# gchhablani/multilingual-image-captioning

Hardware: AMD Instinct MI355X
Metric: train images/sec, ViT-B/32+mBART-50 (bf16 train step, batch 64/GPU, 224x224, seq_len 64) (higher is better)
Workload: dtype bf16

## Files before the change

include/mic_hip.h:

```cpp
#ifndef MIC_HIP_H
#define MIC_HIP_H
#include <stdint.h>
#ifdef __cplusplus
extern "C" {
#endif

#define MIC_OK 0
#define MIC_EINVAL (-1)
#define MIC_ELAUNCH (-2)

#define MIC_BF16 0
#define MIC_F32 1
#define MIC_FP8 2
#define MIC_E4M3 0
#define MIC_E5M2 1

#define MIC_ACT_NONE 0
#define MIC_ACT_GELU_ERF 1
#define MIC_ACT_GELU_TANH 2
#define MIC_ACT_QUICK_GELU 3

int mic_version(void);
const char* mic_last_error(void);

typedef struct {
  int dtype;
  int c_dtype;
  int M, N, K;
  int a_kmajor, b_kmajor;
  const void* A; int lda;
  const void* B; int ldb;
  void* C; int ldc;
  const float* bias;
  int act;
  void* Zout; int ldz;
  const void* Zin; int dact;
  const void* R; int ldr;
  int accumulate;
  float dropout_p; uint32_t dropout_seed;
  float alpha;
  int split_k;
  long long split_stride;
  float* a_rowsum;
  int rowsum_k;
  int a_fmt, b_fmt;
  const float* a_scale_inv;
  const float* b_scale_inv;
  float* rowstat; int rowstat_ld; int rowstat_nvalid;
  const long long* a_ln_stats; const float* a_ln_colsum; int a_ln_width; float a_ln_eps;
  long long* rowsum2;
  int k_valid;
  float* c_q8_state; float* c_q8_amax; int c_q8_fmt;
} mic_gemm_args;
int mic_gemm(const mic_gemm_args* a, void* stream);
int mic_sum_slabs(int dst_dtype, int n_slabs, long long slab_stride, int rows, int cols, const float* src, int ld_src,
                  void* dst, int ld_dst, void* stream);
int mic_gemm_grouped(const mic_gemm_args* args, int count, void* stream);
int mic_set_cu_budget(int cus);
int mic_get_cu_budget(void);
typedef struct { int tile, kgroups, blocks, grid, blocks_per_cu, phased, cu_budget, tile_m; } mic_gemm_plan_info;
int mic_gemm_plan(const mic_gemm_args* args, int count, mic_gemm_plan_info* out);
int mic_ln_fold_weight(int dtype, int N, int K, const void* w, int ldw, const float* gamma, const float* beta, const float* bias,
                       void* w_fold, int ldwf, float* colsum, float* bias_fold, void* stream);

typedef struct {
  const void* src; int ld;
  int rows, cols, rows_pad;
  void* q; int ldq;
  void* qT; int ldqT;
  float* state;
  float* amax_next;
  int fmt;
} mic_fp8_item;
int mic_fp8_amax(const mic_fp8_item* items, int count, void* stream);
int mic_fp8_quantize(const mic_fp8_item* items, int count, void* stream);
int mic_fp8_amax_partials(void);
int mic_fp8_roll_amax(float* state, int stride_floats, float* partials, int count, void* stream);

typedef struct {
  void* q; int ldq;
  float* state;
  float* amax_next;
  int fmt;
} mic_fp8_out;

int mic_layernorm_fwd(int dtype, int rows, int width, const void* x, const float* gamma, const float* beta,
                      float eps, void* y, float* mean, float* rstd, float dropout_p, uint32_t dropout_seed,
                      void* stream);
int mic_layernorm_bwd(int dtype, int rows, int width, const void* x, const float* gamma, const float* mean,
                      const float* rstd, const void* dy, const void* dres, void* dx, float* dgamma, float* dbeta,
                      void* dxm, float dropout_p, uint32_t dropout_seed, float in_dropout_p, uint32_t in_dropout_seed,
                      void* stream);
int mic_layernorm_bwd_blocks(int rows);
int mic_layernorm_bwd_partials(int dtype, int rows, int width, const void* x, const float* gamma, const float* mean,
                               const float* rstd, const void* dy, const void* dres, void* dx, float* partials, void* dxm,
                               float dropout_p, uint32_t dropout_seed, float in_dropout_p, uint32_t in_dropout_seed, void* stream);
int mic_layernorm_fwd_q8(int rows, int width, const void* x, const float* gamma, const float* beta, float eps, void* y, float* mean,
                         float* rstd, float dropout_p, uint32_t dropout_seed, const mic_fp8_out* q8, void* stream);
int mic_layernorm_bwd_partials_q8(int rows, int width, const void* x, const float* gamma, const float* mean, const float* rstd,
                                  const void* dy, const void* dres, void* dx, float* partials, void* dxm, float dropout_p,
                                  uint32_t dropout_seed, float in_dropout_p, uint32_t in_dropout_seed, const mic_fp8_out* q8,
                                  int q8_of_dx, void* stream);
typedef struct { const float* partials; float* dgamma; float* dbeta; int nblk, width, accumulate; } mic_ln_param_item;
int mic_ln_param_grads(const mic_ln_param_item* items, int count, void* stream);

int mic_attn_fwd(int dtype, int B, int H, int Tq, int Tk, const void* q, int ldq, const void* k, int ldk,
                 const void* v, int ldv, void* out, int ldo, const int32_t* key_mask, int causal, float* lse,
                 void* stream);
int mic_attn_bwd(int dtype, int B, int H, int Tq, int Tk, const void* q, int ldq, const void* k, int ldk,
                 const void* v, int ldv, const void* out, int ldo, const void* dout, int lddo, const float* lse,
                 const int32_t* key_mask, int causal, void* dq, int lddq, void* dk, int lddk, void* dv, int lddv,
                 void* stream);

int mic_attn_probs(int dtype, int B, int H, int Tq, int Tk, const void* q, int ldq, const void* k, int ldk,
                   const int32_t* key_mask, int causal, float* out, void* stream);

int mic_attn_fwd_packed(int dtype, int B, int H, int Tq_max, int Tk, const int32_t* q_off, const int32_t* q_len, int kv_packed,
                        const void* q, int ldq, const void* k, int ldk, const void* v, int ldv, void* out, int ldo, int causal,
                        float* lse, void* stream);
int mic_attn_bwd_packed(int dtype, int B, int H, int Tq_max, int Tk, const int32_t* q_off, const int32_t* q_len, int kv_packed,
                        const void* q, int ldq, const void* k, int ldk, const void* v, int ldv, const void* out, int ldo,
                        const void* dout, int lddo, const float* lse, int causal, void* dq, int lddq, void* dk, int lddk,
                        void* dv, int lddv, void* stream);
int mic_attn_bwd_q8(int B, int H, int Tq, int Tk, const int32_t* q_off, const int32_t* q_len, int kv_packed, const void* q, int ldq,
                    const void* k, int ldk, const void* v, int ldv, const void* out, int ldo, const void* dout, int lddo, const float* lse,
                    const int32_t* key_mask, int causal, const mic_fp8_out* dq8, const mic_fp8_out* dk8, void* dv8, void* stream);

int mic_attn_decode(int dtype, int R, int H, int max_len, int cur, const void* q, int ldq, const void* kc,
                    const void* vc, int ldc, const int32_t* src_row, int row_div, void* out, int ldo, void* stream);
int mic_kv_append(int dtype, int R, int HD, int max_len, int cur, const void* k, int ldk, const void* v, int ldv,
                  void* kc, void* vc, void* stream);

int mic_im2col(int dtype, int B, int img, int ps, const float* pixels, void* patches, int ldp, int trunc_int32,
               void* stream);
int mic_vit_assemble(int dtype, int B, int S, int width, const void* patch_out, int ldp, const float* cls,
                     const float* pos, void* x, void* stream);
int mic_vit_assemble_bwd(int dtype, int B, int S, int width, const void* dx, void* dpatch, int ldp, float* dcls,
                         float* dpos, void* stream);

int mic_embed_fwd(int dtype, int rows, int width, const int32_t* ids, const int32_t* pos_ids, const void* table,
                  const float* pos_table, float scale, void* h, void* stream);
int mic_embed_bwd(int dtype, int rows, int width, const int32_t* ids, const int32_t* pos_ids, const void* dh,
                  float scale, float* dtable, float* dpos_table, void* stream);
int mic_embed_rows_add_det(int dtype, int n, int width, int vocab, const int32_t* ids, const void* dh, float scale, float* dtable,
                           int32_t* ws, void* stream);
int64_t mic_embed_rows_add_det_ws(int vocab);

int mic_ce_rows(int dtype, int rows, int V, const void* logits, int ld, const int32_t* labels,
                const int32_t* mask, float label_smoothing, float* row_lse, float* row_loss, void* stream);
int mic_ce_rows_tiles(int dtype, int rows, int V, const void* logits, int ld, const float* rowstat, int stat_ld,
                      const int32_t* labels, float* row_lse, float* row_loss, void* stream);
int mic_ce_reduce(int rows, const float* row_loss, const int32_t* mask, float* loss_out, float* denom_out,
                  void* stream);
int mic_ce_bwd(int dtype, int rows, int V, int Vpad, void* logits, int ld, const int32_t* labels,
               const int32_t* mask, float label_smoothing, const float* row_lse, const float* denom,
               float loss_scale, void* stream);
int mic_ce_bwd_q8(int rows, int V, int Vpad, const void* logits, int ld, const int32_t* labels, const int32_t* mask,
                  float label_smoothing, const float* row_lse, const float* denom, float loss_scale, const mic_fp8_out* q8,
                  float* colsum, float* label_coef, void* stream);
int mic_head_label_terms(int rows, int width, const int32_t* labels, const float* coef, const void* E, int lde, const void* h, int ldh,
                         float* dx_slab, int ldx, float* dE, int ldde, void* stream);
int mic_ce_bwd_t(int rows, int V, int Vpad, void* logits, int ld, const int32_t* labels, const int32_t* mask, float label_smoothing,
                 const float* row_lse, const float* denom, float loss_scale, void* dlogits_t, int ld_t, int rows_pad, float* colsum,
                 void* stream);
int mic_transpose_bf16(int rows, int rows_pad, int cols, const void* src, int ld_src, void* dst, int ld_dst, void* stream);

int mic_colsum(int dtype, int rows, int cols, const void* x, int ld, float* out, int accumulate, void* stream);
typedef struct { const void* x; float* out; int rows, cols, ld; } mic_colsum_item;
int mic_colsum_grouped(int dtype, const mic_colsum_item* items, int count, void* stream);
typedef struct { const void* x; float* out; const float* scale_inv; int rows, cols, ld, fmt; } mic_colsum_q8_item;
int mic_colsum_q8_grouped(const mic_colsum_q8_item* items, int count, void* stream);
int mic_dropout_mask(uint8_t* out, int64_t n, float p, uint32_t seed, void* stream);
int mic_cast(int src_dtype, int dst_dtype, const void* src, void* dst, int64_t n, void* stream);
int mic_zero(void* p, int64_t bytes, void* stream);
int mic_stream_create_cu_masked(int first_cu, int n_cus, void** stream);
int mic_stream_destroy(void* stream);
int mic_comm_emulate(const void* src, void* dst, int64_t bytes, float micros, int blocks, void* stream);
int mic_copy_rows(int dtype, int n, int width, const void* src, int ld_src, const int32_t* src_idx, void* dst, int ld_dst,
                  const int32_t* dst_idx, void* stream);
int mic_cast2d(int src_dtype, int dst_dtype, int rows, int cols, const void* src, int ld_src, void* dst, int ld_dst,
               void* stream);

int mic_adamw(int64_t n, float* p, float* m, float* v, const float* g, void* p_lp, const float* hyper, double b1,
              double b2, double eps, double wd, float grad_scale, void* stream);
int mic_adamw_rows(int64_t rows, int width, const uint8_t* row_flag, int want, float* p, float* m, float* v, const float* g,
                   void* p_lp, const float* hyper, double b1, double b2, double eps, double wd, float grad_scale, void* stream);
int mic_row_flags(const int32_t* ids, int n_ids, uint8_t* flags, int n_rows, void* stream);

int mic_row_lse_topk(int dtype, int R, int V, const void* logits, int ld, int k, int forced_token,
                     int suppress_eos, int eos_token_id, int raw_logits, const float* row_bias, float* top_val,
                     int32_t* top_idx, void* stream);

int mic_row_topk_tiles(int dtype, int R, int V, const void* logits, int ld, const float* rowstat, int stat_ld, int k,
                       int suppress_eos, int eos_token_id, int raw_logits, const float* row_bias, float* top_val,
                       int32_t* top_idx, void* stream);

typedef struct {
  int B, K, max_len, V;
  int cur_len;
  int eos_token_id, pad_token_id;
  float length_penalty; int early_stopping;
  const float* cand_val;
  const int32_t* cand_idx;
  int32_t* running_seq;
  float* running_scores;
  int32_t* seq;
  float* scores;
  int32_t* finished;
  int32_t* src_row;
  int32_t* next_token;
  int32_t* flags;
  int32_t* gstate;
} mic_beam_step_args;
int mic_beam_step(const mic_beam_step_args* a, void* stream);

int mic_greedy_step(int B, int max_len, int cur_len, int eos_token_id, int pad_token_id, const int32_t* top_idx,
                    int ld_top, int32_t* sequences, int32_t* finished, int32_t* next_token, void* stream);

int mic_sample_rows(int dtype, int R, int V, const void* logits, int ld, uint32_t key0, uint32_t key1,
                    float temperature, int forced_token, int suppress_eos, int eos_token_id, const float* min_keep,
                    const int32_t* tie_limit, int32_t* out_idx, void* stream);
int mic_warp_thresholds(int dtype, int R, int V, const void* logits, int ld, float temperature, int suppress_eos,
                        int eos_token_id, int top_k, float top_p, float* thr, int32_t* tie_limit, void* stream);

typedef struct { const void* src; int H, W, hwc; } mic_image_item;
int mic_image_transform(const mic_image_item* items, int n, int out_size, const float* mean, const float* std,
                        float* dst, int dst_chw, void* stream);

#ifdef __cplusplus
}
#endif
#endif
```

multilingual-image-captioning_amd/_lib.py:

```python
from __future__ import annotations

import ctypes as C
import os

_HERE = os.path.dirname(os.path.abspath(__file__))
LIB_PATH = os.path.join(_HERE, "libmic_hip.so")

MIC_BF16, MIC_F32, MIC_FP8 = 0, 1, 2
MIC_E4M3, MIC_E5M2 = 0, 1
ACT_NONE, ACT_GELU_ERF, ACT_GELU_TANH, ACT_QUICK_GELU = 0, 1, 2, 3
ACT_IDS = {"none": 0, None: 0, "gelu": 1, "erf": 1, "gelu_erf": 1, "tanh": 2, "gelu_tanh": 2, "gelu_new": 2, "quick_gelu": 3}


class MicError(RuntimeError):
    pass


class GemmArgs(C.Structure):
    _fields_ = [
        ("dtype", C.c_int), ("c_dtype", C.c_int), ("M", C.c_int), ("N", C.c_int), ("K", C.c_int),
        ("a_kmajor", C.c_int), ("b_kmajor", C.c_int),
        ("A", C.c_void_p), ("lda", C.c_int), ("B", C.c_void_p), ("ldb", C.c_int), ("C", C.c_void_p), ("ldc", C.c_int),
        ("bias", C.c_void_p), ("act", C.c_int), ("Zout", C.c_void_p), ("ldz", C.c_int), ("Zin", C.c_void_p),
        ("dact", C.c_int), ("R", C.c_void_p), ("ldr", C.c_int), ("accumulate", C.c_int), ("dropout_p", C.c_float),
        ("dropout_seed", C.c_uint32), ("alpha", C.c_float), ("split_k", C.c_int),
        ("split_stride", C.c_longlong), ("a_rowsum", C.c_void_p), ("rowsum_k", C.c_int),
        ("a_fmt", C.c_int), ("b_fmt", C.c_int), ("a_scale_inv", C.c_void_p), ("b_scale_inv", C.c_void_p),
        ("rowstat", C.c_void_p), ("rowstat_ld", C.c_int), ("rowstat_nvalid", C.c_int),
        ("a_ln_stats", C.c_void_p), ("a_ln_colsum", C.c_void_p), ("a_ln_width", C.c_int), ("a_ln_eps", C.c_float),
        ("rowsum2", C.c_void_p), ("k_valid", C.c_int),
        ("c_q8_state", C.c_void_p), ("c_q8_amax", C.c_void_p), ("c_q8_fmt", C.c_int),
    ]


class Fp8Item(C.Structure):
    _fields_ = [("src", C.c_void_p), ("ld", C.c_int), ("rows", C.c_int), ("cols", C.c_int), ("rows_pad", C.c_int),
                ("q", C.c_void_p), ("ldq", C.c_int), ("qT", C.c_void_p), ("ldqT", C.c_int), ("state", C.c_void_p), ("amax_next", C.c_void_p),
                ("fmt", C.c_int)]


class Fp8Out(C.Structure):
    _fields_ = [("q", C.c_void_p), ("ldq", C.c_int), ("state", C.c_void_p), ("amax_next", C.c_void_p), ("fmt", C.c_int)]


class ColsumQ8Item(C.Structure):
    _fields_ = [("x", C.c_void_p), ("out", C.c_void_p), ("scale_inv", C.c_void_p), ("rows", C.c_int), ("cols", C.c_int), ("ld", C.c_int), ("fmt", C.c_int)]


class ColsumItem(C.Structure):
    _fields_ = [("x", C.c_void_p), ("out", C.c_void_p), ("rows", C.c_int), ("cols", C.c_int), ("ld", C.c_int)]


class BeamStepArgs(C.Structure):
    _fields_ = [
        ("B", C.c_int), ("K", C.c_int), ("max_len", C.c_int), ("V", C.c_int), ("cur_len", C.c_int),
        ("eos_token_id", C.c_int), ("pad_token_id", C.c_int), ("length_penalty", C.c_float), ("early_stopping", C.c_int),
        ("cand_val", C.c_void_p), ("cand_idx", C.c_void_p), ("running_seq", C.c_void_p), ("running_scores", C.c_void_p),
        ("seq", C.c_void_p), ("scores", C.c_void_p), ("finished", C.c_void_p), ("src_row", C.c_void_p),
        ("next_token", C.c_void_p), ("flags", C.c_void_p), ("gstate", C.c_void_p),
    ]


class GemmPlanInfo(C.Structure):
    _fields_ = [("tile", C.c_int), ("kgroups", C.c_int), ("blocks", C.c_int), ("grid", C.c_int), ("blocks_per_cu", C.c_int),
                ("phased", C.c_int), ("cu_budget", C.c_int), ("tile_m", C.c_int)]


class LnParamItem(C.Structure):
    _fields_ = [("partials", C.c_void_p), ("dgamma", C.c_void_p), ("dbeta", C.c_void_p), ("nblk", C.c_int), ("width", C.c_int), ("accumulate", C.c_int)]


class ImageItem(C.Structure):
    _fields_ = [("src", C.c_void_p), ("H", C.c_int), ("W", C.c_int), ("hwc", C.c_int)]


_i, _f, _p, _u32, _i64 = C.c_int, C.c_float, C.c_void_p, C.c_uint32, C.c_int64
_SIGS = {
    "mic_version": ([], C.c_int),
    "mic_last_error": ([], C.c_char_p),
    "mic_gemm": ([C.POINTER(GemmArgs), _p], C.c_int),
    "mic_gemm_grouped": ([C.POINTER(GemmArgs), _i, _p], C.c_int),
    "mic_set_cu_budget": ([_i], C.c_int),
    "mic_get_cu_budget": ([], C.c_int),
    "mic_gemm_plan": ([C.POINTER(GemmArgs), _i, C.POINTER(GemmPlanInfo)], C.c_int),
    "mic_comm_emulate": ([_p, _p, _i64, _f, _i, _p], C.c_int),
    "mic_ln_fold_weight": ([_i, _i, _i, _p, _i, _p, _p, _p, _p, _i, _p, _p, _p], C.c_int),
    "mic_fp8_amax": ([C.POINTER(Fp8Item), _i, _p], C.c_int),
    "mic_fp8_quantize": ([C.POINTER(Fp8Item), _i, _p], C.c_int),
    "mic_fp8_amax_partials": ([], C.c_int),
    "mic_fp8_roll_amax": ([_p, _i, _p, _i, _p], C.c_int),
    "mic_sum_slabs": ([_i, _i, C.c_longlong, _i, _i, _p, _i, _p, _i, _p], C.c_int),
    "mic_layernorm_fwd": ([_i, _i, _i, _p, _p, _p, _f, _p, _p, _p, _f, _u32, _p], C.c_int),
    "mic_layernorm_bwd": ([_i, _i, _i, _p, _p, _p, _p, _p, _p, _p, _p, _p, _p, _f, _u32, _f, _u32, _p], C.c_int),
    "mic_layernorm_bwd_blocks": ([_i], C.c_int),
    "mic_layernorm_bwd_partials": ([_i, _i, _i, _p, _p, _p, _p, _p, _p, _p, _p, _p, _f, _u32, _f, _u32, _p], C.c_int),
    "mic_ln_param_grads": ([C.POINTER(LnParamItem), _i, _p], C.c_int),
    "mic_layernorm_fwd_q8": ([_i, _i, _p, _p, _p, _f, _p, _p, _p, _f, _u32, C.POINTER(Fp8Out), _p], C.c_int),
    "mic_layernorm_bwd_partials_q8": ([_i, _i, _p, _p, _p, _p, _p, _p, _p, _p, _p, _f, _u32, _f, _u32, C.POINTER(Fp8Out), _i, _p], C.c_int),
    "mic_attn_bwd_q8": ([_i, _i, _i, _i, _p, _p, _i, _p, _i, _p, _i, _p, _i, _p, _i, _p, _i, _p, _p, _i, C.POINTER(Fp8Out), C.POINTER(Fp8Out), _p, _p], C.c_int),
    "mic_colsum_q8_grouped": ([C.POINTER(ColsumQ8Item), _i, _p], C.c_int),
    "mic_attn_fwd": ([_i, _i, _i, _i, _i, _p, _i, _p, _i, _p, _i, _p, _i, _p, _i, _p, _p], C.c_int),
    "mic_attn_probs": ([_i, _i, _i, _i, _i, _p, _i, _p, _i, _p, _i, _p, _p], C.c_int),
    "mic_attn_bwd": ([_i, _i, _i, _i, _i, _p, _i, _p, _i, _p, _i, _p, _i, _p, _i, _p, _p, _i, _p, _i, _p, _i, _p, _i, _p], C.c_int),
    "mic_attn_fwd_packed": ([_i, _i, _i, _i, _i, _p, _p, _i, _p, _i, _p, _i, _p, _i, _p, _i, _i, _p, _p], C.c_int),
    "mic_attn_bwd_packed": ([_i, _i, _i, _i, _i, _p, _p, _i, _p, _i, _p, _i, _p, _i, _p, _i, _p, _i, _p, _i, _p, _i, _p, _i, _p, _i, _p], C.c_int),
    "mic_attn_decode": ([_i, _i, _i, _i, _i, _p, _i, _p, _p, _i, _p, _i, _p, _i, _p], C.c_int),
    "mic_kv_append": ([_i, _i, _i, _i, _i, _p, _i, _p, _i, _p, _p, _p], C.c_int),
    "mic_im2col": ([_i, _i, _i, _i, _p, _p, _i, _i, _p], C.c_int),
    "mic_vit_assemble": ([_i, _i, _i, _i, _p, _i, _p, _p, _p, _p], C.c_int),
    "mic_vit_assemble_bwd": ([_i, _i, _i, _i, _p, _p, _i, _p, _p, _p], C.c_int),
    "mic_embed_fwd": ([_i, _i, _i, _p, _p, _p, _p, _f, _p, _p], C.c_int),
    "mic_embed_bwd": ([_i, _i, _i, _p, _p, _p, _f, _p, _p, _p], C.c_int),
    "mic_embed_rows_add_det": ([_i, _i, _i, _i, _p, _p, _f, _p, _p, _p], C.c_int),
    "mic_embed_rows_add_det_ws": ([_i], C.c_int64),
    "mic_ce_rows": ([_i, _i, _i, _p, _i, _p, _p, _f, _p, _p, _p], C.c_int),
    "mic_ce_rows_tiles": ([_i, _i, _i, _p, _i, _p, _i, _p, _p, _p, _p], C.c_int),
    "mic_row_topk_tiles": ([_i, _i, _i, _p, _i, _p, _i, _i, _i, _i, _i, _p, _p, _p, _p], C.c_int),
    "mic_ce_reduce": ([_i, _p, _p, _p, _p, _p], C.c_int),
    "mic_ce_bwd": ([_i, _i, _i, _i, _p, _i, _p, _p, _f, _p, _p, _f, _p], C.c_int),
    "mic_ce_bwd_t": ([_i, _i, _i, _p, _i, _p, _p, _f, _p, _p, _f, _p, _i, _i, _p, _p], C.c_int),
    "mic_ce_bwd_q8": ([_i, _i, _i, _p, _i, _p, _p, _f, _p, _p, _f, C.POINTER(Fp8Out), _p, _p, _p], C.c_int),
    "mic_head_label_terms": ([_i, _i, _p, _p, _p, _i, _p, _i, _p, _i, _p, _i, _p], C.c_int),
    "mic_transpose_bf16": ([_i, _i, _i, _p, _i, _p, _i, _p], C.c_int),
    "mic_colsum": ([_i, _i, _i, _p, _i, _p, _i, _p], C.c_int),
    "mic_colsum_grouped": ([_i, C.POINTER(ColsumItem), _i, _p], C.c_int),
    "mic_dropout_mask": ([_p, _i64, _f, _u32, _p], C.c_int),
    "mic_cast": ([_i, _i, _p, _p, _i64, _p], C.c_int),
    "mic_zero": ([_p, _i64, _p], C.c_int),
    "mic_stream_create_cu_masked": ([_i, _i, C.POINTER(C.c_void_p)], C.c_int),
    "mic_stream_destroy": ([_p], C.c_int),
    "mic_copy_rows": ([_i, _i, _i, _p, _i, _p, _p, _i, _p, _p], C.c_int),
    "mic_cast2d": ([_i, _i, _i, _i, _p, _i, _p, _i, _p], C.c_int),
    "mic_adamw": ([_i64, _p, _p, _p, _p, _p, _p, C.c_double, C.c_double, C.c_double, C.c_double, _f, _p], C.c_int),
    "mic_adamw_rows": ([_i64, _i, _p, _i, _p, _p, _p, _p, _p, _p, C.c_double, C.c_double, C.c_double, C.c_double, _f, _p], C.c_int),
    "mic_row_flags": ([_p, _i, _p, _i, _p], C.c_int),
    "mic_row_lse_topk": ([_i, _i, _i, _p, _i, _i, _i, _i, _i, _i, _p, _p, _p, _p], C.c_int),
    "mic_beam_step": ([C.POINTER(BeamStepArgs), _p], C.c_int),
    "mic_greedy_step": ([_i, _i, _i, _i, _i, _p, _i, _p, _p, _p, _p], C.c_int),
    "mic_sample_rows": ([_i, _i, _i, _p, _i, _u32, _u32, _f, _i, _i, _i, _p, _p, _p, _p], C.c_int),
    "mic_warp_thresholds": ([_i, _i, _i, _p, _i, _f, _i, _i, _i, _f, _p, _p, _p], C.c_int),
    "mic_image_transform": ([C.POINTER(ImageItem), _i, _i, C.POINTER(C.c_float), C.POINTER(C.c_float), _p, _i, _p], C.c_int),
}
EXPORTS = tuple(_SIGS)

_lib = None


def lib() -> C.CDLL:
    global _lib
    if _lib is None:
        if not os.path.exists(LIB_PATH):
            raise MicError(f"{LIB_PATH} is missing: build it with `python -c 'import __graft_entry__ as g; g.build()'` "
                           "(hipcc --offload-arch=gfx950).  The HIP path has no fallback.")
        l = C.CDLL(LIB_PATH)
        for name, (args, res) in _SIGS.items():
            fn = getattr(l, name)
            fn.argtypes, fn.restype = args, res
        _lib = l
    return _lib


def check(rc: int, what: str = "") -> None:
    if rc != 0:
        raise MicError(f"{what} failed (rc={rc}): {lib().mic_last_error().decode()}")
```

multilingual-image-captioning_amd/csrc/elementwise.hip:

```cpp
#include "common.h"
#include <stdarg.h>
#include <type_traits>

static thread_local char g_err[512] = "";
void mic_set_error(const char* fmt, ...) {
  va_list ap;
  va_start(ap, fmt);
  vsnprintf(g_err, sizeof(g_err), fmt, ap);
  va_end(ap);
}
extern "C" const char* mic_last_error(void) { return g_err; }
extern "C" int mic_version(void) { return 1; }

template <typename F>
static int dispatch_t(int dtype, F&& f) {
  if (dtype == MIC_BF16) f((uint16_t*)nullptr);
  else if (dtype == MIC_F32) f((float*)nullptr);
  else { mic_set_error("bad dtype %d", dtype); return MIC_EINVAL; }
  hipError_t e = hipGetLastError();
  if (e != hipSuccess) { mic_set_error("launch failed: %s", hipGetErrorString(e)); return MIC_ELAUNCH; }
  return MIC_OK;
}
#define TYPE_OF(tag) typename std::remove_pointer<decltype(tag)>::type

// ... 464 lines not shown
__global__ __launch_bounds__(256) void ce_bwd_kernel(int V, int Vpad, T* __restrict__ logits, int ld,
                                                     const int32_t* __restrict__ labels, const int32_t* __restrict__ mask,
                                                     float ls, const float* __restrict__ row_lse, const float* __restrict__ denom,
                                                     float loss_scale) {
  const int row = blockIdx.x;
  T* lr = logits + (size_t)row * ld;
  const float w = mask[row] ? loss_scale / denom[0] : 0.f;
  const float lse = row_lse[row];
  const int label = labels[row];
  const float conf = 1.0f - ls, low = ls > 0.f ? ls / (float)(V - 1) : 0.f;
  const int nchunk = Vpad >> 3;
  constexpr int U = 4;
  for (int ch0 = threadIdx.x; ch0 < nchunk; ch0 += 256 * U) {
    float v[U][8];
#pragma unroll
    for (int u = 0; u < U; ++u)
      if (ch0 + u * 256 < nchunk) ld8(lr + (ch0 + u * 256) * 8, v[u]);
#pragma unroll
    for (int u = 0; u < U; ++u) {
      const int ch = ch0 + u * 256;
      if (ch >= nchunk) break;
      float o[8];
#pragma unroll
      for (int i = 0; i < 8; ++i) {
        const int c = ch * 8 + i;
        o[i] = c < V ? w * (__expf(v[u][i] - lse) - (c == label ? conf : low)) : 0.f;
      }
      st8(lr + ch * 8, o);
    }
  }
}
extern "C" int mic_ce_bwd(int dtype, int rows, int V, int Vpad, void* logits, int ld, const int32_t* labels,
                          const int32_t* mask, float label_smoothing, const float* row_lse, const float* denom,
                          float loss_scale, void* stream) {
  MIC_CHECK(rows > 0 && V > 1 && Vpad >= V && Vpad % 8 == 0 && ld >= Vpad && logits && labels && mask && row_lse && denom, "mic_ce_bwd: bad args");
  return dispatch_t(dtype, [&](auto* tag) {
    using T = TYPE_OF(tag);
    hipLaunchKernelGGL(ce_bwd_kernel<T>, dim3(rows), dim3(256), 0, (hipStream_t)stream, V, Vpad, (T*)logits, ld, labels, mask, label_smoothing, row_lse, denom, loss_scale);
  });
}

struct TransposeArgs {
  const uint16_t* src; uint16_t* src_rw; int ld_src;
  uint16_t* dst; int ld_dst;
  int rows, cols;
  int V; const int32_t* labels; const int32_t* mask; float ls; const float* row_lse; const float* denom; float loss_scale;
  float* colsum;
};
template <int OP>
__global__ __launch_bounds__(256) void tile_transpose_kernel(TransposeArgs a) {
  __shared__ __attribute__((aligned(16))) char img[64 * 1024];
  const int tid = threadIdx.x, lane = tid & 63, wave = tid >> 6;
  const int c0 = blockIdx.x * 512, r0 = blockIdx.y * 64;
  const int col = c0 + lane * 8;
  const bool col_ok = col < a.cols;
  uint4 q[16];
#pragma unroll
  for (int rr = 0; rr < 16; ++rr) {
    const int row = r0 + wave * 16 + rr;
    q[rr] = make_uint4(0u, 0u, 0u, 0u);
    if (row < a.rows && col_ok) q[rr] = *reinterpret_cast<const uint4*>(a.src + (size_t)row * a.ld_src + col);
  }
  float inv_denom = 0.f;
  if constexpr (OP == 1) inv_denom = a.loss_scale / a.denom[0];
#pragma unroll
  for (int rr = 0; rr < 16; ++rr) {
    const int k = wave * 16 + rr, row = r0 + k;
    uint4 u = q[rr];
    if constexpr (OP == 1) {
      if (row < a.rows && col_ok) {
        const float w = a.mask[row] ? inv_denom : 0.f;
        const float lse = a.row_lse[row];
        const int label = a.labels[row];
        const float conf = 1.0f - a.ls, low = a.ls > 0.f ? a.ls / (float)(a.V - 1) : 0.f;
        const uint32_t wd[4] = {u.x, u.y, u.z, u.w};
        float o[8];
#pragma unroll
        for (int i = 0; i < 8; ++i) {
          const float x = __uint_as_float((i & 1) ? (wd[i >> 1] & 0xffff0000u) : (wd[i >> 1] << 16));
          const int c = col + i;
          o[i] = c < a.V ? w * (__expf(x - lse) - (c == label ? conf : low)) : 0.f;
        }
        u.x = f2bf_pk(o[0], o[1]); u.y = f2bf_pk(o[2], o[3]); u.z = f2bf_pk(o[4], o[5]); u.w = f2bf_pk(o[6], o[7]);
        *reinterpret_cast<uint4*>(a.src_rw + (size_t)row * a.ld_src + col) = u;
      }
    }
    const int pos = (lane & ~7) | ((lane ^ (k >> 3)) & 7);
    *reinterpret_cast<uint4*>(img + k * 1024 + pos * 16) = u;
  }
  __syncthreads();
  const int kc = lane & 7, xx = lane >> 3;
#pragma unroll 4
  for (int it = 0; it < 16; ++it) {
    const int xl = wave * 128 + it * 8 + xx;
    const int c = xl >> 3;
    const int pos = (c & ~7) | ((c ^ kc) & 7);
    const char* base = img + (kc * 8) * 1024 + pos * 16 + (xl & 7) * 2;
    uint16_t e[8];
#pragma unroll
    for (int i = 0; i < 8; ++i) e[i] = *reinterpret_cast<const uint16_t*>(base + i * 1024);
    const int x = c0 + xl;
    if (x < a.cols) {
      uint4 u;
      u.x = (uint32_t)e[0] | ((uint32_t)e[1] << 16); u.y = (uint32_t)e[2] | ((uint32_t)e[3] << 16);
      u.z = (uint32_t)e[4] | ((uint32_t)e[5] << 16); u.w = (uint32_t)e[6] | ((uint32_t)e[7] << 16);
      *reinterpret_cast<uint4*>(a.dst + (size_t)x * a.ld_dst + r0 + kc * 8) = u;
    }
    if constexpr (OP == 1) {
      if (a.colsum != nullptr) {
        float sacc = 0.f;
#pragma unroll
        for (int i = 0; i < 8; ++i) sacc += bf2f(e[i]);
        sacc = group8_sum(sacc);
        if (kc == 0 && x < a.cols && sacc != 0.f) atomicAdd(a.colsum + x, sacc);
      }
    }
  }
}
extern "C" int mic_transpose_bf16(int rows, int rows_pad, int cols, const void* src, int ld_src, void* dst, int ld_dst, void* stream) {
  if (rows_pad <= 0) rows_pad = (rows + 63) / 64 * 64;
  MIC_CHECK(rows > 0 && cols > 0 && cols % 8 == 0 && src && dst && ld_src >= cols && ld_src % 8 == 0 && rows_pad >= rows && rows_pad % 64 == 0 &&
                ld_dst >= rows_pad && ld_dst % 8 == 0,
            "mic_transpose_bf16: bad args (cols %% 8 == 0, ld_src %% 8 == 0, rows_pad %% 64 == 0, ld_dst >= rows_pad and %% 8 == 0)");
  MIC_CHECK(((uintptr_t)src & 15) == 0 && ((uintptr_t)dst & 15) == 0, "mic_transpose_bf16: 16-B aligned operands");
  TransposeArgs a{};
  a.src = (const uint16_t*)src; a.ld_src = ld_src; a.dst = (uint16_t*)dst; a.ld_dst = ld_dst; a.rows = rows; a.cols = cols;
  hipLaunchKernelGGL(tile_transpose_kernel<0>, dim3((cols + 511) / 512, rows_pad / 64), dim3(256), 0, (hipStream_t)stream, a);
  MIC_LAUNCH_CHECK();
  return MIC_OK;
}
extern "C" int mic_ce_bwd_t(int rows, int V, int Vpad, void* logits, int ld, const int32_t* labels, const int32_t* mask,
                            float label_smoothing, const float* row_lse, const float* denom, float loss_scale, void* dlogits_t,
                            int ld_t, int rows_pad, float* colsum, void* stream) {
  if (rows_pad <= 0) rows_pad = (rows + 63) / 64 * 64;
  MIC_CHECK(rows_pad >= rows && rows_pad % 64 == 0, "mic_ce_bwd_t: rows_pad >= rows, a multiple of 64");
  MIC_CHECK(rows > 0 && V > 1 && Vpad >= V && Vpad % 8 == 0 && ld >= Vpad && ld % 8 == 0 && logits && labels && mask && row_lse && denom && dlogits_t,
            "mic_ce_bwd_t: bad args");
  MIC_CHECK(ld_t >= rows_pad && ld_t % 8 == 0 && ((uintptr_t)logits & 15) == 0 && ((uintptr_t)dlogits_t & 15) == 0,
            "mic_ce_bwd_t: ld_t >= rows rounded up to 64, ld_t %% 8 == 0, 16-B aligned operands");
  TransposeArgs a{};
  a.src = (const uint16_t*)logits; a.src_rw = (uint16_t*)logits; a.ld_src = ld; a.dst = (uint16_t*)dlogits_t; a.ld_dst = ld_t;
  a.rows = rows; a.cols = Vpad; a.V = V; a.labels = labels; a.mask = mask; a.ls = label_smoothing; a.row_lse = row_lse; a.denom = denom;
  a.loss_scale = loss_scale; a.colsum = colsum;
  hipLaunchKernelGGL(tile_transpose_kernel<1>, dim3((Vpad + 511) / 512, rows_pad / 64), dim3(256), 0, (hipStream_t)stream, a);
  MIC_LAUNCH_CHECK();
  return MIC_OK;
}

struct CeQ8Args {
  const uint16_t* logits; int ld; int rows, V, Vpad;
  const int32_t* labels; const int32_t* mask; float ls; const float* row_lse; const float* denom; float loss_scale;
  float* colsum; uint8_t* q; int ldq; float* state; int fmt;
  float* label_coef;
};
constexpr int CEQ8_RG = 4;
__global__ __launch_bounds__(256) void ce_bwd_q8_kernel(CeQ8Args a) {
  __shared__ __attribute__((aligned(16))) float cs[4][512];
  const int tid = threadIdx.x, lane = tid & 63, wave = tid >> 6;
  const int c0 = blockIdx.x * 512;
  const int col = c0 + lane * 8;
  const bool col_ok = col < a.Vpad;
  const float fmax = a.fmt == MIC_E4M3 ? 448.0f : 57344.0f;
  const float inv_denom = a.loss_scale / a.denom[0];
  if (blockIdx.x == 0 && blockIdx.y == 0 && tid == 0) { a.state[0] = fmax / inv_denom; a.state[1] = inv_denom / fmax; }
  const float conf = 1.0f - a.ls, low = a.ls > 0.f ? a.ls / (float)(a.V - 1) : 0.f;
  float csum[8] = {0.f, 0.f, 0.f, 0.f, 0.f, 0.f, 0.f, 0.f};
  for (int rg = 0; rg < CEQ8_RG; ++rg) {
    const int r0 = (blockIdx.y * CEQ8_RG + rg) * 64;
    if (r0 >= a.rows) break;
    uint4 q[16];
#pragma unroll
    for (int rr = 0; rr < 16; ++rr) {
      const int row = r0 + wave * 16 + rr;
      q[rr] = make_uint4(0u, 0u, 0u, 0u);
      if (row < a.rows && col_ok) q[rr] = *reinterpret_cast<const uint4*>(a.logits + (size_t)row * a.ld + col);
    }
#pragma unroll
    for (int rr = 0; rr < 16; ++rr) {
      const int row = r0 + wave * 16 + rr;
      if (row < a.rows && col_ok) {
        const float w = a.mask[row] ? 1.0f : 0.f;
        const float lse = a.row_lse[row];
        const int label = a.labels[row];
        if (a.label_coef != nullptr && col == 0 && (label < 0 || label >= a.V)) a.label_coef[row] = 0.f;
        const uint32_t wd[4] = {q[rr].x, q[rr].y, q[rr].z, q[rr].w};
        float o[8];
#pragma unroll
        for (int i = 0; i < 8; ++i) {
          const float x = __uint_as_float((i & 1) ? (wd[i >> 1] & 0xffff0000u) : (wd[i >> 1] << 16));
          const int c = col + i;
          const float g = c < a.V ? w * (__expf(x - lse) - (c == label ? conf : low)) : 0.f;
          csum[i] += g;
          o[i] = fminf(fmaxf(g * fmax, -fmax), fmax);
          if (c == label && a.label_coef != nullptr) {
            a.label_coef[row] = g * inv_denom;
            o[i] = 0.f;
          }
        }
        *reinterpret_cast<uint2*>(a.q + (size_t)row * a.ldq + col) = make_uint2(cvt4_fp8(o, a.fmt), cvt4_fp8(o + 4, a.fmt));
      }
    }
  }
  if (a.colsum != nullptr) {
    *reinterpret_cast<float4*>(&cs[wave][lane * 8]) = make_float4(csum[0], csum[1], csum[2], csum[3]);
    *reinterpret_cast<float4*>(&cs[wave][lane * 8 + 4]) = make_float4(csum[4], csum[5], csum[6], csum[7]);
    __syncthreads();
#pragma unroll
    for (int h = 0; h < 2; ++h) {
      const int c = tid + h * 256;
      const float s4 = (cs[0][c] + cs[1][c]) + (cs[2][c] + cs[3][c]);
      if (c0 + c < a.Vpad && s4 != 0.f) atomicAdd(a.colsum + c0 + c, s4 * inv_denom);
    }
  }
}
extern "C" int mic_ce_bwd_q8(int rows, int V, int Vpad, const void* logits, int ld, const int32_t* labels, const int32_t* mask,
                             float label_smoothing, const float* row_lse, const float* denom, float loss_scale, const mic_fp8_out* q8,
                             float* colsum, float* label_coef, void* stream) {
  MIC_CHECK(rows > 0 && V > 1 && Vpad >= V && Vpad % 8 == 0 && ld >= Vpad && ld % 8 == 0 && logits && labels && mask && row_lse && denom && q8,
            "mic_ce_bwd_q8: bad args");
  MIC_CHECK(q8->q && q8->state && q8->ldq >= Vpad && q8->ldq % 8 == 0 && ((uintptr_t)q8->q & 7) == 0 && ((uintptr_t)logits & 15) == 0 &&
                (q8->fmt == MIC_E4M3 || q8->fmt == MIC_E5M2),
            "mic_ce_bwd_q8: fp8 output [rows][ldq >= Vpad] (ldq %% 8 == 0, 8-B aligned), a scale state, 16-B aligned bf16 logits");
  CeQ8Args a{};
  a.logits = (const uint16_t*)logits; a.ld = ld; a.rows = rows; a.V = V; a.Vpad = Vpad; a.labels = labels; a.mask = mask; a.ls = label_smoothing;
  a.row_lse = row_lse; a.denom = denom; a.loss_scale = loss_scale; a.colsum = colsum;
  a.q = (uint8_t*)q8->q; a.ldq = q8->ldq; a.state = q8->state; a.fmt = q8->fmt; a.label_coef = label_coef;
  hipLaunchKernelGGL(ce_bwd_q8_kernel, dim3((Vpad + 511) / 512, (rows + 64 * CEQ8_RG - 1) / (64 * CEQ8_RG)), dim3(256), 0, (hipStream_t)stream, a);
  MIC_LAUNCH_CHECK();
  return MIC_OK;
}

__global__ __launch_bounds__(256) void head_label_terms_kernel(int rows, int width, const int32_t* __restrict__ labels, const float* __restrict__ coef,
                                                               const uint16_t* __restrict__ E, int lde, const uint16_t* __restrict__ h, int ldh,
                                                               float* __restrict__ dx_slab, int ldx, float* __restrict__ dE, int ldde) {
  const int m = blockIdx.x;
  const float c = coef[m];
  const int lab = labels[m];
  for (int j = threadIdx.x; j < width; j += 256) {
    float o = 0.f;
    if (c != 0.f) {
      o = c * bf2f(E[(size_t)lab * lde + j]);
      atomicAdd(dE + (size_t)lab * ldde + j, c * bf2f(h[(size_t)m * ldh + j]));
    }
    dx_slab[(size_t)m * ldx + j] = o;
  }
}
extern "C" int mic_head_label_terms(int rows, int width, const int32_t* labels, const float* coef, const void* E, int lde, const void* h, int ldh,
                                    float* dx_slab, int ldx, float* dE, int ldde, void* stream) {
  MIC_CHECK(rows > 0 && width > 0 && width % 8 == 0 && labels && coef && E && h && dx_slab && dE && lde % 8 == 0 && ldh % 8 == 0 && ldx % 4 == 0,
            "mic_head_label_terms: bad args (width, lde, ldh multiples of 8; bf16 E and h)");
  hipLaunchKernelGGL(head_label_terms_kernel, dim3(rows), dim3(256), 0, (hipStream_t)stream, rows, width, labels, coef, (const uint16_t*)E, lde,
                     (const uint16_t*)h, ldh, dx_slab, ldx, dE, ldde);
  MIC_LAUNCH_CHECK();
  return MIC_OK;
}

#define COLSUM_MAX 8
struct ColsumItem { const void* x; float* out; int rows, cols, ld, gx, gy, block_begin; };
struct ColsumTable { int count; ColsumItem it[COLSUM_MAX]; };

template <typename T>
__global__ __launch_bounds__(256) void colsum_kernel(ColsumTable tab) {
  __shared__ float red[8][256 + 8];
  int pi = 0;
#pragma unroll
  for (int i = 1; i < COLSUM_MAX; ++i)
    if (i < tab.count && (int)blockIdx.x >= tab.it[i].block_begin) pi = i;
  const ColsumItem& I = tab.it[pi];
  const int local = blockIdx.x - I.block_begin;
  const int bx = local % I.gx, by = local / I.gx;
  const T* __restrict__ x = (const T*)I.x;
  const int rows = I.rows, cols = I.cols, ld = I.ld;
  const int cc = threadIdx.x & 31, rl = threadIdx.x >> 5;
  const int c0 = bx * 256 + cc * 8;
  const int rows_per = (rows + I.gy - 1) / I.gy;
  const int r0 = by * rows_per, r1 = min(rows, r0 + rows_per);
  float acc[8] = {0, 0, 0, 0, 0, 0, 0, 0};
  if (c0 + 8 <= cols) {
    for (int r = r0 + rl; r < r1; r += 8) {
      float v[8];
      ld8(x + (size_t)r * ld + c0, v);
#pragma unroll
      for (int i = 0; i < 8; ++i) acc[i] += v[i];
    }
  } else if (c0 < cols) {
    for (int r = r0 + rl; r < r1; r += 8)
      for (int i = 0; i < cols - c0; ++i) acc[i] += ElemT<T>::ld(x + (size_t)r * ld + c0 + i);
  }
#pragma unroll
  for (int i = 0; i < 8; ++i) red[rl][cc * 8 + i] = acc[i];
  __syncthreads();
  const int c = bx * 256 + threadIdx.x;
  if (c < cols) {
    float s = 0.f;
#pragma unroll
    for (int j = 0; j < 8; ++j) s += red[j][threadIdx.x];
    atomicAdd(I.out + c, s);
  }
}
static int colsum_launch(int dtype, const mic_colsum_item* items, int count, void* stream) {
  ColsumTable tab;
  tab.count = count;
  int blocks = 0;
  for (int i = 0; i < count; ++i) {
    const mic_colsum_item& a = items[i];
    MIC_CHECK(a.rows > 0 && a.cols > 0 && a.x && a.out, "mic_colsum: bad args");
    MIC_CHECK(a.ld % 8 == 0 && ((uintptr_t)a.x & 15) == 0, "mic_colsum: rows must be 16-B aligned");
    ColsumItem& t = tab.it[i];
    t.x = a.x; t.out = a.out; t.rows = a.rows; t.cols = a.cols; t.ld = a.ld;
    t.gx = (a.cols + 255) / 256;
    int gy = (a.rows + 63) / 64;
    const int cap = (1024 + t.gx - 1) / t.gx;
    if (gy > cap) gy = cap;
    t.gy = gy < 1 ? 1 : gy;
    t.block_begin = blocks;
    blocks += t.gx * t.gy;
  }
  return dispatch_t(dtype, [&](auto* tag) {
    using T = TYPE_OF(tag);
    hipLaunchKernelGGL(colsum_kernel<T>, dim3(blocks), dim3(256), 0, (hipStream_t)stream, tab);
  });
}
struct Colsum8Item { const uint8_t* x; float* out; const float* scale_inv; int rows, cols, ld, fmt, gx, gy, block_begin; };
struct Colsum8Table { int count; Colsum8Item it[COLSUM_MAX]; };
typedef float f32x2v __attribute__((ext_vector_type(2)));
__global__ __launch_bounds__(256) void colsum_q8_kernel(Colsum8Table tab) {
  __shared__ float red[8][256 + 8];
  int pi = 0;
#pragma unroll
  for (int i = 1; i < COLSUM_MAX; ++i)
    if (i < tab.count && (int)blockIdx.x >= tab.it[i].block_begin) pi = i;
  const Colsum8Item& I = tab.it[pi];
  const int local = blockIdx.x - I.block_begin;
  const int bx = local % I.gx, by = local / I.gx;
  const int cc = threadIdx.x & 31, rl = threadIdx.x >> 5;
  const int c0 = bx * 256 + cc * 8;
  const int rows_per = (I.rows + I.gy - 1) / I.gy;
  const int r0 = by * rows_per, r1 = min(I.rows, r0 + rows_per);
  float acc[8] = {0, 0, 0, 0, 0, 0, 0, 0};
  if (c0 < I.cols) {
    for (int r = r0 + rl; r < r1; r += 8) {
      const uint2 u = *reinterpret_cast<const uint2*>(I.x + (size_t)r * I.ld + c0);
      const int w[2] = {(int)u.x, (int)u.y};
#pragma unroll
      for (int h = 0; h < 2; ++h) {
        f32x2v lo, hi;
        if (I.fmt == MIC_E4M3) { lo = __builtin_amdgcn_cvt_pk_f32_fp8(w[h], false); hi = __builtin_amdgcn_cvt_pk_f32_fp8(w[h], true); }
        else { lo = __builtin_amdgcn_cvt_pk_f32_bf8(w[h], false); hi = __builtin_amdgcn_cvt_pk_f32_bf8(w[h], true); }
        acc[4 * h + 0] += lo[0]; acc[4 * h + 1] += lo[1]; acc[4 * h + 2] += hi[0]; acc[4 * h + 3] += hi[1];
      }
    }
  }
#pragma unroll
  for (int i = 0; i < 8; ++i) red[rl][cc * 8 + i] = acc[i];
  __syncthreads();
  const int c = bx * 256 + threadIdx.x;
  if (c < I.cols) {
    float t = 0.f;
#pragma unroll
    for (int j = 0; j < 8; ++j) t += red[j][threadIdx.x];
    atomicAdd(I.out + c, t * I.scale_inv[0]);
  }
}
extern "C" int mic_colsum_q8_grouped(const mic_colsum_q8_item* items, int count, void* stream) {
  MIC_CHECK(items && count >= 1, "mic_colsum_q8_grouped: bad args");
  for (int i0 = 0; i0 < count; i0 += COLSUM_MAX) {
    Colsum8Table tab;
    tab.count = count - i0 < COLSUM_MAX ? count - i0 : COLSUM_MAX;
    int blocks = 0;
    for (int i = 0; i < tab.count; ++i) {
      const mic_colsum_q8_item& a = items[i0 + i];
      MIC_CHECK(a.rows > 0 && a.cols > 0 && a.x && a.out && a.scale_inv, "mic_colsum_q8_grouped: bad item %d", i0 + i);
      MIC_CHECK(a.cols % 8 == 0 && a.ld % 8 == 0 && ((uintptr_t)a.x & 7) == 0 && (a.fmt == MIC_E4M3 || a.fmt == MIC_E5M2), "mic_colsum_q8_grouped: cols, ld multiples of 8; fmt");
      Colsum8Item& t = tab.it[i];
      t.x = (const uint8_t*)a.x; t.out = a.out; t.scale_inv = a.scale_inv; t.rows = a.rows; t.cols = a.cols; t.ld = a.ld; t.fmt = a.fmt;
      t.gx = (a.cols + 255) / 256;
      int gy = (a.rows + 63) / 64;
      const int cap = (1024 + t.gx - 1) / t.gx;
      if (gy > cap) gy = cap;
// ... 267 lines not shown
```

multilingual-image-captioning_amd/csrc/gemm.hip:

```cpp
#include "gemm_common.h"

__global__ __launch_bounds__(256) void gemm_f32_kernel(const float* __restrict__ A, long sam, long sak,
                                                       const float* __restrict__ B, long sbk, long sbn, int M, int N,
                                                       int K, EpiArgs epi) {
  __shared__ float As[64][17];
  __shared__ float Bs[16][65];
  const int tid = threadIdx.x, lane = tid & 63, wave = tid >> 6;
  const int m0 = blockIdx.y * 64, n0 = blockIdx.x * 64;
  const int wr = wave >> 1, wc = wave & 1;
  f32x16 acc;
#pragma unroll
  for (int r = 0; r < 16; ++r) acc[r] = 0.0f;
  for (int k0 = 0; k0 < K; k0 += 16) {
#pragma unroll
    for (int i = 0; i < 4; ++i) {
      const int e = tid + i * 256;
      {
        int mm, kk;
        if (sak == 1) { mm = e >> 4; kk = e & 15; } else { kk = e >> 6; mm = e & 63; }
        const int gm = m0 + mm, gk = k0 + kk;
        As[mm][kk] = (gm < M && gk < K) ? A[gm * sam + gk * sak] : 0.0f;
      }
      {
        int nn, kk;
        if (sbk == 1) { nn = e >> 4; kk = e & 15; } else { kk = e >> 6; nn = e & 63; }
        const int gn = n0 + nn, gk = k0 + kk;
        Bs[kk][nn] = (gn < N && gk < K) ? B[gk * sbk + gn * sbn] : 0.0f;
      }
    }
    __syncthreads();
#pragma unroll
    for (int k = 0; k < 16; k += 2) {
      const float a = As[wr * 32 + (lane & 31)][k + (lane >> 5)];
      const float b = Bs[k + (lane >> 5)][wc * 32 + (lane & 31)];
      acc = __builtin_amdgcn_mfma_f32_32x32x2f32(a, b, acc, 0, 0, 0);
    }
    __syncthreads();
  }
  const int n = n0 + wc * 32 + (lane & 31);
#pragma unroll
  for (int r = 0; r < 16; ++r) {
    const int m = m0 + wr * 32 + (r & 3) + 8 * (r >> 2) + 4 * (lane >> 5);
    if (m < M && n < N) epilogue_store<float>(epi, m, n, acc[r]);
  }
}

static int fill_epi(const mic_gemm_args* a, EpiArgs& e) {
  MIC_CHECK(a && a->A && a->B && a->C, "mic_gemm: null pointer");
  MIC_CHECK(a->M > 0 && a->N > 0 && a->K > 0, "mic_gemm: bad shape M=%d N=%d K=%d", a->M, a->N, a->K);
  MIC_CHECK(a->dtype == MIC_BF16 || a->dtype == MIC_F32 || a->dtype == MIC_FP8, "mic_gemm: bad dtype %d", a->dtype);
  if (a->dtype == MIC_FP8) {
    MIC_CHECK(a->c_dtype == MIC_BF16 || a->c_dtype == MIC_F32 || a->c_dtype == MIC_FP8, "mic_gemm(fp8): C is bf16, f32 or (fused emission) fp8");
    if (a->c_dtype == MIC_FP8) {
      MIC_CHECK(a->c_q8_state && (a->c_q8_fmt == MIC_E4M3 || a->c_q8_fmt == MIC_E5M2), "mic_gemm(fp8 C): c_q8_state / c_q8_fmt");
      MIC_CHECK((a->act || a->dact || a->Zout) && !a->accumulate && a->split_k <= 1 && !a->a_kmajor, "mic_gemm(fp8 C): an activation / dact epilogue of an NT launch, no accumulate / split-K");
      MIC_CHECK(a->N % 8 == 0 && a->ldc % 8 == 0 && ((uintptr_t)a->C & 7) == 0 && (!a->Zout || a->ldz % 8 == 0) && (!a->Zin || a->ldz % 8 == 0) && (!a->R || a->ldr % 8 == 0),
                "mic_gemm(fp8 C): N, ldc, ldz, ldr multiples of 8");
    }
    MIC_CHECK(a->a_kmajor == a->b_kmajor, "mic_gemm(fp8): both operands k-contiguous (NT) or both k-major (TN, the weight-gradient GEMM)");
    if (a->a_kmajor) MIC_CHECK(a->M % 16 == 0 && a->N % 16 == 0, "mic_gemm(fp8, k-major): M and N must be multiples of 16");
    MIC_CHECK((a->a_fmt == MIC_E4M3 || a->a_fmt == MIC_E5M2) && a->b_fmt == MIC_E4M3, "mic_gemm(fp8): A is e4m3 or e5m2, B is e4m3");
    MIC_CHECK(a->K % 128 == 0, "mic_gemm(fp8): K=%d must be a multiple of 128 (zero-pad the reduction dim)", a->K);
    MIC_CHECK(a->lda % 16 == 0 && a->ldb % 16 == 0, "mic_gemm(fp8): lda/ldb must be multiples of 16 bytes");
    MIC_CHECK(((uintptr_t)a->A & 15) == 0 && ((uintptr_t)a->B & 15) == 0, "mic_gemm(fp8): A/B must be 16-B aligned");
    MIC_CHECK(!a->a_rowsum, "mic_gemm(fp8): no row sums on the fp8 path (mic_colsum_q8_grouped)");
    if (a->split_k > 1)
      MIC_CHECK(a->split_stride > 0 && a->c_dtype == MIC_F32 && !a->a_kmajor && !a->bias && !a->act && !a->dact && !a->Zout && !a->R && !a->accumulate && a->dropout_p == 0.f,
                "mic_gemm(fp8): split_k writes raw fp32 partial sums into per-split slabs (split_stride > 0, NT, no other epilogue)");
  } else
  MIC_CHECK(a->c_dtype == a->dtype || a->c_dtype == MIC_F32, "mic_gemm: c_dtype must be dtype or f32");
  MIC_CHECK(!(a->dact && !a->Zin), "mic_gemm: dact needs Zin");
  MIC_CHECK(a->dropout_p >= 0.f && a->dropout_p < 1.f, "mic_gemm: dropout_p out of range");
  MIC_CHECK(a->c_dtype != MIC_FP8 || a->dtype == MIC_FP8, "mic_gemm: an fp8 C belongs to the fp8 GEMMs");
  e.C = a->C; e.ldc = a->ldc; e.c_f32 = (a->c_dtype == MIC_F32);
  e.c_q8 = a->c_dtype == MIC_FP8 ? 1 + a->c_q8_fmt : 0; e.q8_state = a->c_q8_state; e.q8_amax = a->c_q8_amax;
  e.bias = a->bias; e.act = a->act; e.Zout = a->Zout; e.ldz = a->ldz; e.Zin = a->Zin; e.dact = a->dact;
  e.R = a->R; e.ldr = a->ldr; e.accumulate = a->accumulate;
  e.drop_thr = a->dropout_p > 0.f ? (uint32_t)fminf(a->dropout_p * 4294967296.0f, 4294967295.0f) : 0u;
  e.drop_seed = a->dropout_seed; e.drop_scale = 1.0f / (1.0f - a->dropout_p);
  e.alpha = a->alpha == 0.f ? 1.0f : a->alpha; e.N = a->N;
  e.rowstat = a->rowstat; e.stat_ld = a->rowstat_ld; e.stat_nvalid = a->rowstat_nvalid > 0 ? a->rowstat_nvalid : a->N;
  if (a->rowstat) {
    MIC_CHECK((a->dtype == MIC_BF16 || (a->dtype == MIC_FP8 && !a->a_kmajor)) && a->c_dtype == MIC_BF16 && a->split_k <= 1 && !a->act && !a->dact && !a->R &&
                  !a->accumulate && a->dropout_p == 0.f && !a->Zout,
              "mic_gemm: rowstat goes with the bare bias epilogue of a bf16 / fp8 NT GEMM with a bf16 C (the LM head)");
    MIC_CHECK(a->N % 64 == 0 && a->ldc % 8 == 0 && ((uintptr_t)a->C & 15) == 0, "mic_gemm: rowstat needs N %% 64 == 0 and a 16-B aligned C");
    MIC_CHECK(a->rowstat_ld >= a->N / 64 && ((uintptr_t)a->rowstat & 7) == 0, "mic_gemm: rowstat needs ld >= N / 64 float2 entries per row");
  }
  e.ln_stats = a->a_ln_stats; e.ln_g = a->a_ln_colsum; e.ln_bias = nullptr; e.ln_inv_d = 0.f; e.ln_eps = a->a_ln_eps;
  e.rowsum2 = a->rowsum2;
  if (a->a_ln_stats) {
    MIC_CHECK(a->dtype == MIC_BF16 && a->a_ln_colsum && a->bias && a->a_ln_width > 0, "mic_gemm: a folded LayerNorm needs bf16 operands, a_ln_colsum, bias' and a_ln_width");
    MIC_CHECK(a->split_k <= 1 && !a->dact && !a->accumulate && (a->alpha == 0.f || a->alpha == 1.f), "mic_gemm: folded LayerNorm: no split-K / dact / accumulate / alpha");
    MIC_CHECK(a->N % 8 == 0 && a->ldc % 8 == 0 && ((uintptr_t)a->C & 15) == 0 && (!a->R || a->ldr % 8 == 0) && (!a->Zout || a->ldz % 8 == 0),
              "mic_gemm: folded LayerNorm needs the vector epilogue (N, ldc, ldr, ldz multiples of 8, 16-B aligned C)");
    e.ln_bias = a->bias; e.bias = nullptr; e.ln_inv_d = 1.0f / (float)a->a_ln_width;
  }
  if (a->rowsum2) {
    MIC_CHECK(a->dtype == MIC_BF16 && a->N % 128 == 0 && a->split_k <= 1 && !a->act && !a->dact && !a->Zout && !a->accumulate,
              "mic_gemm: rowsum2 goes with the bare / residual epilogue of a bf16 GEMM, N %% 128 == 0");
    MIC_CHECK(a->ldc % 8 == 0 && ((uintptr_t)a->C & 15) == 0 && (!a->R || (a->ldr % 8 == 0 && ((uintptr_t)a->R & 15) == 0 && a->c_dtype != MIC_F32)),
              "mic_gemm: rowsum2 needs the PLAIN store path (16-B aligned C / R rows)");
  }
  if (a->dtype == MIC_BF16) {
    MIC_CHECK(a->K % 64 == 0, "mic_gemm(bf16): K=%d must be a multiple of 64 (zero-pad the reduction dim)", a->K);
    MIC_CHECK(a->lda % 8 == 0 && a->ldb % 8 == 0, "mic_gemm(bf16): lda/ldb must be multiples of 8");
    MIC_CHECK(((uintptr_t)a->A & 15) == 0 && ((uintptr_t)a->B & 15) == 0, "mic_gemm(bf16): A/B must be 16-B aligned");
    if (a->a_kmajor) MIC_CHECK(a->M % 8 == 0, "mic_gemm(bf16): k-major A needs M %% 8 == 0");
    if (a->b_kmajor) MIC_CHECK(a->N % 8 == 0, "mic_gemm(bf16): k-major B needs N %% 8 == 0");
    if (a->split_k > 1)
      MIC_CHECK(a->c_dtype == MIC_F32 && !a->bias && !a->act && !a->dact && !a->Zout && !a->R && !a->accumulate && a->dropout_p == 0.f,
                "mic_gemm: split_k accumulates raw fp32 partial sums into a zeroed C (no other epilogue)");
  }
  return MIC_OK;
}

bool table_is_plain(const LaunchTable& t) {
  for (int i = 0; i < t.count; ++i) {
    const EpiArgs& e = t.p[i].epi;
    if (t.p[i].nsplit > 1 || e.act || e.Zout || e.dact || e.accumulate || (e.ldc & 7)) return false;
    if (((uintptr_t)e.C & 15) != 0) return false;
    if (e.R && ((e.ldr & 7) || ((uintptr_t)e.R & 15) || e.c_f32)) return false;
  }
  return true;
}
static bool any_rowsum_early(const mic_gemm_args* args, int count) {
  for (int i = 0; i < count; ++i)
    if (args[i].a_rowsum) return true;
  return false;
}
static thread_local int g_cu_budget = 0;
int mic_cu_budget_now() {
  static const int env = [] { const char* e = getenv("MIC_FREE_CUS"); return e ? atoi(e) : 0; }();
  int c = g_cu_budget > 0 ? g_cu_budget : (env > 0 ? env : 256);
  c = c < 8 ? 8 : (c > 256 ? 256 : c);
  return c & ~7;
}
extern "C" int mic_set_cu_budget(int cus) {
  MIC_CHECK(cus == 0 || (cus >= 8 && cus <= 1024), "mic_set_cu_budget: %d (0 = default, else 8..1024)", cus);
  g_cu_budget = cus;
  return MIC_OK;
}
extern "C" int mic_get_cu_budget(void) { return mic_cu_budget_now(); }

struct GemmPlan { int bm, bm_m, kgroups, blocks, grid, per_cu, phased; };

static GemmPlan plan_bf16(const mic_gemm_args* args, int count) {
  const int cus = mic_cu_budget_now();
  GemmPlan pl{};
  long tiles_big = 0, tiles_small = 0;
  for (int i = 0; i < count; ++i) {
    const int sp = args[i].split_k > 1 ? args[i].split_k : 1;
    tiles_big += (long)((args[i].M + 255) / 256) * ((args[i].N + 255) / 256) * sp;
    tiles_small += (long)((args[i].M + 127) / 128) * ((args[i].N + 127) / 128) * sp;
  }
  static const int force = [] { const char* e = getenv("MIC_GEMM_TILE"); return e ? atoi(e) : 0; }();
  static const int tiny_below = [] { const char* e = getenv("MIC_TINY_BELOW"); return e ? atoi(e) : MIC_TINY_BELOW; }();
  int bm = tiles_big >= (200L * cus) / 256 ? 256 : (tiles_small < ((long)tiny_below * cus) / 256 ? 64 : 128);
  static const int quant_env = [] { const char* e = getenv("MIC_GEMM_QUANT"); return e ? atoi(e) : 0; }();
  if (bm == 256 && (cus < 256 || quant_env)) {
    const double c256 = (double)((tiles_big + cus - 1) / cus), c128 = 0.3125 * (double)((tiles_small + cus - 1) / cus);
    if (c128 < c256) bm = 128;
  }
  if (force == 256 || force == 128 || force == 64) bm = force;
  if (args[0].dtype == MIC_FP8 && args[0].a_kmajor && bm < 128) bm = 128;
  for (int i = 0; i < count; ++i)
    if (args[i].c_dtype == MIC_FP8 && bm == 256) bm = 128;
  for (int i = 0; i < count; ++i)
    if (args[i].rowstat) bm = 256;
  static const int t192 = [] { const char* e = getenv("MIC_GEMM_T192"); return e ? atoi(e) : 1; }();
  int bm_m = bm;
  if (bm == 128 && t192 && force == 0 && count == 1 && args[0].dtype == MIC_BF16 && !args[0].a_kmajor && args[0].split_k <= 1) {
    const long t128 = (long)((args[0].M + 127) / 128) * ((args[0].N + 127) / 128), t192n = (long)((args[0].M + 191) / 192) * ((args[0].N + 127) / 128);
    if (t128 > 2L * cus && t192n <= 2L * cus) bm_m = 192;
  }
  int blocks = 0, kmin = 1 << 30;
  for (int i = 0; i < count; ++i) {
    int nsplit = args[i].split_k > 1 ? args[i].split_k : 1;
    const int kt = (args[i].dtype == MIC_FP8 ? args[i].K / 2 : args[i].K) / 64;
    if (nsplit > kt) nsplit = kt;
    if (nsplit < 1) nsplit = 1;
    blocks += ((args[i].M + bm_m - 1) / bm_m) * ((args[i].N + bm - 1) / bm) * nsplit;
    kmin = kt / nsplit < kmin ? kt / nsplit : kmin;
  }
  pl.bm = bm; pl.bm_m = bm_m; pl.blocks = pl.grid = blocks; pl.kgroups = 1; pl.per_cu = 1;
  static const int phased_env = [] { const char* e = getenv("MIC_GEMM_PHASED"); return e ? atoi(e) : 2; }();
  const bool f8 = args[0].dtype == MIC_FP8;
  pl.phased = bm == 256 && !f8 && phased_env != 0 && !args[0].a_kmajor && !args[0].b_kmajor && count == 1 && !any_rowsum_early(args, count);
  static const int w4_env = [] { const char* e = getenv("MIC_GEMM_W4"); return e ? atoi(e) : 1; }();
  if (pl.phased && w4_env && args[0].K >= 256 && args[0].K % 128 == 0) pl.phased = 2;
  if (bm == 256) {
    pl.per_cu = 1;
  } else if (bm == 128) {
    static const int kg128 = [] { const char* e = getenv("MIC_GEMM_KG128"); return e ? atoi(e) : -1; }();
    const bool two = bm_m == 128 && (kg128 >= 0 ? kg128 == 2 : (blocks <= cus && kmin >= 8));
    pl.kgroups = two ? 2 : 1;
    pl.per_cu = two ? 1 : 2;
  } else {
    static const int kg_force = [] { const char* e = getenv("MIC_GEMM_KG"); return e ? atoi(e) : 0; }();
    int kgs = blocks <= cus && kmin >= 16 ? 4 : (blocks <= 2 * cus && kmin >= 8 ? 2 : 1);
    if (kg_force == 1 || kg_force == 2 || kg_force == 4) kgs = kg_force;
    pl.kgroups = kgs;
    pl.per_cu = 4 / kgs;
  }
  return pl;
}

extern "C" int mic_gemm_plan(const mic_gemm_args* args, int count, mic_gemm_plan_info* out) {
  MIC_CHECK(args && out && count >= 1 && count <= MAX_PROBLEMS, "mic_gemm_plan: bad args (1..%d problems)", MAX_PROBLEMS);
  MIC_CHECK(args[0].dtype == MIC_BF16 || args[0].dtype == MIC_FP8, "mic_gemm_plan: the planner belongs to the bf16 / fp8 kernels");
  const GemmPlan pl = plan_bf16(args, count);
  out->tile = pl.bm; out->tile_m = pl.bm_m; out->kgroups = pl.kgroups; out->blocks = pl.blocks; out->blocks_per_cu = pl.per_cu; out->phased = pl.phased;
  out->cu_budget = mic_cu_budget_now();
  static const int persist_env = [] { const char* e = getenv("MIC_GEMM_PERSIST"); return e ? atoi(e) : 1; }();
  bool plain = true;
  for (int i = 0; i < count; ++i) {
    const mic_gemm_args& a = args[i];
    if (a.split_k > 1 || a.act || a.Zout || a.dact || a.accumulate || (a.ldc & 7) || ((uintptr_t)a.C & 15)) plain = false;
    if (a.R && ((a.ldr & 7) || ((uintptr_t)a.R & 15) || a.c_dtype == MIC_F32)) plain = false;
  }
  const bool persist = persist_env && plain && pl.bm == 256 && !pl.phased && pl.kgroups == 1 && pl.blocks > out->cu_budget;
  out->grid = persist ? out->cu_budget : pl.blocks;
  static const int d2_plan_env = [] { const char* e = getenv("MIC_GEMM_D2"); return e ? atoi(e) : 3; }();
  if (d2_plan_env && pl.phased == 2 && count == 1 && args[0].rowstat && args[0].N % 128 == 0) {
    out->tile = 128; out->tile_m = 256; out->blocks_per_cu = 2;
    out->blocks = out->grid = ((args[0].M + 255) / 256) * ((args[0].N + 127) / 128);
  }
  return MIC_OK;
}

static int launch_bf16(const mic_gemm_args* args, int count, hipStream_t s) {
  LaunchTable tab;
  tab.count = count;
  const int f8 = args[0].dtype == MIC_FP8 ? (args[0].a_fmt == MIC_E5M2 ? 2 : 1) : 0;
  const GemmPlan pl = plan_bf16(args, count);
  const int bm = pl.bm, bm_m = pl.bm_m;
  int blocks = 0;
  for (int i = 0; i < count; ++i) {
    Problem& p = tab.p[i];
    if (int rc = fill_epi(&args[i], p.epi)) return rc;
    MIC_CHECK(args[i].a_kmajor == args[0].a_kmajor && args[i].b_kmajor == args[0].b_kmajor && args[i].dtype == args[0].dtype &&
                  (args[i].dtype == MIC_BF16 || (args[i].dtype == MIC_FP8 && args[i].a_fmt == args[0].a_fmt)),
              "mic_gemm_grouped: all problems of a group must share dtype (bf16 / fp8 format) and operand layouts");
    p.A = (const uint16_t*)args[i].A; p.B = (const uint16_t*)args[i].B;
    p.lda = args[i].lda; p.ldb = args[i].ldb; p.M = args[i].M; p.N = args[i].N; p.K = args[i].K;
    p.sa = p.sb = nullptr;
    if (f8) {
      if (!args[i].a_kmajor) { p.lda /= 2; p.ldb /= 2; }
      p.K /= 2;
      p.sa = args[i].a_scale_inv; p.sb = args[i].b_scale_inv;
    }
    p.tiles_m = (p.M + bm_m - 1) / bm_m; p.tiles_n = (p.N + bm - 1) / bm;
    p.nsplit = args[i].split_k > 1 ? args[i].split_k : 1;
    if (p.nsplit > p.K / 64) p.nsplit = p.K / 64;
    p.split_stride = p.nsplit > 1 ? args[i].split_stride : 0;
    MIC_CHECK(args[i].split_stride >= 0 && (args[i].split_stride == 0 || args[i].split_stride >= (long long)(p.M - 1) * args[i].ldc + p.N),
              "mic_gemm: split_stride must cover one M x N slab");
    MIC_CHECK(p.split_stride == 0 || p.nsplit == args[i].split_k, "mic_gemm: split_k exceeds K/64 with a slab workspace");
    MIC_CHECK(!args[i].a_rowsum || args[i].a_kmajor, "mic_gemm: a_rowsum needs a_kmajor (A = dy^T of the weight-gradient GEMM)");
    p.a_rowsum = args[i].a_rowsum;
    p.rowsum_k = args[i].rowsum_k > 0 ? args[i].rowsum_k : p.K;
    MIC_CHECK(args[i].k_valid >= 0 && (args[i].k_valid == 0 || (args[i].a_kmajor && args[i].b_kmajor)),
              "mic_gemm: k_valid is a feature of the k-major x k-major (weight-gradient) launches");
    p.k_valid = args[i].k_valid > 0 ? args[i].k_valid : 0x7fffffff;
    p.block_begin = blocks;
    blocks += p.tiles_m * p.tiles_n * p.nsplit;
  }
  tab.total_blocks = blocks;
  for (int i = 0; i < count; ++i)
    MIC_CHECK(!args[i].rowsum2 || table_is_plain(tab), "mic_gemm_grouped: rowsum2 needs every problem of the launch on the bare / residual epilogue");
  static const int d2_env = [] { const char* e = getenv("MIC_GEMM_D2"); return e ? atoi(e) : 3; }();
  const bool nt1 = bm == 256 && !f8 && !args[0].a_kmajor && !args[0].b_kmajor && count == 1;
  if (d2_env && nt1 && gemm_d2_takes(tab) && (d2_env == 2 || (pl.phased == 2 && gemm_w4_takes(tab))) && (d2_env != 3 || tab.p[0].epi.rowstat)) {
    Problem& p = tab.p[0];
    p.tiles_n = (p.N + 127) / 128;
    tab.total_blocks = p.tiles_m * p.tiles_n * p.nsplit;
    launch_gemm_d2(tab, s);
  } else
  if (bm == 256 && pl.phased == 2 && gemm_w4_takes(tab)) launch_gemm_w4(tab, s);
  else if (bm == 256 && pl.phased && tab.p[0].nsplit == 1) launch_gemm_phased(tab, args[0].a_kmajor, args[0].b_kmajor, table_is_plain(tab), s);
  else if (bm == 256) launch_gemm_t256(tab, args[0].a_kmajor, args[0].b_kmajor, s, f8);
  else if (bm == 128 && bm_m == 192) launch_gemm_t192(tab, args[0].b_kmajor, s);
  else if (bm == 128) launch_gemm_t128(tab, args[0].a_kmajor, args[0].b_kmajor, s, f8, pl.kgroups);
  else launch_gemm_t64(tab, args[0].a_kmajor, args[0].b_kmajor, s, f8, pl.kgroups);
  MIC_LAUNCH_CHECK();
  return MIC_OK;
}

extern "C" int mic_gemm(const mic_gemm_args* a, void* stream) {
  MIC_CHECK(a, "mic_gemm: null args");
  hipStream_t s = (hipStream_t)stream;
  if (a->dtype == MIC_BF16 || a->dtype == MIC_FP8) return launch_bf16(a, 1, s);
  EpiArgs e;
  if (int rc = fill_epi(a, e)) return rc;
  MIC_CHECK(a->split_k <= 1, "mic_gemm(f32): split_k is a bf16-path feature");
  MIC_CHECK(!a->a_rowsum, "mic_gemm(f32): a_rowsum is a bf16-path feature (use mic_colsum)");
  MIC_CHECK(a->k_valid == 0, "mic_gemm(f32): k_valid is a bf16-path feature");
  dim3 grid((a->N + 63) / 64, (a->M + 63) / 64), block(256);
  const long sam = a->a_kmajor ? 1 : a->lda, sak = a->a_kmajor ? a->lda : 1;
  const long sbk = a->b_kmajor ? a->ldb : 1, sbn = a->b_kmajor ? 1 : a->ldb;
  hipLaunchKernelGGL(gemm_f32_kernel, grid, block, 0, s, (const float*)a->A, sam, sak, (const float*)a->B, sbk, sbn,
                     a->M, a->N, a->K, e);
  MIC_LAUNCH_CHECK();
  return MIC_OK;
}

extern "C" int mic_gemm_grouped(const mic_gemm_args* args, int count, void* stream) {
  MIC_CHECK(args && count >= 1, "mic_gemm_grouped: bad args");
  hipStream_t s = (hipStream_t)stream;
  if (args[0].dtype != MIC_BF16 && args[0].dtype != MIC_FP8) {
    for (int i = 0; i < count; ++i)
      if (int rc = mic_gemm(&args[i], stream)) return rc;
    return MIC_OK;
  }
  for (int i = 0; i < count; i += MAX_PROBLEMS) {
    const int n = count - i < MAX_PROBLEMS ? count - i : MAX_PROBLEMS;
    if (int rc = launch_bf16(args + i, n, s)) return rc;
  }
  return MIC_OK;
}
```

multilingual-image-captioning_amd/csrc/gemm_common.h:

```cpp
#pragma once
#include "common.h"

#define MAX_PROBLEMS 8
#ifndef MIC_TINY_BELOW
#define MIC_TINY_BELOW 128
#endif

struct Problem {
  const uint16_t* A; const uint16_t* B;
  int lda, ldb, M, N, K;
  int tiles_m, tiles_n, block_begin, nsplit;
  float* a_rowsum; int rowsum_k;
  int k_valid;
  long long split_stride;
  const float* sa; const float* sb;
  EpiArgs epi;
};
struct LaunchTable { int count; int total_blocks; Problem p[MAX_PROBLEMS]; };
int mic_cu_budget_now();
void launch_gemm_phased(const LaunchTable& tab, int akm, int bkm, bool plain, hipStream_t s);
bool gemm_w4_takes(const LaunchTable& tab);
void launch_gemm_w4(const LaunchTable& tab, hipStream_t s);
bool gemm_d2_takes(const LaunchTable& tab);
void launch_gemm_d2(const LaunchTable& tab, hipStream_t s);
bool table_is_plain(const LaunchTable& t);
void launch_gemm_t256(const LaunchTable& tab, int akm, int bkm, hipStream_t s, int f8);
void launch_gemm_t128(const LaunchTable& tab, int akm, int bkm, hipStream_t s, int f8, int kgroups);
void launch_gemm_t192(const LaunchTable& tab, int bkm, hipStream_t s);
void launch_gemm_t64(const LaunchTable& tab, int akm, int bkm, hipStream_t s, int f8, int kgroups);

template <bool KMAJOR, int NWAVES, int BKT, int ROWS>
struct HalfStager {
  static_assert(ROWS == 128 || (ROWS == 64 && BKT == 64), "image = 128 rows (x) of BKT k, or 64 rows of 64 k");
  static constexpr int NINST = ROWS * BKT * 2 / 1024;
  static constexpr int PER = NINST / NWAVES;
  static_assert(PER >= 1, "too many waves for this image");
  static __device__ __forceinline__ void coords(int q, int lane, int& row, int& c) {
    if (!KMAJOR) {
      if (BKT == 64) { row = q * 8 + (lane >> 3); c = lane & 7; }
      else { row = q * 16 + (lane >> 2); c = lane & 3; }
    } else if (ROWS == 128) { row = q * 4 + (lane >> 4); c = lane & 15; }
    else { row = q * 8 + (lane >> 3); c = lane & 7; }
  }
  static __device__ __forceinline__ void load(u32x4 (&r)[PER], const uint16_t* __restrict__ src, int ld, int x0, int k0, int lim,
                                              int wave, int lane) {
#pragma unroll
    for (int i = 0; i < PER; ++i) {
      int row, c;
      coords(wave * PER + i, lane, row, c);
      const uint16_t* g;
      if (!KMAJOR) {
        int gr = x0 + row;
        gr = gr < lim ? gr : lim - 1;
        g = src + (size_t)gr * ld + k0 + c * 8;
      } else {
        int gx = x0 + c * 8;
        gx = gx < lim ? gx : 0;
        g = src + (size_t)(k0 + row) * ld + gx;
      }
      r[i] = *reinterpret_cast<const u32x4*>(g);
    }
  }
  static __device__ __forceinline__ void store(const u32x4 (&r)[PER], char* lds_tile, int wave, int lane, int k_rows_valid = 0x7fffffff) {
#pragma unroll
    for (int i = 0; i < PER; ++i) {
      int row, c;
      coords(wave * PER + i, lane, row, c);
      int off;
      if (!KMAJOR) off = BKT == 64 ? row * 128 + ((c ^ ((row >> 1) & 7)) << 4) : row * 64 + ((c ^ ((row >> 2) & 3)) << 4);
      else if (ROWS == 128) off = row * 256 + ((c ^ ((row & 3) << 2)) << 4);
      else off = row * 128 + ((c ^ (((row >> 1) & 1) << 2)) << 4);
      u32x4 v = r[i];
      if (KMAJOR && row >= k_rows_valid) v = u32x4{0u, 0u, 0u, 0u};
      *reinterpret_cast<u32x4*>(lds_tile + off) = v;
    }
  }
};

template <bool KMAJOR, int BKT, int ROWS>
__device__ __forceinline__ bf16x8 read_frag(const char* lds_tile, int xb, int kk, int lane) {
  if (!KMAJOR) {
    const int row = xb + (lane & 31);
    const int kc = kk * 2 + (lane >> 5);
    if (BKT == 64) return *reinterpret_cast<const bf16x8*>(lds_tile + row * 128 + ((kc ^ ((row >> 1) & 7)) << 4));
    return *reinterpret_cast<const bf16x8*>(lds_tile + row * 64 + ((kc ^ ((row >> 2) & 3)) << 4));
  } else {
    const int g = lane >> 4, p = lane & 15;
    const int x = xb + 16 * (g & 1) + (p & 3) * 4;
    const int k = kk * 16 + 8 * (g >> 1) + (p >> 2);
    constexpr int RB = ROWS * 2;
    const int off = ROWS == 128 ? k * 256 + ((((x >> 3) ^ ((k & 3) << 2)) << 4) | ((x & 7) << 1))
                                : k * 128 + ((((x >> 3) ^ (((k >> 1) & 1) << 2)) << 4) | ((x & 7) << 1));
    s16x4 lo = __builtin_amdgcn_ds_read_tr16_b64_v4i16(LDS_PTR(s16x4, lds_tile + off));
    s16x4 hi = __builtin_amdgcn_ds_read_tr16_b64_v4i16(LDS_PTR(s16x4, lds_tile + off + 4 * RB));
    s16x8 r = {lo[0], lo[1], lo[2], lo[3], hi[0], hi[1], hi[2], hi[3]};
    return __builtin_bit_cast(bf16x8, r);
  }
}

typedef int i32x8 __attribute__((ext_vector_type(8)));
__device__ __forceinline__ i32x8 read_frag8(const char* lds_tile, int xb, int mm, int lane) {
  const int row = xb + (lane & 31);
  const int kc = mm * 4 + 2 * (lane >> 5);
  const int sw = (row >> 1) & 7;
  const u32x4 lo = *reinterpret_cast<const u32x4*>(lds_tile + row * 128 + (((kc) ^ sw) << 4));
  const u32x4 hi = *reinterpret_cast<const u32x4*>(lds_tile + row * 128 + (((kc + 1) ^ sw) << 4));
  i32x8 r = {(int)lo.x, (int)lo.y, (int)lo.z, (int)lo.w, (int)hi.x, (int)hi.y, (int)hi.z, (int)hi.w};
  return r;
}

typedef int i32x2 __attribute__((ext_vector_type(2)));
template <int NWAVES>
struct Half8Stager {
  static constexpr int NINST = 16, PER = NINST / NWAVES;
  static_assert(PER >= 1, "too many waves for this image");
  static __device__ __forceinline__ void load(u32x4 (&r)[PER], const uint16_t* __restrict__ src, int ld, int x0, int k0, int lim, int wave, int lane) {
    const uint8_t* s8 = reinterpret_cast<const uint8_t*>(src);
#pragma unroll
    for (int i = 0; i < PER; ++i) {
      const int row = (wave * PER + i) * 8 + (lane >> 3), c = lane & 7;
      int gx = x0 + c * 16;
      gx = gx < lim ? gx : 0;
      r[i] = *reinterpret_cast<const u32x4*>(s8 + (size_t)(2 * k0 + row) * ld + gx);
    }
  }
  static __device__ __forceinline__ void store(const u32x4 (&r)[PER], char* lds_tile, int wave, int lane, int k_rows_valid = 0x7fffffff) {
#pragma unroll
    for (int i = 0; i < PER; ++i) {
      const int row = (wave * PER + i) * 8 + (lane >> 3), c = lane & 7;
      u32x4 v = r[i];
      if (row >= k_rows_valid) v = u32x4{0u, 0u, 0u, 0u};
      *reinterpret_cast<u32x4*>(lds_tile + row * 128 + ((c ^ (((row >> 1) & 3) << 1)) << 4)) = v;
    }
  }
};
__device__ __forceinline__ i32x8 read_frag8_tr(const char* lds_tile, int xb, int mm, int lane) {
  const int g = lane >> 4, p = lane & 15;
  const int x = xb + 16 * (g & 1) + 8 * (p & 1);
  const int k = mm * 64 + 32 * (g >> 1) + (p >> 1);
  const char* a = lds_tile + k * 128 + ((((x >> 4) ^ (((k >> 1) & 3) << 1)) << 4) | (x & 15));
  const i32x2 r0 = __builtin_amdgcn_ds_read_tr8_b64_v2i32(LDS_PTR(i32x2, a));
  const i32x2 r1 = __builtin_amdgcn_ds_read_tr8_b64_v2i32(LDS_PTR(i32x2, a + 1024));
  const i32x2 r2 = __builtin_amdgcn_ds_read_tr8_b64_v2i32(LDS_PTR(i32x2, a + 2048));
  const i32x2 r3 = __builtin_amdgcn_ds_read_tr8_b64_v2i32(LDS_PTR(i32x2, a + 3072));
  i32x8 r = {r0[0], r0[1], r1[0], r1[1], r2[0], r2[1], r3[0], r3[1]};
  return r;
}

__device__ __forceinline__ void tile_coords(int lid, int tiles_m, int tiles_n, int& tm, int& tn) {
  const int GROUP_M = 8;
  const int per_group = GROUP_M * tiles_n;
  const int gidx = lid / per_group;
  const int first_m = gidx * GROUP_M;
  const int gsz = min(tiles_m - first_m, GROUP_M);
  const int in_g = lid - gidx * per_group;
  tm = first_m + in_g % gsz;
  tn = in_g / gsz;
}


template <int WM, int WN, int WNW, int KG, bool PLAIN, int F8>
__device__ __forceinline__ void gemm_epilogue(f32x16 (&acc)[WM / 32][WN / 32], const Problem& P, char* smem, int m0, int n0, int split,
                                              int kg, int wave, int lane, int tid) {
  constexpr int NWAVES = 2 * WNW, NTHREADS = 64 * NWAVES * KG, AI = WM / 32, NJ = WN / 32;
  const int wr = wave / WNW, wc = wave % WNW;
  const int M = P.M, N = P.N;
  EpiArgs E = P.epi;
  const bool is_split = P.nsplit > 1;
  const long long split_stride = P.split_stride;
  {
    float bj[NJ];
#pragma unroll
    for (int j = 0; j < NJ; ++j) {
      const int n = n0 + wc * WN + j * 32 + (lane & 31);
      bj[j] = (E.bias && !is_split && n < N) ? E.bias[n] : 0.0f;
// ... 53 lines not shown
```

multilingual-image-captioning_amd/csrc/gemm_w4.hip:

```cpp
#include "gemm_common.h"
#ifdef MIC_TRACE_BLOCKS
__device__ unsigned long long* mic_trace_buf;
#define MIC_TRACE(SLOT) do { if (threadIdx.x == 0) mic_trace_buf[5 * blockIdx.x + (SLOT)] = wall_clock64(); } while (0)
#define MIC_TRACE_ID() do { if (threadIdx.x == 0) { unsigned hw_, xcc_; asm volatile("s_getreg_b32 %0, hwreg(HW_REG_HW_ID)" : "=s"(hw_)); \
  asm volatile("s_getreg_b32 %0, hwreg(HW_REG_XCC_ID)" : "=s"(xcc_)); mic_trace_buf[5 * blockIdx.x + 4] = ((unsigned long long)(xcc_ & 0xf) << 16) | (hw_ & 0xffff); } } while (0)
#else
#define MIC_TRACE(SLOT) do { } while (0)
#define MIC_TRACE_ID() do { } while (0)
#endif

namespace {

constexpr int W4_BK = 64, W4_HIMG = 128 * W4_BK * 2, W4_SLOT = 4 * W4_HIMG;

__device__ __forceinline__ uint32_t w4_source(int ld, int x0, int lim, int q, int lane) {
  const int R = q * 8 + (lane >> 3), c = (lane & 7) ^ ((R >> 1) & 7);
  int gx = x0 + R;
  gx = gx < lim ? gx : lim - 1;
  return ((uint32_t)gx * (uint32_t)ld + (uint32_t)(c * 8)) * 2u;
}

constexpr int W4_EP = 132;
template <bool STATS, bool LNF>
__device__ __forceinline__ void w4_epilogue_lean(f32x16 (&acc)[4][4], const Problem& P, char* smem, int mw, int nw, int wave, int lane) {
  const EpiArgs& E = P.epi;
  const int M = P.M, N = P.N;
  {
    const float alpha = E.alpha;
    float bj[4];
#pragma unroll
    for (int j = 0; j < 4; ++j) {
      const int n = nw + j * 32 + (lane & 31);
      bj[j] = (E.bias && n < N) ? E.bias[n] : 0.0f;
    }
#pragma unroll
    for (int i = 0; i < 4; ++i)
#pragma unroll
      for (int j = 0; j < 4; ++j)
#pragma unroll
        for (int r = 0; r < 16; ++r) acc[i][j][r] = acc[i][j][r] * alpha + bj[j];
  }
  float* Cw = reinterpret_cast<float*>(smem) + wave * (32 * W4_EP);
  uint16_t* C = (uint16_t*)E.C;
  const int ldc = E.ldc;
  const int urow = lane >> 4, c8 = (lane & 15) * 8;
  const int n = nw + c8;
  const bool nfull = n + 8 <= N;
  float2* lnr = reinterpret_cast<float2*>(smem + 4 * 32 * W4_EP * 4) + wave * 128;
  float g8[8], b8[8];
  if constexpr (LNF) {
#pragma unroll
    for (int k = 0; k < 2; ++k) {
      const int m = mw + lane + 64 * k;
      float mu = 0.0f, rstd = 0.0f;
      if (m < M) {
        const longlong2 st = reinterpret_cast<const longlong2*>(E.ln_stats)[m];
        mu = (float)st.x * (MIC_ROWSUM_INV_SCALE * E.ln_inv_d);
        rstd = rsqrtf(fmaxf((float)st.y * (MIC_ROWSUM_INV_SCALE * E.ln_inv_d) - mu * mu, 0.0f) + E.ln_eps);
      }
      lnr[lane + 64 * k] = make_float2(mu, rstd);
    }
#pragma unroll
    for (int i = 0; i < 8; ++i) g8[i] = b8[i] = 0.0f;
    if (nfull) { ld8(E.ln_g + n, g8); ld8(E.ln_bias + n, b8); }
  }
  const bool stat_all = STATS && nw + 128 <= E.stat_nvalid;
#pragma unroll
  for (int p = 0; p < 4; ++p) {
#pragma unroll
    for (int j = 0; j < 4; ++j)
#pragma unroll
      for (int r = 0; r < 16; ++r) Cw[((r & 3) + 8 * (r >> 2) + 4 * (lane >> 5)) * W4_EP + j * 32 + (lane & 31)] = acc[p][j][r];
#pragma unroll
    for (int it = 0; it < 8; ++it) {
      const int row = it * 4 + urow;
      const int m = mw + p * 32 + row;
      const float* src = Cw + row * W4_EP + c8;
      const float4 lo = *reinterpret_cast<const float4*>(src);
      const float4 hi = *reinterpret_cast<const float4*>(src + 4);
      float v[8] = {lo.x, lo.y, lo.z, lo.w, hi.x, hi.y, hi.z, hi.w};
      const bool ok = m < M && n < N;
      if constexpr (LNF) {
        const float2 mr = lnr[p * 32 + row];
        if (nfull) {
#pragma unroll
          for (int i = 0; i < 8; ++i) v[i] = fmaf(mr.y, v[i] - mr.x * g8[i], b8[i]);
        }
      }
      uint4 u;
      u.x = f2bf_pk(v[0], v[1]); u.y = f2bf_pk(v[2], v[3]);
      u.z = f2bf_pk(v[4], v[5]); u.w = f2bf_pk(v[6], v[7]);
      if (ok) {
        if (nfull) *reinterpret_cast<uint4*>(C + (size_t)m * ldc + n) = u;
        else
          for (int i = 0; i < N - n; ++i) C[(size_t)m * ldc + n + i] = f2bf(v[i]);
      }
      if constexpr (STATS) {
        const uint32_t w[4] = {u.x, u.y, u.z, u.w};
        float gm, sm;
        granule_stat8(w, stat_all ? 8 : (ok ? E.stat_nvalid - n : 0), gm, sm);
        if ((lane & 7) == 0 && ok) reinterpret_cast<float2*>(E.rowstat)[(size_t)m * E.stat_ld + n / 64] = make_float2(gm, sm);
      }
    }
  }
}

__device__ __forceinline__ void w4_epilogue_f32(f32x16 (&acc)[4][4], const Problem& P, char* smem, int mw, int nw, int split, int wave, int lane) {
  const EpiArgs& E = P.epi;
  const int M = P.M, N = P.N;
  {
    const float alpha = E.alpha;
    float bj[4];
#pragma unroll
    for (int j = 0; j < 4; ++j) {
      const int n = nw + j * 32 + (lane & 31);
      bj[j] = (E.bias && n < N) ? E.bias[n] : 0.0f;
    }
#pragma unroll
    for (int i = 0; i < 4; ++i)
#pragma unroll
      for (int j = 0; j < 4; ++j)
#pragma unroll
        for (int r = 0; r < 16; ++r) acc[i][j][r] = acc[i][j][r] * alpha + bj[j];
  }
  float* Cw = reinterpret_cast<float*>(smem) + wave * (32 * W4_EP);
  float* C = (float*)E.C + (size_t)split * (size_t)P.split_stride;
  const int ldc = E.ldc;
  const int urow = lane >> 5, c4 = (lane & 31) * 4;
  const int n = nw + c4;
  const bool nfull = n + 4 <= N && (ldc & 3) == 0;
#pragma unroll
  for (int p = 0; p < 4; ++p) {
#pragma unroll
    for (int j = 0; j < 4; ++j)
#pragma unroll
      for (int r = 0; r < 16; ++r) Cw[((r & 3) + 8 * (r >> 2) + 4 * (lane >> 5)) * W4_EP + j * 32 + (lane & 31)] = acc[p][j][r];
#pragma unroll
    for (int it = 0; it < 16; ++it) {
      const int row = it * 2 + urow;
      const int m = mw + p * 32 + row;
      const float4 v = *reinterpret_cast<const float4*>(Cw + row * W4_EP + c4);
      if (m < M && n < N) {
        float* dst = C + (size_t)m * ldc + n;
        if (nfull) *reinterpret_cast<float4*>(dst) = v;
        else {
          const float x[4] = {v.x, v.y, v.z, v.w};
          for (int i = 0; i < N - n && i < 4; ++i) dst[i] = x[i];
        }
      }
    }
  }
}

template <int EPI>
__global__ __launch_bounds__(256) void gemm_w4_kernel(LaunchTable tab) {
  constexpr int WM = 128, WN = 128, WNW = 2, AI = 4, NJ = 4, BM = 256, BN = 256;
  extern __shared__ __attribute__((aligned(16))) char smem[];
  const int tid = threadIdx.x, lane = tid & 63, wave = __builtin_amdgcn_readfirstlane(tid >> 6);
  int lid;
  {
    const int bid = blockIdx.x, nwg = tab.total_blocks;
    const int xcd = bid & 7, q = nwg >> 3, r = nwg & 7;
    lid = (xcd < r ? xcd * (q + 1) : r * (q + 1) + (xcd - r) * q) + (bid >> 3);
  }
  const Problem& P = tab.p[0];
  MIC_TRACE(0);
  MIC_TRACE_ID();
  int tile = lid, split = 0;
  if (P.nsplit > 1) {
    const int T = P.tiles_m * P.tiles_n;
    if ((P.nsplit & 7) == 0) {
      const int S = P.nsplit >> 3, j = blockIdx.x >> 3;
      split = (blockIdx.x & 7) * S + j / T;
      tile = j % T;
    } else {
      split = lid / T;
      tile = lid - split * T;
    }
  }
  int tm, tn;
  tile_coords(tile, P.tiles_m, P.tiles_n, tm, tn);
  const int m0 = tm * BM, n0 = tn * BN;
  const int wr = wave >> 1, wc = wave & 1;

  f32x16 acc[AI][NJ];
#pragma unroll
  for (int i = 0; i < AI; ++i)
#pragma unroll
    for (int j = 0; j < NJ; ++j)
#pragma unroll
      for (int r = 0; r < 16; ++r) acc[i][j][r] = 0.0f;

  const int nk_total = P.K / 64;
  const int nk_per = ((nk_total + P.nsplit - 1) / P.nsplit + 1) & ~1;
  const int kt0 = min(nk_total, split * nk_per), kt1 = min(nk_total, kt0 + nk_per);
  const int nsteps = 2 * max(kt1 - kt0, 0);

  uint32_t go[16];
#pragma unroll
  for (int h = 0; h < 4; ++h)
#pragma unroll
    for (int i = 0; i < 4; ++i)
      go[h * 4 + i] = h < 2 ? w4_source(P.lda, m0 + h * 128, P.M, wave * 4 + i, lane) : w4_source(P.ldb, n0 + (h - 2) * 128, P.N, wave * 4 + i, lane);
  const __amdgpu_buffer_rsrc_t rA = __builtin_amdgcn_make_buffer_rsrc((void*)(reinterpret_cast<const char*>(P.A) + (size_t)kt0 * 128), 0, 0x7fffffff, 0x00020000);
  const __amdgpu_buffer_rsrc_t rB = __builtin_amdgcn_make_buffer_rsrc((void*)(reinterpret_cast<const char*>(P.B) + (size_t)kt0 * 128), 0, 0x7fffffff, 0x00020000);
  const int nk = nsteps / 2;
  bf16x8 fa[AI][4], fb[NJ][4];
  const char* fa_ = smem + wr * W4_HIMG;
  const char* fb_ = smem + (2 + wc) * W4_HIMG;
  const __amdgpu_buffer_rsrc_t rZ = __builtin_amdgcn_make_buffer_rsrc((void*)P.A, 0, 0, 0x00020000);
#define W4_DMA(TILE, SLOT, Q)                                                                                                  \
  __builtin_amdgcn_raw_ptr_buffer_load_lds((TILE) < nk ? ((Q) < 8 ? rA : rB) : rZ,                                             \
                                           LDS_PTR(void, smem + (SLOT) * W4_SLOT + ((Q) >> 2) * W4_HIMG + (wave * 4 + ((Q) & 3)) * 1024), \
                                           16, go[Q], (TILE) * 128, 0, 0)
#define W4_BARRIER()                       \
  do {                                     \
    __builtin_amdgcn_sched_barrier(0);     \
    __builtin_amdgcn_s_barrier();          \
    __builtin_amdgcn_sched_barrier(0);     \
  } while (0)
#define W4_TILE(C)                                                                                                             \
  do {                                                                                                                         \
    _Pragma("unroll") for (int g_ = 0; g_ < 64; ++g_) {                                                                        \
      if (g_ == 16) {                                                                                                          \
        asm volatile("s_waitcnt vmcnt(0) lgkmcnt(0)" ::: "memory");                                                            \
        W4_BARRIER();                                                                                                          \
      }                                                                                                                        \
      acc[(g_ & 15) >> 2][g_ & 3] = __builtin_amdgcn_mfma_f32_32x32x16_bf16(fa[(g_ & 15) >> 2][g_ >> 4], fb[g_ & 3][g_ >> 4],  \
                                                                           acc[(g_ & 15) >> 2][g_ & 3], 0, 0, 0);             \
      const int q_ = g_ >> 4, x_ = g_ & 15;                                                                                    \
      const int rk_ = (q_ + 3) & 3, rs_ = q_ == 0 ? (C) : 1 - (C);            \
      if (x_ < 4) fa[x_][rk_] = read_frag<false, W4_BK, 128>(fa_ + rs_ * W4_SLOT, x_ * 32, rk_, lane);                         \
      else if (x_ < 8) fb[x_ - 4][rk_] = read_frag<false, W4_BK, 128>(fb_ + rs_ * W4_SLOT, (x_ - 4) * 32, rk_, lane);          \
      if ((q_ == 1 || q_ == 2) && (x_ & 1) == 1) W4_DMA(t + (C) + 2, C, (q_ - 1) * 8 + (x_ >> 1));                             \
      __builtin_amdgcn_sched_barrier(0);                                                                                       \
    }                                                                                                                          \
  } while (0)

  const bool live = m0 + wr * WM < P.M;
  if (nk >= 2) {
#pragma unroll
    for (int q = 0; q < 16; ++q) W4_DMA(0, 0, q);
#pragma unroll
    for (int q = 0; q < 16; ++q) W4_DMA(1, 1, q);
    asm volatile("s_waitcnt vmcnt(16)" ::: "memory");
    W4_BARRIER();
    MIC_TRACE(1);
#pragma unroll
    for (int kk = 0; kk < 3; ++kk)
#pragma unroll
      for (int x = 0; x < 4; ++x) {
        fa[x][kk] = read_frag<false, W4_BK, 128>(fa_, x * 32, kk, lane);
        fb[x][kk] = read_frag<false, W4_BK, 128>(fb_, x * 32, kk, lane);
      }
    __builtin_amdgcn_sched_barrier(0);
    if (live) {
      for (int t = 0; t < nk; t += 2) {
        W4_TILE(0);
        W4_TILE(1);
      }
    } else {
      for (int t = 0; t < nk; ++t) {
        asm volatile("s_waitcnt vmcnt(0)" ::: "memory");
        W4_BARRIER();
#pragma unroll
        for (int q = 0; q < 16; ++q) W4_DMA(t + 2, t & 1, q);
      }
    }
    asm volatile("s_waitcnt vmcnt(0)" ::: "memory");
  }
  __syncthreads();
  MIC_TRACE(2);
  if (live) {
    if constexpr (EPI == 8) w4_epilogue_f32(acc, P, smem, m0 + wr * WM, n0 + wc * WN, split, wave, lane);
    else w4_epilogue_lean<(EPI & 1) != 0, (EPI & 4) != 0>(acc, P, smem, m0 + wr * WM, n0 + wc * WN, wave, lane);
  }
#ifdef MIC_TRACE_BLOCKS
  asm volatile("s_waitcnt vmcnt(0)" ::: "memory");
#endif
  MIC_TRACE(3);
}

template <int EPI>
void launch_w4(const LaunchTable& tab, hipStream_t s) {
  constexpr int lds = 2 * W4_SLOT;
  static bool attr_set_dev[64] = {};
  int dev_ = 0;
  (void)hipGetDevice(&dev_);
  bool& attr_set = attr_set_dev[dev_ & 63];
  if (!attr_set) {
    hipFuncSetAttribute(reinterpret_cast<const void*>(&gemm_w4_kernel<EPI>), hipFuncAttributeMaxDynamicSharedMemorySize, lds);
    attr_set = true;
  }
  hipLaunchKernelGGL((gemm_w4_kernel<EPI>), dim3(tab.total_blocks), dim3(256), lds, s, tab);
}

}

bool gemm_w4_takes(const LaunchTable& tab) {
  if (tab.count != 1) return false;
  const Problem& p = tab.p[0];
  const EpiArgs& e = p.epi;
  const long long lim = 0x7fffffffLL;
  if ((long long)p.M * p.lda * 2 >= lim || (long long)p.N * p.ldb * 2 >= lim) return false;
  if (p.K < 256 || p.K % 128 != 0 || e.R || e.drop_thr || e.rowsum2 || e.act || e.Zout || e.dact || e.accumulate) return false;
  if (((uintptr_t)e.C & 15) != 0) return false;
  if (e.c_f32)
    return !e.rowstat && !e.ln_stats && (p.nsplit == 1 || p.split_stride > 0) && p.K / 64 / p.nsplit >= 2;
  return p.nsplit == 1 && (e.ldc & 7) == 0 && (!e.ln_stats || p.N % 8 == 0);
}
void launch_gemm_w4(const LaunchTable& tab, hipStream_t s) {
  const EpiArgs& e = tab.p[0].epi;
  if (e.c_f32) { launch_w4<8>(tab, s); return; }
  const int epi = 2 + (e.rowstat ? 1 : 0) + (e.ln_stats ? 4 : 0);
  switch (epi) {
    case 2: launch_w4<2>(tab, s); break;
    case 3: launch_w4<3>(tab, s); break;
    case 6: launch_w4<6>(tab, s); break;
    default: launch_w4<7>(tab, s); break;
  }
}
```

multilingual-image-captioning_amd/engine.py:

```python
from __future__ import annotations

import math
from typing import Dict, Optional

import torch

from . import _lib as L
from . import ops
from .params import ParamStore, _rup

ROWPAD = 128


def _mix(seed: int, site: int) -> int:
    x = (seed * 0x9E3779B1 + site * 0x85EBCA6B + 0x27D4EB2F) & 0xFFFFFFFF
    x ^= x >> 15
    x = (x * 0x2C1B3C6D) & 0xFFFFFFFF
    x ^= x >> 12
    return x & 0xFFFFFFFF


class Engine:
    def __init__(self, store: ParamStore):
        self.P = store
        self.dt = store.dtype
        self.dev = store.device
        self._bufs: Dict[str, torch.Tensor] = {}
        mc = store.cfg.mbart_config
        self.gelu = L.ACT_IDS[getattr(mc, "gelu_variant", "tanh")]
        self.dec_eps = float(getattr(mc, "decoder_ln_eps", 1e-6))
        self.vit_eps = float(store.cfg.clip_vision_config.layer_norm_eps)
        self.p_drop = float(mc.dropout)
        self.embed_scale = math.sqrt(store.d) if mc.scale_embedding else 1.0
        self.defer_embed = False
        self.embed_rows = None
        self._dw_queue = []
        self._cs_queue = []
        self.on_free = []
        self.fp8 = False
        import os
        self.use_head_stats = os.environ.get("MIC_HEAD_STATS", "1") != "0"
        self.grad_progress = None
        self.on_embed_rows = None
        self.dw_overlap = self.dev.type == "cuda" and os.environ.get("MIC_DW_OVERLAP", "1") != "0"
        self.decode_ln_fold = self.dev.type == "cuda" and os.environ.get("MIC_DECODE_LNFOLD", "1") != "0"
        self._ckv_hoist = os.environ.get("MIC_CKV_HOIST", "1") != "0"
        self._lnf = {}
        self._lnf_version = -1
        self._dw_stream = None
        import os as _os
        self.head_nt = _os.environ.get("MIC_HEAD_NT", "1") != "0"
        self.ln_partials = _os.environ.get("MIC_LN_PARTIALS", "1") != "0"
        self._lnp_queue = []
        self._head_nt_state = None
        self.fp8_head = 0
        self._head8_state = None
        self._head_x8 = None
        self._ET_version, self._ET_event = -1, None
        self._dw_events = []
        self.dw_every = int(os.environ.get("MIC_DW_EVERY", "0"))
        self.dw_late_flush = os.environ.get("MIC_DW_LATE_FLUSH", "1") != "0"
        self._dw_side = False
        self._ckv_block_name = None

    FP8_KINDS = ("qkv", "cq", "ckv", "fc1", "fc2")

    def set_gemm_dtype(self, name, scaling: str = "delayed", head: Optional[str] = None):
        if name in (None, "bf16", "bfloat16", "f32", "float32"):
            self.fp8 = False
            return
        if name != "fp8":
            raise ValueError(f"unknown gemm_dtype {name!r}")
        if scaling not in ("delayed", "current"):
            raise ValueError(f"fp8 scaling must be 'delayed' or 'current', got {scaling!r}")
        if self.dt != torch.bfloat16:
            raise ValueError("gemm_dtype='fp8' needs the bfloat16 storage mode (dtype=bfloat16)")
        import os as _os
        P = self.P
        self.fp8 = True
        self.fp8_scaling = scaling
        kinds = tuple(k for k in self.FP8_KINDS if not (k == "ckv" and self._ckv_hoist))
        names = [f"dec{l}.{k}" for l in range(P.L) for k in kinds] + [f"vit{l}.{k}" for l in range(P.vL) for k in ("qkv", "fc1", "fc2")]
        if self._ckv_hoist:
            names.append("ckvcat")
        mode = head if head is not None else _os.environ.get("MIC_FP8_HEAD", "all")
        if mode not in ("0", "bwd", "all"):
            raise ValueError(f"MIC_FP8_HEAD / head={mode!r}: 0 | bwd | all")
        self.fp8_head = {"0": 0, "bwd": 1, "all": 2}[mode] if (P.d % 128 == 0 and P.Vpad % 128 == 0) else 0
        if self.fp8_head:
            names.append("shared")
        self._head8_state = None
        self._head_x8 = None
        self._w8 = {}
        self._w8_state = torch.zeros((len(names), 2), dtype=torch.float32, device=self.dev)
        for i, n in enumerate(names):
            N, K = self._w8_src(n).shape
            self._w8[n] = (torch.empty((N, K), dtype=torch.float8_e4m3fn, device=self.dev),
                           torch.empty((K, N), dtype=torch.float8_e4m3fn, device=self.dev),
                           self._w8_state[i])
        self._w8_stale = True
        self._w8_part = torch.zeros((len(names), ops.fp8_amax_partials()), dtype=torch.float32, device=self.dev) if scaling == "delayed" else None
        self._w8_seen = False
        self._w8_fresh = set()
        self._w8_requant_opt = _os.environ.get("MIC_FP8_REQUANT_OPT", "0") == "1"
        self._w8_async = _os.environ.get("MIC_FP8_W8_ASYNC", "1") != "0"
        self._w8_event = None
        self._w8_rolled = False
        self._w8_index = {n: i for i, n in enumerate(names)}
        segs = P.segs
        def span(n):
            if n == "ckvcat":
                return segs["dec0.ckv.w"].offset, segs[f"dec{P.L - 1}.ckv.w"].offset + segs[f"dec{P.L - 1}.ckv.w"].numel
            sg = segs["shared" if n == "shared" else n + ".w"]
            return sg.offset, sg.offset + sg.numel
        self._w8_span = {n: span(n) for n in names}
        self._a8_state = torch.zeros((1024, 2), dtype=torch.float32, device=self.dev)
        self._a8_part = torch.zeros((1024, ops.fp8_amax_partials()), dtype=torch.float32, device=self.dev) if scaling == "delayed" else None
        self._a8_slots: Dict[str, int] = {}
        self._a8_ready = set()
        self._a8_cache: Dict = {}
        self._dw8_queue = []
        self._cs8_queue = []
        self._x8: Dict[str, tuple] = {}
        self.fp8_fused = scaling == "delayed" and self.ln_partials and _os.environ.get("MIC_FP8_FUSED", "1") != "0"

    def _w8_src(self, name: str):
        if name == "shared":
            return self.P.w("shared")
        return self.P.ckv_cat("w")[0] if name == "ckvcat" else self.P.w(name + ".w")

    def storage_dtype_gemms(self):
        import contextlib

        @contextlib.contextmanager
        def ctx():
            keep = self.fp8
            self.fp8 = False
            try:
                yield
            finally:
                self.fp8 = keep
        return ctx()

    def fp8_weights_changed(self, by_optimizer: bool = False):
        self._w8_stale = True
        if not by_optimizer:
            self._w8_seen = False
            self._w8_fresh = set()

    def _w8_items_all(self):
        key = (self.P.lp.data_ptr(), id(self._w8))
        if getattr(self, "_w8_items_key", None) != key:
            self._w8_items = [ops.fp8_item(self._w8_src(n), q.shape[0], q.shape[1], st, torch.float8_e4m3fn, q=q, qT=qT,
                                           amax_next=self._w8_part[i]) for i, (n, (q, qT, st)) in enumerate(self._w8.items())]
            self._w8_items_key = key
        return self._w8_items

    def fp8_refresh_weights(self, side, upto: Optional[int] = None, wait_event=None):
        if not (self.fp8 and self.fp8_scaling == "delayed" and self._w8_seen and self._w8_async):
            return
        items = self._w8_items_all()
        names = list(self._w8)
        if upto is not None:
            todo = [i for i, n in enumerate(names) if self._w8_span[n][1] <= upto and n not in self._w8_fresh]
            if not todo:
                return
            with torch.cuda.stream(side):
                if wait_event is not None:
                    side.wait_event(wait_event)
                with ops.pinned_stream():
                    if not self._w8_rolled:
                        ops.fp8_roll_amax(self._w8_state, self._w8_part, len(names))
                        self._w8_rolled = True
                    ops.fp8_quantize([items[i] for i in todo], amax_pass=False)
            self._w8_fresh.update(names[i] for i in todo)
            return
        if not self._w8_stale:
            return
        todo = [i for i, n in enumerate(names) if n not in self._w8_fresh]
        ev = torch.cuda.Event()
        ev.record(torch.cuda.current_stream())
        with torch.cuda.stream(side):
            side.wait_event(ev)
            with ops.pinned_stream():
                if not self._w8_rolled:
                    ops.fp8_roll_amax(self._w8_state, self._w8_part, len(names))
                if todo:
                    ops.fp8_quantize([items[i] for i in todo], amax_pass=False)
            done = torch.cuda.Event()
            done.record(side)
        self._w8_event, self._w8_stale, self._w8_fresh, self._w8_rolled = done, False, set(), False

    def _w8_wait(self):
        if self._w8_event is not None:
            torch.cuda.current_stream().wait_event(self._w8_event)
            self._w8_event = None

    def fp8_requantize_range(self, b: int, e: int):
        if not (self.fp8 and self.fp8_scaling == "delayed" and self._w8_seen and self._w8_requant_opt):
            return
        todo = [n for n, (o, oe) in self._w8_span.items() if b < oe <= e and n not in self._w8_fresh and n != "shared"]
        if not todo:
            return
        items = []
        for n in todo:
            q, qT, st = self._w8[n]
            items.append(ops.fp8_item(self._w8_src(n), q.shape[0], q.shape[1], st, torch.float8_e4m3fn, q=q, qT=qT,
                                      amax_next=self._w8_part[self._w8_index[n]]))
        ops.fp8_quantize(items, amax_pass=False)
        self._w8_fresh.update(todo)

    def _fp8_begin_pass(self):
        if not self.fp8:
            return
        if self._w8_stale and self.fp8_scaling == "delayed" and self._w8_seen and len(self._w8_fresh) == len(self._w8):
            ops.fp8_roll_amax(self._w8_state, self._w8_part, len(self._w8))
            self._w8_stale = False
        self._w8_fresh = set()
        if self._w8_stale:
            P = self.P
            delayed = self.fp8_scaling == "delayed"
            if delayed and self._w8_seen:
                ops.fp8_roll_amax(self._w8_state, self._w8_part, len(self._w8))
            else:
                ops.zero(self._w8_state)
                if delayed:
                    ops.zero(self._w8_part)
            self._w8_wait()
            items = self._w8_items_all() if delayed else [ops.fp8_item(self._w8_src(n), q.shape[0], q.shape[1], st, torch.float8_e4m3fn, q=q, qT=qT)
                                                          for (n, (q, qT, st)) in self._w8.items()]
            ops.fp8_quantize(items, amax_pass=not (delayed and self._w8_seen))
            self._w8_seen = delayed
            self._w8_stale = False
        n = len(self._a8_slots)
        if self.fp8_scaling == "delayed":
            if n:
                ops.fp8_roll_amax(self._a8_state, self._a8_part, n)
            self._a8_ready = set(self._a8_slots)
        else:
            ops.zero(self._a8_state[: max(n, 1)])
        self._a8_cache = {}
        self._x8 = {}
        self._head_x8 = None

    def _fp8_ok(self, wname: str) -> bool:
        return self.fp8 and wname.split(".")[-1] in self.FP8_KINDS and wname in self._w8

    def _a8_slot(self, tag: str) -> int:
        i = self._a8_slots.get(tag)
        if i is None:
            i = self._a8_slots[tag] = len(self._a8_slots)
            if i >= self._a8_state.shape[0]:
                raise RuntimeError("fp8: out of activation scale slots")
        return i

    def _quant(self, x, rows: int, cols: int, tag: str, buf_tag: str, fmt, cache: bool = False):
        key = (x.data_ptr(), rows, cols, fmt)
        hit = self._a8_cache.get(key) if cache else None
        if hit is not None:
            return hit
        cap = max(int(x.shape[0]), _rup(rows, ROWPAD))
        q = self.buf(buf_tag + ".q8", cap, cols, fmt)
        slot = self._a8_slot(tag)
        st = self._a8_state[slot]
        delayed = self.fp8_scaling == "delayed"
        item = ops.fp8_item(x, rows, cols, st, fmt, q=q, amax_next=self._a8_part[slot] if delayed else None)
        ops.fp8_quantize([item], amax_pass=not (delayed and tag in self._a8_ready))
        if cache:
            self._a8_cache[key] = (q, st)
        return q, st

    def _q8_target(self, tag: str, buf_tag: str, rows_cap: int, cols: int, fmt):
        if not (self.fp8 and self.fp8_fused and tag in self._a8_ready):
            return None
        slot = self._a8_slot(tag)
        st, part = self._a8_state[slot], self._a8_part[slot]
        q = self.buf(buf_tag + ".q8", rows_cap, cols, fmt)
        return q, st, ops.fp8_out(q, st, part), (st, part)

    def ln_x8(self, x, ln: str, eps: float, a_name: str, cap: int, mean, rstd, rows: int, wname: str, q_tag: str, **kw):
        P = self.P
        width = x.shape[-1]
        t = self._q8_target(wname + ".x", q_tag + wname.split(".")[-1] + ".x", cap, width, torch.float8_e4m3fn) if self._fp8_ok(wname) else None
        if t is not None:
            ops.layernorm_fwd(x, P.f32(ln + ".g"), P.f32(ln + ".b"), eps, None, mean, rstd, rows=rows, q8=t[2], **kw)
            return None, (t[0], t[1])
        a = self.buf(a_name, cap, width)
        ops.layernorm_fwd(x, P.f32(ln + ".g"), P.f32(ln + ".b"), eps, a, mean, rstd, rows=rows, **kw)
        return a, None

    def _done(self, seg_name: str):
        if self.grad_progress is not None:
            if self._dw_events and not self._dw_side:
                torch.cuda.current_stream().wait_event(self._dw_events[-1])
            s = self.P.segs[seg_name]
            self.grad_progress(s.offset + s.numel)

    def buf(self, name: str, rows: int, cols: int, dtype=None) -> torch.Tensor:
        dtype = dtype or self.dt
        key = (name, rows, cols, dtype)
        t = self._bufs.get(key)
        if t is None:
            t = torch.zeros((_rup(max(rows, 1), ROWPAD), cols), dtype=dtype, device=self.dev)
            self._bufs[key] = t
        return t

    def vec(self, name: str, n: int, dtype=torch.float32) -> torch.Tensor:
        key = (name, n, dtype)
        t = self._bufs.get(key)
        if t is None:
            t = torch.zeros(n, dtype=dtype, device=self.dev)
            self._bufs[key] = t
        return t

    def free_buffers(self):
        for cb in list(self.on_free):
            cb()
        self._bufs.clear()
        self._ET_version, self._ET_event, self._head_nt_state = -1, None, None
        self._lnf = {}
        self._lnf_version = -1

    def linear(self, x, wname, out, M, *, act=0, zout=None, residual=None, drop_seed=None, bias=True, save_tag=None, fp8=True,
               stable_input=False, x8=None, out8=None):
        P = self.P
        w = P.w(wname + ".w")
        N, K = w.shape
        p = self.p_drop if drop_seed is not None else 0.0
        if fp8 and self._fp8_ok(wname):
            self._w8_wait()
            wq, _, ws = self._w8[wname]
            if x8 is None:
                x8 = self._quant(x, M, K, wname + ".x", (save_tag or "f8.") + wname.split(".")[-1] + ".x", torch.float8_e4m3fn,
                                 cache=stable_input)
            if save_tag is not None:
                self._x8[wname] = x8
            kw = dict(bias=P.f32(wname + ".b") if bias else None, act=act, zout=zout, residual=residual, dropout_p=p, dropout_seed=drop_seed or 0,
                      a_scale_inv=x8[1][1:], b_scale_inv=ws[1:])
            if out8 is not None:
                ops.gemm(x8[0], wq, out8[0], M, N, K, c_q8=out8[3], **kw)
                return out8[0], out8[1]
            return ops.gemm(x8[0], wq, out, M, N, K, **kw)
        return ops.gemm(x, w, out, M, N, K, bias=P.f32(wname + ".b") if bias else None, act=act, zout=zout,
                        residual=residual, dropout_p=p, dropout_seed=drop_seed or 0)

    def linear_bwd(self, wname, x, dy, M, *, dx=None, zin=None, dact=0, dx_accumulate=False, bias=True, defer=False, x_tag=True,
                   dy8=None, dx8=None, par=0):
        P = self.P
        w = P.w(wname + ".w")
        N, K = w.shape
        Mp = _rup(M, ROWPAD)
        if self._fp8_ok(wname) and x_tag is not None:
            kind = wname.split(".")[0].rstrip("0123456789") + "." + wname.split(".")[-1]
            if dy8 is None:
                dy8 = self._quant(dy, M, N, wname + ".dy", f"f8.{kind}.dy.{par}", torch.float8_e5m2)
            x8 = self._x8.get(wname)
            if x8 is None:
                raise RuntimeError(f"fp8 backward of {wname}: the forward pass did not keep the fp8 copy of its input (save_tag missing)")
            _, wqT, ws = self._w8[wname]
            ga = ops.gemm_args(dy8[0], x8[0], P.g(wname + ".w"), N, K, Mp, a_kmajor=True, b_kmajor=True, k_valid=M,
                               a_scale_inv=dy8[1][1:], b_scale_inv=x8[1][1:])
            cs = (dy8[0], P.g(wname + ".b"), dy8[1][1:], M, N) if bias else None
            if defer:
                self._dw8_queue.append((ga, wname, bias))
                if cs is not None:
                    self._cs8_queue.append(cs)
            else:
                ops.gemm_grouped([ga])
                if cs is not None:
                    ops.colsum_q8_grouped([cs])
            if dx8 is not None:
                ops.gemm(dy8[0], wqT, dx8[0], M, K, N, zin=zin, dact=dact, a_scale_inv=dy8[1][1:], b_scale_inv=ws[1:], c_q8=dx8[3])
            elif dx is not None:
                ops.gemm(dy8[0], wqT, dx, M, K, N, zin=zin, dact=dact, accumulate=dx_accumulate, a_scale_inv=dy8[1][1:], b_scale_inv=ws[1:])
            if not defer:
                self._done(wname + ".w")
            return dx
        fuse = bias and self.dt == torch.bfloat16
        rs = dict(a_rowsum=P.g(wname + ".b"), rowsum_k=M) if fuse else {}
        if self.dt == torch.bfloat16:
            rs["k_valid"] = M
        if defer:
            self._dw_queue.append((ops.gemm_args(dy, x, P.g(wname + ".w"), N, K, Mp, a_kmajor=True, b_kmajor=True, **rs), wname, bias))
        else:
            ops.gemm(dy, x, P.g(wname + ".w"), N, K, Mp, a_kmajor=True, b_kmajor=True, **rs)
        if bias and not fuse:
            if defer:
                self._cs_queue.append((dy, P.g(wname + ".b"), M, N, dy.stride(0)))
            else:
                ops.colsum(dy, P.g(wname + ".b"), M, N, dy.stride(0), accumulate=True)
        if dx is not None:
            ops.gemm(dy, w, dx, M, K, N, b_kmajor=True, zin=zin, dact=dact, accumulate=dx_accumulate)
        if not defer:
            self._done(wname + ".w")
        return dx

    def dy8_target(self, wname: str, par: int, cap: int):
        if not self._fp8_ok(wname):
            return None
        kind = wname.split(".")[0].rstrip("0123456789") + "." + wname.split(".")[-1]
        return self._q8_target(wname + ".dy", f"f8.{kind}.dy.{par}", cap, self.P.w(wname + ".w").shape[0], torch.float8_e5m2)

    def ln_folded(self, wname: str, ln: str):
        P = self.P
        ver = getattr(P, "version", 0)
        if ver != self._lnf_version:
            self._lnf_fresh = set()
            self._lnf_version = ver
        hit = self._lnf.get(wname)
        if hit is None:
            w = P.w(wname + ".w")
            hit = self._lnf[wname] = (torch.empty_like(w), torch.empty(w.shape[0], dtype=torch.float32, device=self.dev),
                                      torch.empty(w.shape[0], dtype=torch.float32, device=self.dev))
        if wname not in self._lnf_fresh:
            ops.ln_fold_weight(P.w(wname + ".w"), P.f32(ln + ".g"), P.f32(ln + ".b"), P.f32(wname + ".b"), *hit)
            self._lnf_fresh.add(wname)
        return hit

    def dyb(self, name: str, l: int, rows: int, cols: int) -> torch.Tensor:
        return self.buf(f"{name}.{self._par(l)}" if self._dw_on() else name, rows, cols)

    def ln_bwd(self, tag: str, l: int, x, ln: str, mean, rstd, dy, dx, rows: int, **kw):
        P = self.P
        if not self.ln_partials:
            return ops.layernorm_bwd(x, P.f32(ln + ".g"), mean, rstd, dy, dx, P.g(ln + ".g"), P.g(ln + ".b"), rows=rows, **kw)
        width = x.shape[-1]
        part = self.buf(f"lnp.{tag}.{self._par(l)}", 2 * ops.layernorm_bwd_blocks(1 << 30), width, torch.float32)
        ops.layernorm_bwd_partials(x, P.f32(ln + ".g"), mean, rstd, dy, dx, part, rows=rows, **kw)
        self._lnp_queue.append((part, ops.layernorm_bwd_blocks(rows), width, P.g(ln + ".g"), P.g(ln + ".b"), False))
        return dx

    def _dw_on(self) -> bool:
        return self.dw_overlap

    def _par(self, l: int) -> int:
        return l % (2 * self._dw_every_now())

    def _dw_every_now(self) -> int:
        if not self._dw_on():
            return 1
        return self.dw_every if self.dw_every > 0 else (2 if self.fp8 else 1)

    def _dw_flush_layer(self, l: int) -> bool:
        return l % self._dw_every_now() == 0

    def dw_fence(self) -> bool:
        if not (self._dw_on() and self.dw_late_flush):
            return False
        if self._dw_events:
            torch.cuda.current_stream().wait_event(self._dw_events[-1])
        return True

    def flush_dw(self, fence: bool = True):
        if not (self._cs_queue or self._dw_queue or self._lnp_queue or (self.fp8 and (self._dw8_queue or self._cs8_queue))):
            return
        side = None
        if self._dw_on():
            if self._dw_stream is None:
                import os

                n = int(os.environ.get("MIC_DW_CUS", "0"))
                self._dw_stream = ops.cu_masked_stream(256 - n, n, self.dev) if n > 0 else ops.role_stream(self.dev, "dw")
            side = self._dw_stream
            ev = torch.cuda.Event()
            ev.record(torch.cuda.current_stream())
            side.wait_event(ev)
        import contextlib

        with (torch.cuda.stream(side) if side is not None else contextlib.nullcontext()):
            with (ops.pinned_stream() if side is not None else contextlib.nullcontext()):
                self._dw_side = side is not None
                try:
# ... 128 lines not shown
            if flush_now and not late:
                self.flush_dw()
            dx = self.dyb("vb.dx", l - 1, Mv, vd)
            dx8t = self.dy8_target(f"vit{l - 1}.fc2", self._par(l - 1), Mv) if l > 0 else None
            if dx8t is not None:
                self.ln_bwd("v1", l, x_in, p + "ln1", st1[0], st1[1], da, dx, Mv, dres=dxm, q8=dx8t[2], q8_of_dx=True)
                dx8 = (dx8t[0], dx8t[1])
            else:
                self.ln_bwd("v1", l, x_in, p + "ln1", st1[0], st1[1], da, dx, Mv, dres=dxm)
                dx8 = None
            if flush_now and late:
                self.flush_dw(fence=False)
        emb = self.buf("v.emb", Mv, vd)
        st = self.buf("v.pre.stats", 2, _rup(Mv, ROWPAD), torch.float32)
        demb = self.buf("vb.demb", Mv, vd)
        self.ln_bwd("vpre", 0, emb, "vit.pre_ln", st[0], st[1], dx, demb, Mv)
        dpe = self.buf("vb.dpe", Mp, vd)
        ops.vit_assemble_bwd(demb, dpe, P.g("vit.cls"), P.g("vit.pos"), B, S, vd, vd)
        pk = P.ps * P.ps * 3
        patches = self.buf("v.patches", Mp, pk)
        ops.gemm(dpe, patches, P.g("patch.w"), vd, pk, _rup(Mp, ROWPAD), a_kmajor=True, b_kmajor=True)
        self._done("patch.w")

    def decoder_forward(self, ids, pos_ids, key_mask, ehs, B: int, T: int, save: bool, seed: Optional[int], pack=None):
        P = self.P
        d, f, H, S = P.d, P.ffn, P.H, P.S
        Mcap, Mv = B * T, B * S
        M = pack[2] if pack is not None else Mcap
        drop = seed is not None and self.p_drop > 0

        def sd(site):
            return _mix(seed, site) if drop else None

        h0 = self.buf("d.h0", Mcap, d)
        ops.embed_fwd(ids, pos_ids, P.w("shared"), P.f32("dec.pos"), self.embed_scale, h0, M, d)
        x = self.buf("d.x0", Mcap, d)
        ste = self.buf("d.emb.stats", 2, _rup(Mcap, ROWPAD), torch.float32)
        ops.layernorm_fwd(h0, P.f32("dec.ln_emb.g"), P.f32("dec.ln_emb.b"), self.dec_eps, x, ste[0], ste[1], rows=M,
                          dropout_p=self.p_drop if drop else 0.0, dropout_seed=sd(1) or 0)
        kvcat = self.cross_kv_all(ehs, Mv, "d." if save else "d_.", save) if self.ckv_hoisted() else None
        for l in range(P.L):
            tag = f"d{l}." if save else "d_."
            p = f"dec{l}."
            stats = self.buf(tag + "stats", 6, _rup(Mcap, ROWPAD), torch.float32)
            a, a8 = self.ln_x8(x, p + "ln_sa", self.dec_eps, tag + "a_sa", Mcap, stats[0], stats[1], M, p + "qkv", tag)
            qkv = self.buf(tag + "qkv", Mcap, 3 * d)
            self.linear(a, p + "qkv", qkv, M, save_tag=tag if save else None, x8=a8)
            ctx = self.buf(tag + "ctx", Mcap, d)
            lse = self.vec(tag + "lse", B * H * T)
            if pack is not None:
                ops.attn_fwd_packed(qkv, qkv[:, d:], qkv[:, 2 * d:], ctx, B, H, T, T, pack[0], pack[1], kv_packed=True, ldq=3 * d, ldk=3 * d,
                                    ldv=3 * d, ldo=d, causal=True, lse=lse)
            else:
                ops.attn_fwd(qkv, qkv[:, d:], qkv[:, 2 * d:], ctx, B, H, T, T, ldq=3 * d, ldk=3 * d, ldv=3 * d, ldo=d, key_mask=key_mask,
                             causal=True, lse=lse)
            x1 = self.buf(tag + "x1", Mcap, d)
            self.linear(ctx, p + "so", x1, M, residual=x, drop_seed=sd(10 + 3 * l))
            a, a8 = self.ln_x8(x1, p + "ln_ca", self.dec_eps, tag + "a_ca", Mcap, stats[2], stats[3], M, p + "cq", tag)
            q = self.buf(tag + "cq", Mcap, d)
            self.linear(a, p + "cq", q, M, save_tag=tag if save else None, x8=a8)
            if kvcat is not None:
                kv, ldkv = kvcat[:, l * 2 * d:], kvcat.stride(0)
            else:
                kv, ldkv = self.buf(tag + "ckv", Mv, 2 * d), 2 * d
                self.linear(ehs, p + "ckv", kv, Mv, save_tag="d.ehs." if save else None, stable_input=True)
            cctx = self.buf(tag + "cctx", Mcap, d)
            clse = self.vec(tag + "clse", B * H * T)
            if pack is not None:
                ops.attn_fwd_packed(q, kv, kv[:, d:], cctx, B, H, T, S, pack[0], pack[1], kv_packed=False, ldq=d, ldk=ldkv, ldv=ldkv, ldo=d,
                                    lse=clse)
            else:
                ops.attn_fwd(q, kv, kv[:, d:], cctx, B, H, T, S, ldq=d, ldk=ldkv, ldv=ldkv, ldo=d, lse=clse)
            x2 = self.buf(tag + "x2", Mcap, d)
            self.linear(cctx, p + "co", x2, M, residual=x1, drop_seed=sd(11 + 3 * l))
            a, a8 = self.ln_x8(x2, p + "ln_ff", self.dec_eps, tag + "a_ff", Mcap, stats[4], stats[5], M, p + "fc1", tag)
            z = self.buf(tag + "z", Mcap, f)
            u8t = self._q8_target(p + "fc2.x", tag + "fc2.x", Mcap, f, torch.float8_e4m3fn) if self._fp8_ok(p + "fc2") else None
            u = self.buf(tag + "u", Mcap, f) if u8t is None else None
            u8 = self.linear(a, p + "fc1", u, M, act=self.gelu, zout=z, save_tag=tag if save else None, x8=a8, out8=u8t)
            x3 = self.buf(f"d{l}.x3" if save else f"d_.x3{l & 1}", Mcap, d)
            self.linear(u, p + "fc2", x3, M, residual=x2, drop_seed=sd(12 + 3 * l), save_tag=tag if save else None,
                        x8=u8 if u8t is not None else None)
            x = x3
        hf = self.buf("d.hf", Mcap, d)
        stf = self.buf("d.f.stats", 2, _rup(Mcap, ROWPAD), torch.float32)
        ops.layernorm_fwd(x, P.f32("dec.ln_f.g"), P.f32("dec.ln_f.b"), self.dec_eps, hf, stf[0], stf[1], rows=M)
        return hf

    def ckv_hoisted(self) -> bool:
        return self._ckv_hoist

    def cross_kv_all(self, ehs, Mv: int, tag: str, save: bool = False):
        P = self.P
        w, b = P.ckv_cat("w")
        kvcat = self.buf(tag + "ckvcat", Mv, P.L * 2 * P.d)
        if self.fp8 and "ckvcat" in self._w8:
            self._w8_wait()
            wq, _, ws = self._w8["ckvcat"]
            x8 = self._quant(ehs, Mv, P.d, "ckvcat.x", tag + "ckvcat.x", torch.float8_e4m3fn)
            if save:
                self._x8["ckvcat"] = x8
            ops.gemm(x8[0], wq, kvcat, Mv, P.L * 2 * P.d, P.d, bias=b, a_scale_inv=x8[1][1:], b_scale_inv=ws[1:])
        else:
            ops.gemm(ehs, w, kvcat, Mv, P.L * 2 * P.d, P.d, bias=b)
        return kvcat

    def head_logits(self, hf, M: int, name: str = "d.logits", stats: bool = False, fp8: bool = False):
        P = self.P
        logits = self.buf(name, M, P.Vpad)
        stat = self.head_stats(name, M) if stats else None
        self._head_project(hf, logits, M, stat, fp8=fp8)
        return (logits, stat) if stats else logits

    def _head8(self) -> bool:
        return self.fp8 and self.fp8_head > 0

    def _head_project(self, hf, logits, M: int, stat, fp8: bool = True):
        P = self.P
        if fp8 and self._head8() and self.fp8_head == 2:
            x8 = self._head_x8 = self._quant(hf, M, P.d, "head.x", "head.x", torch.float8_e4m3fn)
            E8, _, wst = self._w8["shared"]
            self._w8_wait()
            ops.gemm(x8[0], E8, logits, M, P.Vpad, P.d, bias=P.f32("flb"), rowstat=stat, rowstat_nvalid=P.V,
                     a_scale_inv=x8[1][1:], b_scale_inv=wst[1:])
        else:
            ops.gemm(hf, P.w("shared"), logits, M, P.Vpad, P.d, bias=P.f32("flb"), rowstat=stat, rowstat_nvalid=P.V)

    def head_stats(self, name: str, M: int):
        if self.dt != torch.bfloat16 or not self.use_head_stats:
            return None
        return self.buf(name + ".stat", M, 2 * (self.P.Vpad // 64), torch.float32)

    def decoder_backward(self, B: int, T: int, ids, pos_ids, key_mask, ehs, dlogits, seed: Optional[int], rows=None, pack=None):
        P = self.P
        d, f, H, S = P.d, P.ffn, P.H, P.S
        Mcap, Mv = B * T, B * S
        M = pack[2] if pack is not None else Mcap
        drop = seed is not None and self.p_drop > 0
        pd = self.p_drop if drop else 0.0

        def sd(site):
            return _mix(seed, site) if drop else 0

        dhf = self.buf("db.dhf", Mcap, d)
        if rows is None:
            hf = self.buf("d.hf", Mcap, d)
            Mh = M
        else:
            hf = self.buf("d.hf" if pack is not None else "d.hfc", Mcap, d)
            Mh = rows[1]
        Mhp = _rup(Mh, 64)
        nt = self._head_nt_state
        self._head_nt_state = None
        h8s, self._head8_state = self._head8_state, None
        if h8s is not None:
            x8 = self._head_x8 or self._quant(hf, Mh, d, "head.x", "head.x", torch.float8_e4m3fn)
            ops.gemm(h8s[0], x8[0], P.g("shared"), P.Vpad, d, _rup(Mh, 128), a_kmajor=True, b_kmajor=True, k_valid=Mh,
                     a_scale_inv=h8s[1][1:], b_scale_inv=x8[1][1:])
            tiles = ((Mh + 255) // 256) * ((d + 255) // 256)
            nsp = max(1, min(ops.get_cu_budget() // tiles, P.Vpad // 128 // 2))
            slab_rows = _rup(Mh, 256)
            cap_rows = max(_rup(Mcap, 256), (256 // max(1, (d + 255) // 256)) * 256) + _rup(Mcap, 256)
            d32 = self.buf("db.dhf32", cap_rows, d, torch.float32)
            assert (nsp + 1) * slab_rows <= d32.shape[0], (nsp, slab_rows, d32.shape)
            ops.head_label_terms(h8s[3], h8s[2], P.w("shared"), hf, d32[nsp * slab_rows:], P.g("shared"), Mh, d)
        elif nt is not None:
            dT, Kp = nt
            hfT = self.buf("d.hfT", d, dT.shape[1])
            ops.transpose_bf16(hf, hfT, Mh, d, rows_pad=Kp)
            ops.gemm(dT, hfT, P.g("shared"), P.Vpad, d, Kp)
        elif self.dt == torch.bfloat16:
            ops.zero(P.g("flb"))
            ops.gemm(dlogits, hf, P.g("shared"), P.Vpad, d, Mhp, a_kmajor=True, b_kmajor=True, a_rowsum=P.g("flb"), rowsum_k=Mh)
        else:
            ops.colsum(dlogits, P.g("flb"), Mh, P.Vpad, dlogits.stride(0))
            ops.gemm(dlogits, hf, P.g("shared"), P.Vpad, d, Mhp, a_kmajor=True, b_kmajor=True)
        self._done("shared")
        dhc = dhf if (rows is None or pack is not None) else self.buf("db.dhfc", Mcap, d)
        if h8s is not None:
            _, ET8, wst = self._w8["shared"]
            self._w8_wait()
            slab = slab_rows * d
            ops.gemm(h8s[0], ET8, d32, Mh, d, P.Vpad, split_k=nsp, split_stride=slab if nsp > 1 else 0, a_scale_inv=h8s[1][1:], b_scale_inv=wst[1:])
            ops.sum_slabs(d32, nsp + 1, slab, dhc, Mh, d, d32.stride(0), dhc.stride(0))
        elif nt is not None:
            tiles = ((Mh + 255) // 256) * ((d + 255) // 256)
            nsp = max(1, min(ops.get_cu_budget() // tiles, P.Vpad // 128 // 2))
            slab_rows = _rup(Mh, 256)
            cap_rows = max(_rup(Mcap, 256), (256 // max(1, (d + 255) // 256)) * 256)
            d32 = self.buf("db.dhf32", cap_rows, d, torch.float32)
            assert nsp * slab_rows <= d32.shape[0], (nsp, slab_rows, d32.shape)
            slab = slab_rows * d
            ops.gemm(dlogits, self.shared_T(), d32, Mh, d, P.Vpad, split_k=nsp, split_stride=slab if nsp > 1 else 0)
            if nsp > 1:
                ops.sum_slabs(d32, nsp, slab, dhc, Mh, d, d32.stride(0), dhc.stride(0))
            else:
                ops.cast2d(d32, dhc, Mh, d, d32.stride(0), dhc.stride(0))
        elif self.dt == torch.bfloat16 and P.Vpad >= 16384:
            nsp = 32
            d32 = self.buf("db.dhf32", nsp * _rup(Mcap, ROWPAD), d, torch.float32)
            slab = _rup(Mcap, ROWPAD) * d
            ops.gemm(dlogits, P.w("shared"), d32, Mh, d, P.Vpad, b_kmajor=True, split_k=nsp, split_stride=slab)
            ops.sum_slabs(d32, nsp, slab, dhc, Mh, d, d32.stride(0), dhc.stride(0))
        else:
            ops.gemm(dlogits, P.w("shared"), dhc, Mh, d, P.Vpad, b_kmajor=True)
        if rows is not None and pack is None:
            ops.zero(dhf[:M])
            ops.copy_rows(dhc, dhf, Mh, d, dst_idx=rows[0])
        dx = self.buf("db.dx", Mcap, d)
        stf = self.buf("d.f.stats", 2, _rup(Mcap, ROWPAD), torch.float32)
        x_last = self.buf(f"d{P.L - 1}.x3", Mcap, d)
        dxm8t = self.dy8_target(f"dec{P.L - 1}.fc2", self._par(P.L - 1), Mcap)
        dxm = self.dyb("db.dxm_a", P.L - 1, Mcap, d) if dxm8t is None else None
        self.ln_bwd("f", 0, x_last, "dec.ln_f", stf[0], stf[1], dhf, dx, M, dxm=dxm, dropout_p=pd, dropout_seed=sd(12 + 3 * (P.L - 1)),
                    **({} if dxm8t is None else dict(q8=dxm8t[2])))
        dxm8 = None if dxm8t is None else (dxm8t[0], dxm8t[1])
        f8 = self.fp8
        dehs = self.buf("db.dehs", Mv, d)
        hoist = self.ckv_hoisted()
        kvcat = self.buf("d.ckvcat", Mv, P.L * 2 * d) if hoist else None
        hoist8 = hoist and self.fp8 and "ckvcat" in self._w8
        dkvcat8t = self._q8_target("ckvcat.dy", "f8.ckvcat.dy", Mv, P.L * 2 * d, torch.float8_e5m2) if (hoist8 and T <= 64 and S <= 64) else None
        dkvcat = self.buf("db.dkvcat", Mv, P.L * 2 * d) if (hoist and dkvcat8t is None) else None
        for l in reversed(range(P.L)):
            tag, p = f"d{l}.", f"dec{l}."
            stats = self.buf(tag + "stats", 6, _rup(Mcap, ROWPAD), torch.float32)
            qkv, ctx, x1 = (self.buf(tag + n, Mcap, c) for n, c in (("qkv", 3 * d), ("ctx", d), ("x1", d)))
            cq, cctx, x2 = (self.buf(tag + n, Mcap, d) for n in ("cq", "cctx", "x2"))
            ckv, ldkv = (kvcat[:, l * 2 * d:], kvcat.stride(0)) if hoist else (self.buf(tag + "ckv", Mv, 2 * d), 2 * d)
            z = self.buf(tag + "z", Mcap, f)
            a_sa, a_ca, a_ff, u = (None,) * 4 if f8 else (self.buf(tag + "a_sa", Mcap, d), self.buf(tag + "a_ca", Mcap, d),
                                                          self.buf(tag + "a_ff", Mcap, d), self.buf(tag + "u", Mcap, f))
            lse, clse = self.vec(tag + "lse", B * H * T), self.vec(tag + "clse", B * H * T)
            x_in = self.buf(f"d{l - 1}.x3", Mcap, d) if l > 0 else self.buf("d.x0", Mcap, d)
            dxm_b, dxm_c = self.dyb("db.dxm_b", l, Mcap, d), self.dyb("db.dxm_c", l, Mcap, d)
            dz8t = self.dy8_target(p + "fc1", self._par(l), Mcap)
            dz = self.dyb("db.dz", l, Mcap, f) if dz8t is None else None
            self.linear_bwd(p + "fc2", u, dxm, M, dx=dz, zin=z, dact=self.gelu, defer=True, dy8=dxm8, dx8=dz8t, par=self._par(l))
            da = self.buf("db.da", Mcap, d)
            self.linear_bwd(p + "fc1", a_ff, dz, M, dx=da, defer=True, dy8=None if dz8t is None else (dz8t[0], dz8t[1]), par=self._par(l))
            dx2 = self.buf("db.dx2", Mcap, d)
            self.ln_bwd("ff", l, x2, p + "ln_ff", stats[4], stats[5], da, dx2, M,
                        dres=dx, dxm=dxm_b, dropout_p=pd, dropout_seed=sd(11 + 3 * l))
            dctx = self.buf("db.dctx", Mcap, d)
            self.linear_bwd(p + "co", cctx, dxm_b, M, dx=dctx, defer=True)
            one_tile = T <= 64 and S <= 64
            dq8t = self.dy8_target(p + "cq", self._par(l), Mcap) if one_tile else None
            if hoist:
                kv8 = None if dkvcat8t is None else dkvcat8t[0][:, l * 2 * d:]
                dkv8t = None if kv8 is None else (kv8, dkvcat8t[1], ops.fp8_out(kv8, dkvcat8t[1], dkvcat8t[3][1]))
            else:
                dkv8t = self.dy8_target(p + "ckv", self._par(l), Mv) if one_tile else None
            if dq8t is not None and dkv8t is not None:
                ops.attn_bwd_q8(cq, ckv, ckv[:, d:], cctx, dctx, clse, dq8t[2], dkv8t[2], dkv8t[0][:, d:], B, H, T, S, ldq=d, ldk=ldkv, ldv=ldkv,
                                ldo=d, lddo=d, q_off=pack[0] if pack is not None else None, q_len=pack[1] if pack is not None else None, kv_packed=False)
                self.linear_bwd(p + "cq", a_ca, None, M, dx=da, defer=True, dy8=(dq8t[0], dq8t[1]), par=self._par(l))
                if not hoist:
                    self.linear_bwd(p + "ckv", ehs, None, Mv, dx=dehs, dx_accumulate=(l != P.L - 1), defer=True, dy8=(dkv8t[0], dkv8t[1]), par=self._par(l))
            elif hoist and dkvcat8t is not None:
                raise RuntimeError("fp8: cross-attention dQ without a scale history beside a hoisted k/v gradient with one")
            else:
                dq = self.dyb("db.dq", l, Mcap, d)
                dkv = dkvcat[:, l * 2 * d:] if hoist else self.dyb("db.dkv", l, Mv, 2 * d)
                if pack is not None:
                    ops.attn_bwd_packed(cq, ckv, ckv[:, d:], cctx, dctx, clse, dq, dkv, dkv[:, d:], B, H, T, S, pack[0], pack[1], kv_packed=False,
                                        ldq=d, ldk=ldkv, ldv=ldkv, ldo=d, lddo=d, lddq=d, lddk=ldkv, lddv=ldkv)
                else:
                    ops.attn_bwd(cq, ckv, ckv[:, d:], cctx, dctx, clse, dq, dkv, dkv[:, d:], B, H, T, S, ldq=d, ldk=ldkv, ldv=ldkv, ldo=d,
                                 lddo=d, lddq=d, lddk=ldkv, lddv=ldkv)
                self.linear_bwd(p + "cq", a_ca, dq, M, dx=da, defer=True, par=self._par(l))
                if not hoist:
                    self.linear_bwd(p + "ckv", ehs, dkv, Mv, dx=dehs, dx_accumulate=(l != P.L - 1), defer=True, par=self._par(l))
            dx1 = self.buf("db.dx1", Mcap, d)
            self.ln_bwd("ca", l, x1, p + "ln_ca", stats[2], stats[3], da, dx1, M,
                        dres=dx2, dxm=dxm_c, dropout_p=pd, dropout_seed=sd(10 + 3 * l))
            self.linear_bwd(p + "so", ctx, dxm_c, M, dx=dctx, defer=True)
            dqkv8t = self.dy8_target(p + "qkv", self._par(l), Mcap) if T <= 64 else None
            if dqkv8t is not None:
                q8 = dqkv8t[0]
                ops.attn_bwd_q8(qkv, qkv[:, d:], qkv[:, 2 * d:], ctx, dctx, lse, dqkv8t[2], ops.fp8_out(q8[:, d:], dqkv8t[1], dqkv8t[3][1]), q8[:, 2 * d:],
                                B, H, T, T, ldq=3 * d, ldk=3 * d, ldv=3 * d, ldo=d, lddo=d, q_off=pack[0] if pack is not None else None,
                                q_len=pack[1] if pack is not None else None, kv_packed=pack is not None,
                                key_mask=key_mask if pack is None else None, causal=True)
                self.linear_bwd(p + "qkv", a_sa, None, M, dx=da, defer=True, dy8=(dqkv8t[0], dqkv8t[1]), par=self._par(l))
            else:
                dqkv = self.dyb("db.dqkv", l, Mcap, 3 * d)
                if pack is not None:
                    ops.attn_bwd_packed(qkv, qkv[:, d:], qkv[:, 2 * d:], ctx, dctx, lse, dqkv, dqkv[:, d:], dqkv[:, 2 * d:], B, H, T, T, pack[0],
                                        pack[1], kv_packed=True, ldq=3 * d, ldk=3 * d, ldv=3 * d, ldo=d, lddo=d, lddq=3 * d, lddk=3 * d,
                                        lddv=3 * d, causal=True)
                else:
                    ops.attn_bwd(qkv, qkv[:, d:], qkv[:, 2 * d:], ctx, dctx, lse, dqkv, dqkv[:, d:], dqkv[:, 2 * d:], B, H, T, T, ldq=3 * d,
                                 ldk=3 * d, ldv=3 * d, ldo=d, lddo=d, lddq=3 * d, lddk=3 * d, lddv=3 * d, key_mask=key_mask, causal=True)
                self.linear_bwd(p + "qkv", a_sa, dqkv, M, dx=da, defer=True, par=self._par(l))
            flush_now = self._dw_flush_layer(l)
            late = self.dw_fence() if flush_now else False
            if flush_now and not late:
                self.flush_dw()
            if l > 0:
                dxm8t = self.dy8_target(f"dec{l - 1}.fc2", self._par(l - 1), Mcap)
                dxm = self.dyb("db.dxm_a", l - 1, Mcap, d) if dxm8t is None else None
                self.ln_bwd("sa", l, x_in, p + "ln_sa", stats[0], stats[1], da, dx, M, dres=dx1, dxm=dxm, dropout_p=pd,
                            dropout_seed=sd(12 + 3 * (l - 1)), **({} if dxm8t is None else dict(q8=dxm8t[2])))
                dxm8 = None if dxm8t is None else (dxm8t[0], dxm8t[1])
            else:
                self.ln_bwd("sa", l, x_in, p + "ln_sa", stats[0], stats[1], da, dx, M, dres=dx1)
            if flush_now and late:
                self.flush_dw(fence=False)
        if hoist:
            wcat, _ = P.ckv_cat("w")
            gw, gb = P.ckv_cat("g")
            N = P.L * 2 * d
            Mvp = _rup(Mv, ROWPAD)
            if hoist8:
                dkv8 = (dkvcat8t[0], dkvcat8t[1]) if dkvcat8t is not None else self._quant(dkvcat, Mv, N, "ckvcat.dy", "f8.ckvcat.dy", torch.float8_e5m2)
                x8 = self._x8.get("ckvcat")
                if x8 is None:
                    raise RuntimeError("fp8 backward of the hoisted cross k/v projection: the forward pass did not keep the fp8 encoder states")
                _, wqT, ws = self._w8["ckvcat"]
                nsp = min(8, N // 128)
                if nsp > 1:
                    slab = Mvp * d
                    d32 = self.buf("db.dehs32", nsp * Mvp, d, torch.float32)
                    ops.gemm(dkv8[0], wqT, d32, Mv, d, N, split_k=nsp, split_stride=slab, a_scale_inv=dkv8[1][1:], b_scale_inv=ws[1:])
                    ops.sum_slabs(d32, nsp, slab, dehs, Mv, d, d32.stride(0), dehs.stride(0))
                else:
                    ops.gemm(dkv8[0], wqT, dehs, Mv, d, N, a_scale_inv=dkv8[1][1:], b_scale_inv=ws[1:])
                self._dw8_queue.append((ops.gemm_args(dkv8[0], x8[0], gw, N, d, Mvp, a_kmajor=True, b_kmajor=True, k_valid=Mv,
                                                      a_scale_inv=dkv8[1][1:], b_scale_inv=x8[1][1:]), f"dec{P.L - 1}.ckv", True))
                self._cs8_queue.append((dkv8[0], gb, dkv8[1][1:], Mv, N))
                self._ckv_block_name = f"dec{P.L - 1}.ckv"
                try:
                    self.flush_dw()
                finally:
                    self._ckv_block_name = None
            else:
                fuse = self.dt == torch.bfloat16
                rs = dict(a_rowsum=gb, rowsum_k=Mv) if fuse else {}
                nsp = min(8, N // 64)
                if self.dt == torch.bfloat16 and nsp > 1:
                    slab = Mvp * d
                    d32 = self.buf("db.dehs32", nsp * Mvp, d, torch.float32)
                    ops.gemm(dkvcat, wcat, d32, Mv, d, N, b_kmajor=True, split_k=nsp, split_stride=slab)
                    ops.sum_slabs(d32, nsp, slab, dehs, Mv, d, d32.stride(0), dehs.stride(0))
                else:
                    ops.gemm(dkvcat, wcat, dehs, Mv, d, N, b_kmajor=True)
                self._dw_queue.append((ops.gemm_args(dkvcat, ehs, gw, N, d, Mvp, a_kmajor=True, b_kmajor=True, **rs), f"dec{P.L - 1}.ckv", True))
                if not fuse:
                    self._cs_queue.append((dkvcat, gb, Mv, N, dkvcat.stride(0)))
                self._ckv_block_name = f"dec{P.L - 1}.ckv"
                try:
                    self.flush_dw()
                finally:
                    self._ckv_block_name = None
        else:
            self._done(f"dec{P.L - 1}.ckv.w")
        h0 = self.buf("d.h0", Mcap, d)
        ste = self.buf("d.emb.stats", 2, _rup(Mcap, ROWPAD), torch.float32)
        dh0 = self.buf("db.dh0", Mcap, d)
        self.ln_bwd("emb", 0, h0, "dec.ln_emb", ste[0], ste[1], dx, dh0, M,
                    in_dropout_p=pd, in_dropout_seed=sd(1))
        if self.defer_embed:
            ops.embed_bwd(ids, pos_ids, dh0, self.embed_scale, None, P.g("dec.pos"), M, d)
            n_x = Mcap if pack is not None else M
            ids_x = self.vec("db.ids_x", Mcap, torch.int32)
            ids_x[:n_x].copy_(ids[:n_x])
            if pack is not None:
                if M < Mcap:
                    ids_x[M:Mcap].fill_(-1)
            elif key_mask is not None:
                ids_x[:n_x].masked_fill_(key_mask.reshape(-1)[:n_x] == 0, -1)
            self.embed_rows = (ids_x, dh0, n_x)
        else:
            ops.embed_bwd(ids, pos_ids, dh0, self.embed_scale, P.g("shared"), P.g("dec.pos"), M, d)
            if self.on_embed_rows is not None:
                self.on_embed_rows()
        return dehs

    def loss_and_dlogits(self, logits, labels, mask, M: int, label_smoothing: float, backward: bool, stat=None):
        P = self.P
        lse, rl = self.vec("ce.lse", _rup(M, ROWPAD)), self.vec("ce.rowloss", _rup(M, ROWPAD))
        loss, denom = self.vec("ce.loss", 1), self.vec("ce.denom", 1)
        if stat is not None and label_smoothing == 0.0:
            ops.ce_rows_tiles(logits, logits.stride(0), P.V, stat, labels, lse, rl, M)
        else:
            ops.ce_rows(logits, logits.stride(0), P.V, labels, mask, label_smoothing, lse, rl, M)
        ops.ce_reduce(rl, mask, loss, denom, M)
        if backward and self._head8():
            ops.zero(P.g("flb"))
            q = self.buf("head.dl.q8", logits.shape[0], P.Vpad, torch.float8_e5m2)
            st = self.vec("head.dl.state", 2)
            coef = self.vec("head.dl.coef", _rup(logits.shape[0], ROWPAD))
            ops.ce_bwd_q8(logits, logits.stride(0), P.V, P.Vpad, labels, mask, label_smoothing, lse, denom, M, ops.fp8_out(q, st), colsum=P.g("flb"),
                          label_coef=coef)
            self._head8_state = (q, st, coef, labels)
            self._head_nt_state = None
        elif backward:
            kcap = self._head_nt_kcap(logits)
            if kcap:
                Kp = _rup(M, 128)
                dT = self.buf("d.dlogitsT", P.Vpad, kcap)
                ops.zero(P.g("flb"))
                ops.ce_bwd_t(logits, logits.stride(0), P.V, P.Vpad, labels, mask, label_smoothing, lse, denom, M, dT, rows_pad=Kp, colsum=P.g("flb"))
                self._head_nt_state = (dT, Kp)
            else:
                ops.ce_bwd(logits, logits.stride(0), P.V, P.Vpad, labels, mask, label_smoothing, lse, denom, M)
                self._head_nt_state = None
        return loss

    def _head_nt_kcap(self, logits) -> int:
        P = self.P
        if not self.head_nt or self.dt != torch.bfloat16 or P.Vpad < 16384 or P.d % 128 != 0 or self._head8():
            return 0
        kcap = _rup(logits.shape[0], 128)
        return kcap if P.Vpad * kcap * 2 < 0x7fffffff and logits.shape[0] * logits.stride(0) * 2 < 0x7fffffff else 0

    def shared_T(self):
        P = self.P
        ET = self.buf("w.sharedT", P.d, P.Vpad)
        ver = getattr(P, "version", 0)
        if self._ET_version != ver:
            if self._ET_event is not None:
                torch.cuda.current_stream().wait_event(self._ET_event)
            ops.transpose_bf16(P.w("shared"), ET, P.Vpad, P.d)
            self._ET_version, self._ET_event = ver, None
        elif self._ET_event is not None:
            torch.cuda.current_stream().wait_event(self._ET_event)
            self._ET_event = None
        return ET

    def refresh_shared_T(self, side, version: int):
        P = self.P
        ET = self._bufs.get(("w.sharedT", P.d, P.Vpad, self.dt))
        if not self.head_nt or self.dt != torch.bfloat16 or ET is None or self._head8():
            return
        ev = torch.cuda.Event()
        ev.record(torch.cuda.current_stream())
        with torch.cuda.stream(side):
            side.wait_event(ev)
            with ops.pinned_stream():
                ops.transpose_bf16(P.w("shared"), ET, P.Vpad, P.d)
            done = torch.cuda.Event()
            done.record(side)
        self._ET_version, self._ET_event = version, done

    def forward_logits(self, pixels, ids, pos_ids, key_mask, B, T, *, save=False, seed=None, trunc_int32=False, stats=False):
        self._fp8_begin_pass()
        _, ehs = self.vit_forward(pixels, save, trunc_int32)
        hf = self.decoder_forward(ids, pos_ids, key_mask, ehs, B, T, save, seed)
        if stats:
            logits, stat = self.head_logits(hf, B * T, stats=True, fp8=True)
            return logits, ehs, stat
        return self.head_logits(hf, B * T, fp8=True), ehs

    def compact_head(self, hf, M: int, rows, packed: bool = False):
        P = self.P
        idx, Mc = rows
        Mcp = _rup(Mc, 64)
        if packed:
            hfc = hf
        else:
            hfc = self.buf("d.hfc", M, P.d)
            ops.copy_rows(hf, hfc, Mc, P.d, src_idx=idx)
        if Mcp > Mc:
            ops.zero(hfc[Mc:Mcp])
        logits = self.buf("d.logits", M, P.Vpad)
        stat = self.head_stats("d.logits", M)
        self._head_project(hfc, logits, Mc, stat)
        if Mcp > Mc:
            ops.zero(logits[Mc:Mcp])
        return logits, stat

    def loss_only(self, pixels, ids, pos_ids, key_mask, labels, B, T, *, label_smoothing=0.0, rows=None, row_labels=None, pack=None):
        M = B * T
        pack = self._check_pack(pack, rows, T)
        if rows is None:
            logits, _, stat = self.forward_logits(pixels, ids, pos_ids, key_mask, B, T, save=False, seed=None, stats=True)
            return self.loss_and_dlogits(logits, labels, key_mask.reshape(-1), M, label_smoothing, backward=False, stat=stat)
        self._fp8_begin_pass()
        _, ehs = self.vit_forward(pixels, False)
        hf = self.decoder_forward(ids, pos_ids, key_mask, ehs, B, T, False, None, pack=pack)
        logits, stat = self.compact_head(hf, M, rows, packed=pack is not None)
        return self.loss_and_dlogits(logits, row_labels, self.ones_i32(rows[1]), rows[1], label_smoothing, backward=False, stat=stat)

    def _check_pack(self, pack, rows, T: int):
        if pack is None:
            return None
        if rows is None or rows[1] != pack[2]:
            raise ValueError("packed decoder rows go with the compacted LM head on the same rows (rows=(idx, n) with n == pack rows)")
        if self.dt != torch.bfloat16 or T > 64 or self.P.S > 64:
            raise ValueError("packed decoder rows: bfloat16 storage mode, seq_len <= 64 and at most 64 encoder positions")
        return pack

    def ones_i32(self, n: int):
        t = self._bufs.get("ones_i32")
        if t is None or t.numel() < n:
            t = torch.ones(max(_rup(max(n, 1), 4096), 2 * (t.numel() if t is not None else 0)), dtype=torch.int32, device=self.dev)
            self._bufs["ones_i32"] = t
        return t[:n]

    def loss_and_grads(self, pixels, ids, pos_ids, key_mask, labels, B, T, *, label_smoothing=0.0, seed=None, rows=None,
                       row_labels=None, pack=None):
        P = self.P
        P.ensure_grads()
        ops.zero(P.grad[P.atomic_begin:])
        M = B * T
        pack = self._check_pack(pack, rows, T)
        if rows is None:
            logits, ehs, stat = self.forward_logits(pixels, ids, pos_ids, key_mask, B, T, save=True, seed=seed, stats=True)
            loss = self.loss_and_dlogits(logits, labels, key_mask.reshape(-1), M, label_smoothing, backward=True, stat=stat)
        else:
            self._fp8_begin_pass()
            _, ehs = self.vit_forward(pixels, True)
            hf = self.decoder_forward(ids, pos_ids, key_mask, ehs, B, T, True, seed, pack=pack)
            logits, stat = self.compact_head(hf, M, rows, packed=pack is not None)
            loss = self.loss_and_dlogits(logits, row_labels, self.ones_i32(rows[1]), rows[1], label_smoothing, backward=True, stat=stat)
        dehs = self.decoder_backward(B, T, ids, pos_ids, key_mask, ehs, logits, seed, rows=rows, pack=pack)
        self.vit_backward(B, dehs)
        self.dw_join()
        return loss
```

multilingual-image-captioning_amd/ops.py:

```python
from __future__ import annotations

import ctypes as C
from typing import Optional

import torch

from . import _lib as L


_FP8 = {torch.float8_e4m3fn: L.MIC_E4M3, torch.float8_e5m2: L.MIC_E5M2}


def _dt(t_or_dtype) -> int:
    d = t_or_dtype.dtype if isinstance(t_or_dtype, torch.Tensor) else t_or_dtype
    if d == torch.bfloat16:
        return L.MIC_BF16
    if d == torch.float32:
        return L.MIC_F32
    if d in _FP8:
        return L.MIC_FP8
    raise L.MicError(f"unsupported dtype {d}")


def _p(t: Optional[torch.Tensor]):
    if t is None:
        return None
    if not t.is_cuda:
        raise L.MicError("libmic_hip ops need device tensors (no CPU fallback)")
    return t.data_ptr()


_STREAM_OVERRIDE = None


def _stream():
    if _STREAM_OVERRIDE is not None:
        return _STREAM_OVERRIDE
    return torch.cuda.current_stream().cuda_stream


class pinned_stream:

    def __enter__(self):
        global _STREAM_OVERRIDE
        self.prev = _STREAM_OVERRIDE
        _STREAM_OVERRIDE = torch.cuda.current_stream().cuda_stream
        return self

    def __exit__(self, *a):
        global _STREAM_OVERRIDE
        _STREAM_OVERRIDE = self.prev


def gemm_args(a: torch.Tensor, b: torch.Tensor, out: torch.Tensor, M: int, N: int, K: int, *, a_kmajor=False, b_kmajor=False,
              bias=None, act=0, zout=None, zin=None, dact=0, residual=None, accumulate=False, dropout_p=0.0, dropout_seed=0,
              alpha=1.0, lda=None, ldb=None, ldc=None, ldz=None, ldr=None, split_k=0, split_stride=0, a_rowsum=None, rowsum_k=0,
              a_scale_inv=None, b_scale_inv=None, rowstat=None, rowstat_nvalid=0, ln_stats=None, ln_colsum=None, ln_width=0,
              ln_eps=0.0, rowsum2=None, k_valid=0, c_q8=None) -> "L.GemmArgs":
    g = L.GemmArgs()
    g.dtype, g.c_dtype = _dt(a), _dt(out)
    if g.dtype == L.MIC_FP8:
        g.a_fmt, g.b_fmt = _FP8[a.dtype], _FP8[b.dtype]
        g.a_scale_inv, g.b_scale_inv = _p(a_scale_inv), _p(b_scale_inv)
    g.M, g.N, g.K = M, N, K
    g.a_kmajor, g.b_kmajor = int(a_kmajor), int(b_kmajor)
    g.A, g.lda = _p(a), lda if lda is not None else a.stride(0)
    g.B, g.ldb = _p(b), ldb if ldb is not None else b.stride(0)
    g.C, g.ldc = _p(out), ldc if ldc is not None else out.stride(0)
    g.bias, g.act = _p(bias), act
    zz = zout if zout is not None else zin
    g.Zout, g.Zin, g.dact = _p(zout), _p(zin), dact
    g.ldz = ldz if ldz is not None else (zz.stride(0) if zz is not None else 0)
    g.R, g.ldr = _p(residual), ldr if ldr is not None else (residual.stride(0) if residual is not None else 0)
    g.accumulate, g.dropout_p, g.dropout_seed, g.alpha = int(accumulate), float(dropout_p), int(dropout_seed) & 0xFFFFFFFF, float(alpha)
    g.split_k, g.split_stride = int(split_k), int(split_stride)
    g.a_rowsum, g.rowsum_k = _p(a_rowsum), int(rowsum_k)
    if rowstat is not None:
        g.rowstat, g.rowstat_ld, g.rowstat_nvalid = _p(rowstat), rowstat.stride(0) // 2, int(rowstat_nvalid)
    if ln_stats is not None:
        g.a_ln_stats, g.a_ln_colsum, g.a_ln_width, g.a_ln_eps = _p(ln_stats), _p(ln_colsum), int(ln_width), float(ln_eps)
    g.rowsum2 = _p(rowsum2)
    g.k_valid = int(k_valid)
    if c_q8 is not None:
        if g.c_dtype != L.MIC_FP8:
            raise L.MicError("c_q8 goes with an fp8 output tensor")
        g.c_q8_state, g.c_q8_amax, g.c_q8_fmt = _p(c_q8[0]), _p(c_q8[1]), _FP8[out.dtype]
    return g


def gemm(a: torch.Tensor, b: torch.Tensor, out: torch.Tensor, M: int, N: int, K: int, **kw):
    g = gemm_args(a, b, out, M, N, K, **kw)
    L.check(L.lib().mic_gemm(C.byref(g), _stream()), "mic_gemm")
    return out


def gemm_grouped(arg_list):
    arr = (L.GemmArgs * len(arg_list))(*arg_list)
    L.check(L.lib().mic_gemm_grouped(arr, len(arg_list), _stream()), "mic_gemm_grouped")


def set_cu_budget(cus: int) -> None:
    L.check(L.lib().mic_set_cu_budget(int(cus)), "mic_set_cu_budget")


def get_cu_budget() -> int:
    return int(L.lib().mic_get_cu_budget())


def gemm_plan(shapes, *, a_kmajor=False, b_kmajor=False, split_k=0, dtype=None) -> dict:
    arr = (L.GemmArgs * len(shapes))()
    for g, (M, N, K) in zip(arr, shapes):
        g.dtype = g.c_dtype = L.MIC_BF16 if dtype is None else dtype
        g.M, g.N, g.K, g.a_kmajor, g.b_kmajor, g.split_k = M, N, K, int(a_kmajor), int(b_kmajor), int(split_k)
    out = L.GemmPlanInfo()
    L.check(L.lib().mic_gemm_plan(arr, len(shapes), C.byref(out)), "mic_gemm_plan")
    return {k: getattr(out, k) for k, _ in L.GemmPlanInfo._fields_}


def comm_emulate(src: torch.Tensor, dst: torch.Tensor, nbytes: int, micros: float, blocks: int):
    L.check(L.lib().mic_comm_emulate(_p(src), _p(dst), int(nbytes), float(micros), int(blocks), _stream()), "mic_comm_emulate")


def ln_fold_weight(w, gamma, beta, bias, w_fold, colsum, bias_fold):
    N, K = w.shape
    L.check(L.lib().mic_ln_fold_weight(_dt(w), N, K, _p(w), w.stride(0), _p(gamma), _p(beta), _p(bias), _p(w_fold), w_fold.stride(0),
                                       _p(colsum), _p(bias_fold), _stream()), "mic_ln_fold_weight")


def fp8_item(src, rows, cols, state, fmt_dtype, q=None, qT=None, rows_pad=0, amax_next=None) -> "L.Fp8Item":
    if src.dtype != torch.bfloat16:
        raise L.MicError("fp8 quantisation reads bf16 tensors (the fp8 path needs the bfloat16 storage mode)")
    it = L.Fp8Item()
    it.src, it.ld, it.rows, it.cols, it.rows_pad = _p(src), src.stride(0), rows, cols, rows_pad
    it.q, it.ldq = _p(q), (q.stride(0) if q is not None else 0)
    it.qT, it.ldqT = _p(qT), (qT.stride(0) if qT is not None else 0)
    it.state, it.amax_next, it.fmt = _p(state), _p(amax_next), _FP8[fmt_dtype]
    return it


def fp8_quantize(items, amax_pass: bool = True):
    arr = (L.Fp8Item * len(items))(*items)
    if amax_pass:
        L.check(L.lib().mic_fp8_amax(arr, len(items), _stream()), "mic_fp8_amax")
    L.check(L.lib().mic_fp8_quantize(arr, len(items), _stream()), "mic_fp8_quantize")


def fp8_amax_partials() -> int:
    return int(L.lib().mic_fp8_amax_partials())


def fp8_roll_amax(state: torch.Tensor, partials: torch.Tensor, count: int):
    L.check(L.lib().mic_fp8_roll_amax(_p(state), state.stride(0), _p(partials), count, _stream()), "mic_fp8_roll_amax")


def fp8_out(q, state, amax_next=None) -> "L.Fp8Out":
    o = L.Fp8Out()
    o.q, o.ldq, o.state, o.amax_next, o.fmt = _p(q), q.stride(0), _p(state), _p(amax_next), _FP8[q.dtype]
    return o


def layernorm_fwd(x, gamma, beta, eps, y, mean=None, rstd=None, rows=None, dropout_p=0.0, dropout_seed=0, q8=None):
    rows = rows if rows is not None else x.shape[0]
    if q8 is not None:
        L.check(L.lib().mic_layernorm_fwd_q8(rows, x.shape[-1], _p(x), _p(gamma), _p(beta), float(eps), _p(y), _p(mean), _p(rstd),
                                             float(dropout_p), int(dropout_seed) & 0xFFFFFFFF, C.byref(q8), _stream()), "mic_layernorm_fwd_q8")
        return y
    L.check(L.lib().mic_layernorm_fwd(_dt(x), rows, x.shape[-1], _p(x), _p(gamma), _p(beta), float(eps), _p(y), _p(mean), _p(rstd),
                                      float(dropout_p), int(dropout_seed) & 0xFFFFFFFF, _stream()), "mic_layernorm_fwd")
    return y


def layernorm_bwd(x, gamma, mean, rstd, dy, dx, dgamma, dbeta, rows=None, dres=None, dxm=None, dropout_p=0.0, dropout_seed=0,
                  in_dropout_p=0.0, in_dropout_seed=0):
    rows = rows if rows is not None else x.shape[0]
    L.check(L.lib().mic_layernorm_bwd(_dt(x), rows, x.shape[-1], _p(x), _p(gamma), _p(mean), _p(rstd), _p(dy), _p(dres), _p(dx),
                                      _p(dgamma), _p(dbeta), _p(dxm), float(dropout_p), int(dropout_seed) & 0xFFFFFFFF,
                                      float(in_dropout_p), int(in_dropout_seed) & 0xFFFFFFFF, _stream()), "mic_layernorm_bwd")
    return dx


def layernorm_bwd_blocks(rows: int) -> int:
    return int(L.lib().mic_layernorm_bwd_blocks(int(rows)))


def layernorm_bwd_partials(x, gamma, mean, rstd, dy, dx, partials, rows=None, dres=None, dxm=None, dropout_p=0.0, dropout_seed=0,
                           in_dropout_p=0.0, in_dropout_seed=0, q8=None, q8_of_dx=False):
    rows = rows if rows is not None else x.shape[0]
    if q8 is not None:
        L.check(L.lib().mic_layernorm_bwd_partials_q8(rows, x.shape[-1], _p(x), _p(gamma), _p(mean), _p(rstd), _p(dy), _p(dres), _p(dx), _p(partials),
                                                      _p(dxm), float(dropout_p), int(dropout_seed) & 0xFFFFFFFF, float(in_dropout_p),
                                                      int(in_dropout_seed) & 0xFFFFFFFF, C.byref(q8), int(bool(q8_of_dx)), _stream()),
                "mic_layernorm_bwd_partials_q8")
        return dx
    L.check(L.lib().mic_layernorm_bwd_partials(_dt(x), rows, x.shape[-1], _p(x), _p(gamma), _p(mean), _p(rstd), _p(dy), _p(dres), _p(dx),
                                               _p(partials), _p(dxm), float(dropout_p), int(dropout_seed) & 0xFFFFFFFF,
                                               float(in_dropout_p), int(in_dropout_seed) & 0xFFFFFFFF, _stream()), "mic_layernorm_bwd_partials")
    return dx


def ln_param_grads(items):
    arr = (L.LnParamItem * len(items))()
    for a, (part, nblk, width, dg, db, acc) in zip(arr, items):
        a.partials, a.dgamma, a.dbeta, a.nblk, a.width, a.accumulate = _p(part), _p(dg), _p(db), int(nblk), int(width), int(bool(acc))
    L.check(L.lib().mic_ln_param_grads(arr, len(items), _stream()), "mic_ln_param_grads")


def attn_fwd(q, k, v, out, B, H, Tq, Tk, *, ldq, ldk, ldv, ldo, key_mask=None, causal=False, lse=None):
    L.check(L.lib().mic_attn_fwd(_dt(q), B, H, Tq, Tk, _p(q), ldq, _p(k), ldk, _p(v), ldv, _p(out), ldo, _p(key_mask), int(causal),
                                 _p(lse), _stream()), "mic_attn_fwd")
    return out


def attn_probs(q, k, out, B, H, Tq, Tk, *, ldq, ldk, key_mask=None, causal=False):
    L.check(L.lib().mic_attn_probs(_dt(q), B, H, Tq, Tk, _p(q), ldq, _p(k), ldk, _p(key_mask), int(causal), _p(out), _stream()), "mic_attn_probs")
    return out


def attn_bwd(q, k, v, out, dout, lse, dq, dk, dv, B, H, Tq, Tk, *, ldq, ldk, ldv, ldo, lddo, lddq, lddk, lddv, key_mask=None,
             causal=False):
    L.check(L.lib().mic_attn_bwd(_dt(q), B, H, Tq, Tk, _p(q), ldq, _p(k), ldk, _p(v), ldv, _p(out), ldo, _p(dout), lddo, _p(lse),
                                 _p(key_mask), int(causal), _p(dq), lddq, _p(dk), lddk, _p(dv), lddv, _stream()), "mic_attn_bwd")


def attn_fwd_packed(q, k, v, out, B, H, Tq_max, Tk, q_off, q_len, *, kv_packed, ldq, ldk, ldv, ldo, causal=False, lse=None):
    L.check(L.lib().mic_attn_fwd_packed(_dt(q), B, H, Tq_max, Tk, _p(q_off), _p(q_len), int(kv_packed), _p(q), ldq, _p(k), ldk, _p(v), ldv,
                                        _p(out), ldo, int(causal), _p(lse), _stream()), "mic_attn_fwd_packed")
    return out


def attn_bwd_packed(q, k, v, out, dout, lse, dq, dk, dv, B, H, Tq_max, Tk, q_off, q_len, *, kv_packed, ldq, ldk, ldv, ldo, lddo, lddq,
                    lddk, lddv, causal=False):
    L.check(L.lib().mic_attn_bwd_packed(_dt(q), B, H, Tq_max, Tk, _p(q_off), _p(q_len), int(kv_packed), _p(q), ldq, _p(k), ldk, _p(v), ldv,
                                        _p(out), ldo, _p(dout), lddo, _p(lse), int(causal), _p(dq), lddq, _p(dk), lddk, _p(dv), lddv,
                                        _stream()), "mic_attn_bwd_packed")


def attn_bwd_q8(q, k, v, out, dout, lse, dq8, dk8, dv8, B, H, Tq, Tk, *, ldq, ldk, ldv, ldo, lddo, q_off=None, q_len=None, kv_packed=False,
                key_mask=None, causal=False):
    L.check(L.lib().mic_attn_bwd_q8(B, H, Tq, Tk, _p(q_off), _p(q_len), int(bool(kv_packed)), _p(q), ldq, _p(k), ldk, _p(v), ldv, _p(out), ldo,
                                    _p(dout), lddo, _p(lse), _p(key_mask), int(causal), C.byref(dq8), C.byref(dk8), _p(dv8), _stream()), "mic_attn_bwd_q8")


def colsum_q8_grouped(items):
    arr = (L.ColsumQ8Item * len(items))()
    for a, (x, out, sinv, rows, cols) in zip(arr, items):
        a.x, a.out, a.scale_inv, a.rows, a.cols, a.ld, a.fmt = _p(x), _p(out), _p(sinv), int(rows), int(cols), x.stride(0), _FP8[x.dtype]
    L.check(L.lib().mic_colsum_q8_grouped(arr, len(items), _stream()), "mic_colsum_q8_grouped")


def attn_decode(q, kc, vc, out, R, H, max_len, cur, *, ldq, ldo, ldc=None, src_row=None, row_div=1):
    ldc = ldc if ldc is not None else H * 64
    L.check(L.lib().mic_attn_decode(_dt(q), R, H, max_len, cur, _p(q), ldq, _p(kc), _p(vc), ldc, _p(src_row), row_div, _p(out), ldo,
                                    _stream()), "mic_attn_decode")
    return out


def kv_append(k, v, kc, vc, R, HD, max_len, cur, *, ldk, ldv):
    L.check(L.lib().mic_kv_append(_dt(k), R, HD, max_len, cur, _p(k), ldk, _p(v), ldv, _p(kc), _p(vc), _stream()), "mic_kv_append")


def im2col(pixels, patches, B, img, ps, ldp, trunc_int32=False):
    L.check(L.lib().mic_im2col(_dt(patches), B, img, ps, _p(pixels), _p(patches), ldp, int(trunc_int32), _stream()), "mic_im2col")


def vit_assemble(patch_out, cls, pos, x, B, S, width, ldp):
    L.check(L.lib().mic_vit_assemble(_dt(x), B, S, width, _p(patch_out), ldp, _p(cls), _p(pos), _p(x), _stream()), "mic_vit_assemble")


def vit_assemble_bwd(dx, dpatch, dcls, dpos, B, S, width, ldp):
    L.check(L.lib().mic_vit_assemble_bwd(_dt(dx), B, S, width, _p(dx), _p(dpatch), ldp, _p(dcls), _p(dpos), _stream()), "mic_vit_assemble_bwd")


def embed_fwd(ids, pos_ids, table, pos_table, scale, h, rows, width):
    L.check(L.lib().mic_embed_fwd(_dt(h), rows, width, _p(ids), _p(pos_ids), _p(table), _p(pos_table), float(scale), _p(h), _stream()), "mic_embed_fwd")


def embed_bwd(ids, pos_ids, dh, scale, dtable, dpos_table, rows, width):
    L.check(L.lib().mic_embed_bwd(_dt(dh), rows, width, _p(ids), _p(pos_ids), _p(dh), float(scale), _p(dtable), _p(dpos_table), _stream()), "mic_embed_bwd")


def embed_rows_add_det_workspace(vocab: int, device) -> torch.Tensor:
    n = int(L.lib().mic_embed_rows_add_det_ws(int(vocab)))
    ws = torch.zeros(n, dtype=torch.int32, device=device)
    ws[:vocab] = 0x7FFFFFFF
    ws[2 * vocab: 3 * vocab] = -1
    return ws


def embed_rows_add_det(ids, dh, scale, dtable, n, width, ws):
    L.check(L.lib().mic_embed_rows_add_det(_dt(dh), int(n), int(width), int(dtable.shape[0]) if dtable.dim() == 2 else int(dtable.numel() // width),
                                           _p(ids), _p(dh), float(scale), _p(dtable), _p(ws), _stream()), "mic_embed_rows_add_det")


def ce_rows(logits, ld, V, labels, mask, ls, row_lse, row_loss, rows):
    L.check(L.lib().mic_ce_rows(_dt(logits), rows, V, _p(logits), ld, _p(labels), _p(mask), float(ls), _p(row_lse), _p(row_loss), _stream()), "mic_ce_rows")


def ce_rows_tiles(logits, ld, V, rowstat, labels, row_lse, row_loss, rows):
    L.check(L.lib().mic_ce_rows_tiles(_dt(logits), rows, V, _p(logits), ld, _p(rowstat), rowstat.stride(0) // 2, _p(labels), _p(row_lse),
                                      _p(row_loss), _stream()), "mic_ce_rows_tiles")


def row_topk_tiles(logits, ld, V, rowstat, k, top_val, top_idx, R, *, suppress_eos=False, eos_token_id=2, raw_logits=False, row_bias=None):
    L.check(L.lib().mic_row_topk_tiles(_dt(logits), R, V, _p(logits), ld, _p(rowstat), rowstat.stride(0) // 2, k, int(suppress_eos),
                                       eos_token_id, int(raw_logits), _p(row_bias), _p(top_val), _p(top_idx), _stream()), "mic_row_topk_tiles")


def ce_reduce(row_loss, mask, loss_out, denom_out, rows):
    L.check(L.lib().mic_ce_reduce(rows, _p(row_loss), _p(mask), _p(loss_out), _p(denom_out), _stream()), "mic_ce_reduce")


def ce_bwd(logits, ld, V, Vpad, labels, mask, ls, row_lse, denom, rows, loss_scale=1.0):
    L.check(L.lib().mic_ce_bwd(_dt(logits), rows, V, Vpad, _p(logits), ld, _p(labels), _p(mask), float(ls), _p(row_lse), _p(denom),
                               float(loss_scale), _stream()), "mic_ce_bwd")


def ce_bwd_q8(logits, ld, V, Vpad, labels, mask, ls, row_lse, denom, rows, q8, colsum=None, label_coef=None, loss_scale=1.0):
    L.check(L.lib().mic_ce_bwd_q8(rows, V, Vpad, _p(logits), ld, _p(labels), _p(mask), float(ls), _p(row_lse), _p(denom), float(loss_scale),
                                  C.byref(q8), _p(colsum), _p(label_coef), _stream()), "mic_ce_bwd_q8")


def head_label_terms(labels, coef, E, h, dx_slab, dE, rows, width):
    L.check(L.lib().mic_head_label_terms(rows, width, _p(labels), _p(coef), _p(E), E.stride(0), _p(h), h.stride(0), _p(dx_slab), dx_slab.stride(0),
                                         _p(dE), dE.stride(0), _stream()), "mic_head_label_terms")


def ce_bwd_t(logits, ld, V, Vpad, labels, mask, ls, row_lse, denom, rows, dlogits_t, rows_pad=0, colsum=None, loss_scale=1.0):
    L.check(L.lib().mic_ce_bwd_t(rows, V, Vpad, _p(logits), ld, _p(labels), _p(mask), float(ls), _p(row_lse), _p(denom), float(loss_scale),
                                 _p(dlogits_t), dlogits_t.stride(0), int(rows_pad), _p(colsum), _stream()), "mic_ce_bwd_t")


def transpose_bf16(src, dst, rows, cols, rows_pad=0):
    L.check(L.lib().mic_transpose_bf16(int(rows), int(rows_pad), int(cols), _p(src), src.stride(0), _p(dst), dst.stride(0), _stream()),
            "mic_transpose_bf16")
    return dst


def colsum(x, out, rows, cols, ld, accumulate=False):
    L.check(L.lib().mic_colsum(_dt(x), rows, cols, _p(x), ld, _p(out), int(accumulate), _stream()), "mic_colsum")


def colsum_grouped(items):
    arr = (L.ColsumItem * len(items))(*[L.ColsumItem(_p(x), _p(out), rows, cols, ld) for (x, out, rows, cols, ld) in items])
    L.check(L.lib().mic_colsum_grouped(_dt(items[0][0]), arr, len(items), _stream()), "mic_colsum_grouped")


def dropout_mask(n: int, p: float, seed: int, device) -> torch.Tensor:
    out = torch.empty(n, dtype=torch.uint8, device=device)
    L.check(L.lib().mic_dropout_mask(_p(out), n, float(p), int(seed) & 0xFFFFFFFF, _stream()), "mic_dropout_mask")
    return out


def cast(src, dst, n=None):
    n = n if n is not None else src.numel()
    L.check(L.lib().mic_cast(_dt(src), _dt(dst), _p(src), _p(dst), n, _stream()), "mic_cast")
    return dst


def zero(t: torch.Tensor):
    if t.numel() == 0:
        return t
    if not t.is_contiguous():
        raise L.MicError("ops.zero needs a contiguous tensor")
    L.check(L.lib().mic_zero(_p(t), t.numel() * t.element_size(), _stream()), "mic_zero")
    return t


def cu_masked_stream(first_cu: int, n_cus: int, device) -> "torch.cuda.Stream":
    import ctypes

    dev = torch.device(device)
    key = (dev.index if dev.index is not None else torch.cuda.current_device(), int(first_cu), int(n_cus))
    st = _masked_streams.get(key)
    if st is None:
        h = ctypes.c_void_p()
        with torch.cuda.device(dev):
            L.check(L.lib().mic_stream_create_cu_masked(int(first_cu), int(n_cus), ctypes.byref(h)), "mic_stream_create_cu_masked")
        st = _masked_streams[key] = torch.cuda.ExternalStream(h.value, device=dev)
    return st


_masked_streams = {}
_role_streams = {}


def role_stream(device, role: str) -> "torch.cuda.Stream":
    dev = torch.device(device)
    key = (dev.index if dev.index is not None else torch.cuda.current_device(), role)
    st = _role_streams.get(key)
    if st is None:
        import os

        prio = int(os.environ.get("MIC_PRIO_" + role.upper(), "0"))
        st = _role_streams[key] = torch.cuda.Stream(device=dev, priority=prio) if prio else torch.cuda.Stream(device=dev)
    return st


def sum_slabs(src, n_slabs, slab_stride, dst, rows, cols, ld_src, ld_dst):
    L.check(L.lib().mic_sum_slabs(_dt(dst), n_slabs, int(slab_stride), rows, cols, _p(src), ld_src, _p(dst), ld_dst, _stream()), "mic_sum_slabs")
    return dst


def cast2d(src, dst, rows, cols, ld_src, ld_dst):
    L.check(L.lib().mic_cast2d(_dt(src), _dt(dst), rows, cols, _p(src), ld_src, _p(dst), ld_dst, _stream()), "mic_cast2d")
    return dst


def copy_rows(src, dst, n, width, *, src_idx=None, dst_idx=None):
    L.check(L.lib().mic_copy_rows(_dt(src), n, width, _p(src), src.stride(0), _p(src_idx), _p(dst), dst.stride(0), _p(dst_idx), _stream()),
            "mic_copy_rows")


def adamw(p, m, v, g, p_lp, hyper, b1, b2, eps, wd, grad_scale=1.0, n=None):
    n = n if n is not None else p.numel()
    L.check(L.lib().mic_adamw(n, _p(p), _p(m), _p(v), _p(g), _p(p_lp), _p(hyper), float(b1), float(b2), float(eps), float(wd),
                              float(grad_scale), _stream()), "mic_adamw")


def adamw_rows(rows, width, row_flag, want, p, m, v, g, p_lp, hyper, b1, b2, eps, wd, grad_scale=1.0):
    L.check(L.lib().mic_adamw_rows(int(rows), int(width), _p(row_flag), int(want), _p(p), _p(m), _p(v), _p(g), _p(p_lp), _p(hyper), float(b1),
                                   float(b2), float(eps), float(wd), float(grad_scale), _stream()), "mic_adamw_rows")


def row_flags(ids, n_ids, flags):
    L.check(L.lib().mic_row_flags(_p(ids), int(n_ids), _p(flags), flags.numel(), _stream()), "mic_row_flags")


def row_lse_topk(logits, ld, V, k, top_val, top_idx, R, *, forced_token=-1, suppress_eos=False, eos_token_id=2, raw_logits=False,
                 row_bias=None):
    L.check(L.lib().mic_row_lse_topk(_dt(logits), R, V, _p(logits), ld, k, int(forced_token), int(suppress_eos), eos_token_id,
                                     int(raw_logits), _p(row_bias), _p(top_val), _p(top_idx), _stream()), "mic_row_lse_topk")


def beam_step(B, K, max_len, V, cur_len, eos, pad, length_penalty, early_stopping, cand_val, cand_idx, running_seq, running_scores,
              seq, scores, finished, src_row, next_token, flags, gstate=None):
    a = L.BeamStepArgs()
    a.B, a.K, a.max_len, a.V, a.cur_len = B, K, max_len, V, cur_len
    a.eos_token_id, a.pad_token_id, a.length_penalty, a.early_stopping = eos, pad, float(length_penalty), int(bool(early_stopping))
    a.cand_val, a.cand_idx = _p(cand_val), _p(cand_idx)
    a.running_seq, a.running_scores, a.seq, a.scores = _p(running_seq), _p(running_scores), _p(seq), _p(scores)
    a.finished, a.src_row, a.next_token, a.flags = _p(finished), _p(src_row), _p(next_token), _p(flags)
    a.gstate = _p(gstate)
    L.check(L.lib().mic_beam_step(C.byref(a), _stream()), "mic_beam_step")


def greedy_step(B, max_len, cur_len, eos, pad, top_idx, ld_top, sequences, finished, next_token):
    L.check(L.lib().mic_greedy_step(B, max_len, cur_len, eos, pad, _p(top_idx), ld_top, _p(sequences), _p(finished), _p(next_token),
                                    _stream()), "mic_greedy_step")


def sample_rows(logits, ld, V, key, out_idx, R, *, temperature=1.0, forced_token=-1, suppress_eos=False, eos_token_id=2, min_keep=None,
                tie_limit=None):
    L.check(L.lib().mic_sample_rows(_dt(logits), R, V, _p(logits), ld, int(key[0]) & 0xFFFFFFFF, int(key[1]) & 0xFFFFFFFF,
                                    float(temperature), int(forced_token), int(suppress_eos), eos_token_id, _p(min_keep), _p(tie_limit),
                                    _p(out_idx), _stream()), "mic_sample_rows")


def warp_thresholds(logits, ld, V, thr, tie_limit, R, *, temperature=1.0, suppress_eos=False, eos_token_id=2, top_k=0, top_p=1.0):
    L.check(L.lib().mic_warp_thresholds(_dt(logits), R, V, _p(logits), ld, float(temperature), int(suppress_eos), eos_token_id,
                                        int(top_k or 0), float(top_p if top_p is not None else 1.0), _p(thr), _p(tie_limit), _stream()),
            "mic_warp_thresholds")


def image_transform(images, out_size, mean, std, dst, *, chw_out=False):
    import ctypes as C

    n = len(images)
    items = (L.ImageItem * n)()
    for i, im in enumerate(images):
        if im.dtype != torch.uint8 or im.dim() != 3 or not im.is_contiguous():
            raise L.MicError("image_transform: images must be contiguous uint8 [3,H,W] or [H,W,3] tensors")
        hwc = im.shape[-1] == 3 and im.shape[0] != 3
        H, W = (im.shape[0], im.shape[1]) if hwc else (im.shape[1], im.shape[2])
        items[i].src, items[i].H, items[i].W, items[i].hwc = _p(im), H, W, int(hwc)
    m, s = (C.c_float * 3)(*[float(x) for x in mean]), (C.c_float * 3)(*[float(x) for x in std])
    L.check(L.lib().mic_image_transform(items, n, out_size, m, s, _p(dst), int(chw_out), _stream()), "mic_image_transform")
    return dst
```

Baseline: 3540.

## Run LM-head backward GEMMs on the w4 kernel with k-major operands

Adds k-major operand support to the w4 pipelined GEMM kernel, using transposing LDS reads (ds_read_b64_tr_b16) and k-strided buffer loads. The default head path now writes bf16 dlogits in place while accumulating the bias column sum, then feeds dlogits and the shared embedding directly to the w4 kernel for both dE and dh. This removes the explicit dlogits transpose and the transposed embedding copy. In exchange it adds new addressing and swizzle code and a wider plan that forces 256 tiles with K padded to 256.

New measurement: 3576, median of 6. 1.0% higher.

```diff
diff --git a/include/mic_hip.h b/include/mic_hip.h
--- a/include/mic_hip.h
+++ b/include/mic_hip.h
@@ -51,6 +51,7 @@
   long long* rowsum2;
   int k_valid;
   float* c_q8_state; float* c_q8_amax; int c_q8_fmt;
+  int w4_kmajor;
 } mic_gemm_args;
 int mic_gemm(const mic_gemm_args* a, void* stream);
 int mic_sum_slabs(int dst_dtype, int n_slabs, long long slab_stride, int rows, int cols, const float* src, int ld_src,
@@ -163,6 +164,8 @@
 int mic_ce_bwd_t(int rows, int V, int Vpad, void* logits, int ld, const int32_t* labels, const int32_t* mask, float label_smoothing,
                  const float* row_lse, const float* denom, float loss_scale, void* dlogits_t, int ld_t, int rows_pad, float* colsum,
                  void* stream);
+int mic_ce_bwd_colsum(int rows, int V, int Vpad, void* logits, int ld, const int32_t* labels, const int32_t* mask, float label_smoothing,
+                      const float* row_lse, const float* denom, float loss_scale, float* colsum, void* stream);
 int mic_transpose_bf16(int rows, int rows_pad, int cols, const void* src, int ld_src, void* dst, int ld_dst, void* stream);
 
 int mic_colsum(int dtype, int rows, int cols, const void* x, int ld, float* out, int accumulate, void* stream);
diff --git a/multilingual-image-captioning_amd/_lib.py b/multilingual-image-captioning_amd/_lib.py
--- a/multilingual-image-captioning_amd/_lib.py
+++ b/multilingual-image-captioning_amd/_lib.py
@@ -30,6 +30,7 @@
         ("a_ln_stats", C.c_void_p), ("a_ln_colsum", C.c_void_p), ("a_ln_width", C.c_int), ("a_ln_eps", C.c_float),
         ("rowsum2", C.c_void_p), ("k_valid", C.c_int),
         ("c_q8_state", C.c_void_p), ("c_q8_amax", C.c_void_p), ("c_q8_fmt", C.c_int),
+        ("w4_kmajor", C.c_int),
     ]
 
 
@@ -119,6 +120,7 @@
     "mic_ce_reduce": ([_i, _p, _p, _p, _p, _p], C.c_int),
     "mic_ce_bwd": ([_i, _i, _i, _i, _p, _i, _p, _p, _f, _p, _p, _f, _p], C.c_int),
     "mic_ce_bwd_t": ([_i, _i, _i, _p, _i, _p, _p, _f, _p, _p, _f, _p, _i, _i, _p, _p], C.c_int),
+    "mic_ce_bwd_colsum": ([_i, _i, _i, _p, _i, _p, _p, _f, _p, _p, _f, _p, _p], C.c_int),
     "mic_ce_bwd_q8": ([_i, _i, _i, _p, _i, _p, _p, _f, _p, _p, _f, C.POINTER(Fp8Out), _p, _p, _p], C.c_int),
     "mic_head_label_terms": ([_i, _i, _p, _p, _p, _i, _p, _i, _p, _i, _p, _i, _p], C.c_int),
     "mic_transpose_bf16": ([_i, _i, _i, _p, _i, _p, _i, _p], C.c_int),
diff --git a/multilingual-image-captioning_amd/csrc/elementwise.hip b/multilingual-image-captioning_amd/csrc/elementwise.hip
--- a/multilingual-image-captioning_amd/csrc/elementwise.hip
+++ b/multilingual-image-captioning_amd/csrc/elementwise.hip
@@ -640,6 +640,7 @@
   const int32_t* labels; const int32_t* mask; float ls; const float* row_lse; const float* denom; float loss_scale;
   float* colsum; uint8_t* q; int ldq; float* state; int fmt;
   float* label_coef;
+  uint16_t* d16;
 };
 constexpr int CEQ8_RG = 4;
 __global__ __launch_bounds__(256) void ce_bwd_q8_kernel(CeQ8Args a) {
@@ -648,9 +649,11 @@
   const int c0 = blockIdx.x * 512;
   const int col = c0 + lane * 8;
   const bool col_ok = col < a.Vpad;
+  const bool b16 = a.d16 != nullptr;
   const float fmax = a.fmt == MIC_E4M3 ? 448.0f : 57344.0f;
   const float inv_denom = a.loss_scale / a.denom[0];
-  if (blockIdx.x == 0 && blockIdx.y == 0 && tid == 0) { a.state[0] = fmax / inv_denom; a.state[1] = inv_denom / fmax; }
+  if (!b16 && blockIdx.x == 0 && blockIdx.y == 0 && tid == 0) { a.state[0] = fmax / inv_denom; a.state[1] = inv_denom / fmax; }
+  const float wm = b16 ? inv_denom : 1.0f;
   const float conf = 1.0f - a.ls, low = a.ls > 0.f ? a.ls / (float)(a.V - 1) : 0.f;
   float csum[8] = {0.f, 0.f, 0.f, 0.f, 0.f, 0.f, 0.f, 0.f};
   for (int rg = 0; rg < CEQ8_RG; ++rg) {
@@ -667,12 +670,27 @@
     for (int rr = 0; rr < 16; ++rr) {
       const int row = r0 + wave * 16 + rr;
       if (row < a.rows && col_ok) {
-        const float w = a.mask[row] ? 1.0f : 0.f;
+        const float w = a.mask[row] ? wm : 0.f;
         const float lse = a.row_lse[row];
         const int label = a.labels[row];
-        if (a.label_coef != nullptr && col == 0 && (label < 0 || label >= a.V)) a.label_coef[row] = 0.f;
+        if (!b16 && a.label_coef != nullptr && col == 0 && (label < 0 || label >= a.V)) a.label_coef[row] = 0.f;
         const uint32_t wd[4] = {q[rr].x, q[rr].y, q[rr].z, q[rr].w};
         float o[8];
+        if (b16) {
+#pragma unroll
+          for (int i = 0; i < 8; ++i) {
+            const float x = __uint_as_float((i & 1) ? (wd[i >> 1] & 0xffff0000u) : (wd[i >> 1] << 16));
+            const int c = col + i;
+            o[i] = c < a.V ? w * (__expf(x - lse) - (c == label ? conf : low)) : 0.f;
+          }
+          uint4 u;
+          u.x = f2bf_pk(o[0], o[1]); u.y = f2bf_pk(o[2], o[3]); u.z = f2bf_pk(o[4], o[5]); u.w = f2bf_pk(o[6], o[7]);
+          *reinterpret_cast<uint4*>(a.d16 + (size_t)row * a.ld + col) = u;
+          const uint32_t sw[4] = {u.x, u.y, u.z, u.w};
+#pragma unroll
+          for (int i = 0; i < 8; ++i) csum[i] += __uint_as_float((i & 1) ? (sw[i >> 1] & 0xffff0000u) : (sw[i >> 1] << 16));
+          continue;
+        }
 #pragma unroll
         for (int i = 0; i < 8; ++i) {
           const float x = __uint_as_float((i & 1) ? (wd[i >> 1] & 0xffff0000u) : (wd[i >> 1] << 16));
@@ -697,7 +715,7 @@
     for (int h = 0; h < 2; ++h) {
       const int c = tid + h * 256;
       const float s4 = (cs[0][c] + cs[1][c]) + (cs[2][c] + cs[3][c]);
-      if (c0 + c < a.Vpad && s4 != 0.f) atomicAdd(a.colsum + c0 + c, s4 * inv_denom);
+      if (c0 + c < a.Vpad && s4 != 0.f) atomicAdd(a.colsum + c0 + c, b16 ? s4 : s4 * inv_denom);
     }
   }
 }
@@ -713,6 +731,21 @@
   a.logits = (const uint16_t*)logits; a.ld = ld; a.rows = rows; a.V = V; a.Vpad = Vpad; a.labels = labels; a.mask = mask; a.ls = label_smoothing;
   a.row_lse = row_lse; a.denom = denom; a.loss_scale = loss_scale; a.colsum = colsum;
   a.q = (uint8_t*)q8->q; a.ldq = q8->ldq; a.state = q8->state; a.fmt = q8->fmt; a.label_coef = label_coef;
+  hipLaunchKernelGGL(ce_bwd_q8_kernel, dim3((Vpad + 511) / 512, (rows + 64 * CEQ8_RG - 1) / (64 * CEQ8_RG)), dim3(256), 0, (hipStream_t)stream, a);
+  MIC_LAUNCH_CHECK();
+  return MIC_OK;
+}
+
+extern "C" int mic_ce_bwd_colsum(int rows, int V, int Vpad, void* logits, int ld, const int32_t* labels, const int32_t* mask,
+                                 float label_smoothing, const float* row_lse, const float* denom, float loss_scale, float* colsum,
+                                 void* stream) {
+  MIC_CHECK(rows > 0 && V > 1 && Vpad >= V && Vpad % 8 == 0 && ld >= Vpad && ld % 8 == 0 && logits && labels && mask && row_lse && denom,
+            "mic_ce_bwd_colsum: bad args");
+  MIC_CHECK(((uintptr_t)logits & 15) == 0, "mic_ce_bwd_colsum: 16-B aligned bf16 logits");
+  CeQ8Args a{};
+  a.logits = (const uint16_t*)logits; a.ld = ld; a.rows = rows; a.V = V; a.Vpad = Vpad; a.labels = labels; a.mask = mask; a.ls = label_smoothing;
+  a.row_lse = row_lse; a.denom = denom; a.loss_scale = loss_scale; a.colsum = colsum;
+  a.d16 = (uint16_t*)logits;
   hipLaunchKernelGGL(ce_bwd_q8_kernel, dim3((Vpad + 511) / 512, (rows + 64 * CEQ8_RG - 1) / (64 * CEQ8_RG)), dim3(256), 0, (hipStream_t)stream, a);
   MIC_LAUNCH_CHECK();
   return MIC_OK;
diff --git a/multilingual-image-captioning_amd/csrc/gemm.hip b/multilingual-image-captioning_amd/csrc/gemm.hip
--- a/multilingual-image-captioning_amd/csrc/gemm.hip
+++ b/multilingual-image-captioning_amd/csrc/gemm.hip
@@ -163,6 +163,7 @@
     if (c128 < c256) bm = 128;
   }
   if (force == 256 || force == 128 || force == 64) bm = force;
+  if (args[0].w4_kmajor) bm = 256;
   if (args[0].dtype == MIC_FP8 && args[0].a_kmajor && bm < 128) bm = 128;
   for (int i = 0; i < count; ++i)
     if (args[i].c_dtype == MIC_FP8 && bm == 256) bm = 128;
@@ -189,6 +190,7 @@
   pl.phased = bm == 256 && !f8 && phased_env != 0 && !args[0].a_kmajor && !args[0].b_kmajor && count == 1 && !any_rowsum_early(args, count);
   static const int w4_env = [] { const char* e = getenv("MIC_GEMM_W4"); return e ? atoi(e) : 1; }();
   if (pl.phased && w4_env && args[0].K >= 256 && args[0].K % 128 == 0) pl.phased = 2;
+  if (args[0].w4_kmajor) pl.phased = 2;
   if (bm == 256) {
     pl.per_cu = 1;
   } else if (bm == 128) {
@@ -232,6 +234,7 @@
 static int launch_bf16(const mic_gemm_args* args, int count, hipStream_t s) {
   LaunchTable tab;
   tab.count = count;
+  tab.w4_layout = MIC_W4_NT;
   const int f8 = args[0].dtype == MIC_FP8 ? (args[0].a_fmt == MIC_E5M2 ? 2 : 1) : 0;
   const GemmPlan pl = plan_bf16(args, count);
   const int bm = pl.bm, bm_m = pl.bm_m;
@@ -270,6 +273,15 @@
   for (int i = 0; i < count; ++i)
     MIC_CHECK(!args[i].rowsum2 || table_is_plain(tab), "mic_gemm_grouped: rowsum2 needs every problem of the launch on the bare / residual epilogue");
   static const int d2_env = [] { const char* e = getenv("MIC_GEMM_D2"); return e ? atoi(e) : 3; }();
+  if (args[0].w4_kmajor) {
+    MIC_CHECK(count == 1 && !f8 && (args[0].a_kmajor || args[0].b_kmajor) && args[0].c_dtype == MIC_F32 && gemm_w4_takes(tab, args[0].a_kmajor, args[0].b_kmajor),
+              "mic_gemm: w4_kmajor takes one bf16 problem with a k-major operand, fp32 C (alpha / bias, split-K slabs), K %% 128 == 0 and >= 256, "
+              "k-major M / N %% 8 == 0, operands < 2^31 bytes (M=%d N=%d K=%d)", args[0].M, args[0].N, args[0].K);
+    tab.w4_layout = args[0].a_kmajor ? MIC_W4_TN : MIC_W4_NN;
+    launch_gemm_w4(tab, args[0].a_kmajor, args[0].b_kmajor, s);
+    MIC_LAUNCH_CHECK();
+    return MIC_OK;
+  }
   const bool nt1 = bm == 256 && !f8 && !args[0].a_kmajor && !args[0].b_kmajor && count == 1;
   if (d2_env && nt1 && gemm_d2_takes(tab) && (d2_env == 2 || (pl.phased == 2 && gemm_w4_takes(tab))) && (d2_env != 3 || tab.p[0].epi.rowstat)) {
     Problem& p = tab.p[0];
@@ -277,7 +289,7 @@
     tab.total_blocks = p.tiles_m * p.tiles_n * p.nsplit;
     launch_gemm_d2(tab, s);
   } else
-  if (bm == 256 && pl.phased == 2 && gemm_w4_takes(tab)) launch_gemm_w4(tab, s);
+  if (bm == 256 && pl.phased == 2 && gemm_w4_takes(tab)) launch_gemm_w4(tab, 0, 0, s);
   else if (bm == 256 && pl.phased && tab.p[0].nsplit == 1) launch_gemm_phased(tab, args[0].a_kmajor, args[0].b_kmajor, table_is_plain(tab), s);
   else if (bm == 256) launch_gemm_t256(tab, args[0].a_kmajor, args[0].b_kmajor, s, f8);
   else if (bm == 128 && bm_m == 192) launch_gemm_t192(tab, args[0].b_kmajor, s);
diff --git a/multilingual-image-captioning_amd/csrc/gemm_common.h b/multilingual-image-captioning_amd/csrc/gemm_common.h
--- a/multilingual-image-captioning_amd/csrc/gemm_common.h
+++ b/multilingual-image-captioning_amd/csrc/gemm_common.h
@@ -16,11 +16,12 @@
   const float* sa; const float* sb;
   EpiArgs epi;
 };
-struct LaunchTable { int count; int total_blocks; Problem p[MAX_PROBLEMS]; };
+enum { MIC_W4_NT = 0, MIC_W4_NN = 1, MIC_W4_TN = 2 };
+struct LaunchTable { int count; int total_blocks; Problem p[MAX_PROBLEMS]; int w4_layout; };
 int mic_cu_budget_now();
 void launch_gemm_phased(const LaunchTable& tab, int akm, int bkm, bool plain, hipStream_t s);
-bool gemm_w4_takes(const LaunchTable& tab);
-void launch_gemm_w4(const LaunchTable& tab, hipStream_t s);
+bool gemm_w4_takes(const LaunchTable& tab, int akm = 0, int bkm = 0);
+void launch_gemm_w4(const LaunchTable& tab, int akm, int bkm, hipStream_t s);
 bool gemm_d2_takes(const LaunchTable& tab);
 void launch_gemm_d2(const LaunchTable& tab, hipStream_t s);
 bool table_is_plain(const LaunchTable& t);
diff --git a/multilingual-image-captioning_amd/csrc/gemm_w4.hip b/multilingual-image-captioning_amd/csrc/gemm_w4.hip
--- a/multilingual-image-captioning_amd/csrc/gemm_w4.hip
+++ b/multilingual-image-captioning_amd/csrc/gemm_w4.hip
@@ -18,6 +18,29 @@
   int gx = x0 + R;
   gx = gx < lim ? gx : lim - 1;
   return ((uint32_t)gx * (uint32_t)ld + (uint32_t)(c * 8)) * 2u;
+}
+__device__ __forceinline__ uint32_t w4_source_k(int ld, int x0, int lim, int q, int lane) {
+  const int k = q * 4 + (lane >> 4), c = (lane & 15) ^ ((k & 3) << 2);
+  int gx = x0 + c * 8;
+  gx = gx < lim ? gx : 0;
+  return ((uint32_t)k * (uint32_t)ld + (uint32_t)gx) * 2u;
+}
+__device__ __forceinline__ bf16x8 w4_read_frag_k(const char* lds_tile, int xb, int kk, int lane) {
+  const int g = lane >> 4, p = lane & 15;
+  const int x = xb + 16 * (g & 1) + (p & 3) * 4;
+  const int k = kk * 16 + 8 * (g >> 1) + (p >> 2);
+  const int off = k * 256 + ((((x >> 3) ^ ((k & 3) << 2)) << 4) | ((x & 7) << 1));
+  const uint32_t a = (uint32_t)(uintptr_t)LDS_PTR(char, lds_tile + off);
+  s16x4 lo, hi;
+  asm volatile("ds_read_b64_tr_b16 %0, %1" : "=v"(lo) : "v"(a));
+  asm volatile("ds_read_b64_tr_b16 %0, %1 offset:1024" : "=v"(hi) : "v"(a));
+  s16x8 r = {lo[0], lo[1], lo[2], lo[3], hi[0], hi[1], hi[2], hi[3]};
+  return __builtin_bit_cast(bf16x8, r);
+}
+template <bool KM>
+__device__ __forceinline__ bf16x8 w4_frag(const char* lds_tile, int xb, int kk, int lane) {
+  if constexpr (KM) return w4_read_frag_k(lds_tile, xb, kk, lane);
+  else return read_frag<false, W4_BK, 128>(lds_tile, xb, kk, lane);
 }
 
 constexpr int W4_EP = 132;
@@ -152,8 +175,8 @@
   }
 }
 
-template <int EPI>
-__global__ __launch_bounds__(256) void gemm_w4_kernel(LaunchTable tab) {
+template <int EPI, bool AKM, bool BKM>
+__device__ __forceinline__ void w4_block(const LaunchTable& tab) {
   constexpr int WM = 128, WN = 128, WNW = 2, AI = 4, NJ = 4, BM = 256, BN = 256;
   extern __shared__ __attribute__((aligned(16))) char smem[];
   const int tid = threadIdx.x, lane = tid & 63, wave = __builtin_amdgcn_readfirstlane(tid >> 6);
@@ -201,9 +224,16 @@
   for (int h = 0; h < 4; ++h)
 #pragma unroll
     for (int i = 0; i < 4; ++i)
-      go[h * 4 + i] = h < 2 ? w4_source(P.lda, m0 + h * 128, P.M, wave * 4 + i, lane) : w4_source(P.ldb, n0 + (h - 2) * 128, P.N, wave * 4 + i, lane);
-  const __amdgpu_buffer_rsrc_t rA = __builtin_amdgcn_make_buffer_rsrc((void*)(reinterpret_cast<const char*>(P.A) + (size_t)kt0 * 128), 0, 0x7fffffff, 0x00020000);
-  const __amdgpu_buffer_rsrc_t rB = __builtin_amdgcn_make_buffer_rsrc((void*)(reinterpret_cast<const char*>(P.B) + (size_t)kt0 * 128), 0, 0x7fffffff, 0x00020000);
+      go[h * 4 + i] = h < 2 ? (AKM ? w4_source_k(P.lda, m0 + h * 128, P.M, wave * 4 + i, lane) : w4_source(P.lda, m0 + h * 128, P.M, wave * 4 + i, lane))
+                            : (BKM ? w4_source_k(P.ldb, n0 + (h - 2) * 128, P.N, wave * 4 + i, lane) : w4_source(P.ldb, n0 + (h - 2) * 128, P.N, wave * 4 + i, lane));
+  const char* kA = reinterpret_cast<const char*>(P.A) + (AKM ? (size_t)kt0 * 128 * (size_t)P.lda : (size_t)kt0 * 128);
+  const char* kB = reinterpret_cast<const char*>(P.B) + (BKM ? (size_t)kt0 * 128 * (size_t)P.ldb : (size_t)kt0 * 128);
+  const uint32_t kstA = 128u * (uint32_t)P.lda, kstB = 128u * (uint32_t)P.ldb;
+  const int kleft = max(P.k_valid - kt0 * 64, 0);
+  const int recA = AKM ? (int)min((long long)kleft * P.lda * 2, 0x7fffffffLL) : 0x7fffffff;
+  const int recB = AKM ? (int)min((long long)kleft * P.ldb * 2, 0x7fffffffLL) : 0x7fffffff;
+  const __amdgpu_buffer_rsrc_t rA = __builtin_amdgcn_make_buffer_rsrc((void*)kA, 0, recA, 0x00020000);
+  const __amdgpu_buffer_rsrc_t rB = __builtin_amdgcn_make_buffer_rsrc((void*)kB, 0, recB, 0x00020000);
   const int nk = nsteps / 2;
   bf16x8 fa[AI][4], fb[NJ][4];
   const char* fa_ = smem + wr * W4_HIMG;
@@ -212,7 +242,8 @@
 #define W4_DMA(TILE, SLOT, Q)                                                                                                  \
   __builtin_amdgcn_raw_ptr_buffer_load_lds((TILE) < nk ? ((Q) < 8 ? rA : rB) : rZ,                                             \
                                            LDS_PTR(void, smem + (SLOT) * W4_SLOT + ((Q) >> 2) * W4_HIMG + (wave * 4 + ((Q) & 3)) * 1024), \
-                                           16, go[Q], (TILE) * 128, 0, 0)
+                                           16, AKM ? go[Q] + (uint32_t)(TILE) * ((Q) < 8 ? kstA : kstB) : go[Q],                  \
+                                           AKM ? 0 : (int)((uint32_t)(TILE) * ((Q) >= 8 && BKM ? kstB : 128u)), 0, 0)
 #define W4_BARRIER()                       \
   do {                                     \
     __builtin_amdgcn_sched_barrier(0);     \
@@ -230,8 +261,8 @@
                                                                            acc[(g_ & 15) >> 2][g_ & 3], 0, 0, 0);             \
       const int q_ = g_ >> 4, x_ = g_ & 15;                                                                                    \
       const int rk_ = (q_ + 3) & 3, rs_ = q_ == 0 ? (C) : 1 - (C);            \
-      if (x_ < 4) fa[x_][rk_] = read_frag<false, W4_BK, 128>(fa_ + rs_ * W4_SLOT, x_ * 32, rk_, lane);                         \
-      else if (x_ < 8) fb[x_ - 4][rk_] = read_frag<false, W4_BK, 128>(fb_ + rs_ * W4_SLOT, (x_ - 4) * 32, rk_, lane);          \
+      if (x_ < 4) fa[x_][rk_] = w4_frag<AKM>(fa_ + rs_ * W4_SLOT, x_ * 32, rk_, lane);                         \
+      else if (x_ < 8) fb[x_ - 4][rk_] = w4_frag<BKM>(fb_ + rs_ * W4_SLOT, (x_ - 4) * 32, rk_, lane);          \
       if ((q_ == 1 || q_ == 2) && (x_ & 1) == 1) W4_DMA(t + (C) + 2, C, (q_ - 1) * 8 + (x_ >> 1));                             \
       __builtin_amdgcn_sched_barrier(0);                                                                                       \
     }                                                                                                                          \
@@ -250,9 +281,10 @@
     for (int kk = 0; kk < 3; ++kk)
 #pragma unroll
       for (int x = 0; x < 4; ++x) {
-        fa[x][kk] = read_frag<false, W4_BK, 128>(fa_, x * 32, kk, lane);
-        fb[x][kk] = read_frag<false, W4_BK, 128>(fb_, x * 32, kk, lane);
-      }
+        fa[x][kk] = w4_frag<AKM>(fa_, x * 32, kk, lane);
+        fb[x][kk] = w4_frag<BKM>(fb_, x * 32, kk, lane);
+      }
+    if constexpr (AKM || BKM) asm volatile("s_waitcnt lgkmcnt(0)" ::: "memory");
     __builtin_amdgcn_sched_barrier(0);
     if (live) {
       for (int t = 0; t < nk; t += 2) {
@@ -272,13 +304,24 @@
   __syncthreads();
   MIC_TRACE(2);
   if (live) {
-    if constexpr (EPI == 8) w4_epilogue_f32(acc, P, smem, m0 + wr * WM, n0 + wc * WN, split, wave, lane);
+    if constexpr ((EPI & 8) != 0) w4_epilogue_f32(acc, P, smem, m0 + wr * WM, n0 + wc * WN, split, wave, lane);
     else w4_epilogue_lean<(EPI & 1) != 0, (EPI & 4) != 0>(acc, P, smem, m0 + wr * WM, n0 + wc * WN, wave, lane);
   }
 #ifdef MIC_TRACE_BLOCKS
   asm volatile("s_waitcnt vmcnt(0)" ::: "memory");
 #endif
   MIC_TRACE(3);
+}
+
+template <int EPI>
+__global__ __launch_bounds__(256) void gemm_w4_kernel(LaunchTable tab) {
+  if constexpr (EPI == 8) {
+    if (tab.w4_layout == MIC_W4_TN) w4_block<8, true, true>(tab);
+    else if (tab.w4_layout == MIC_W4_NN) w4_block<8, false, true>(tab);
+    else w4_block<8, false, false>(tab);
+  } else {
+    w4_block<EPI, false, false>(tab);
+  }
 }
 
 template <int EPI>
@@ -297,20 +340,25 @@
 
 }
 
-bool gemm_w4_takes(const LaunchTable& tab) {
+bool gemm_w4_takes(const LaunchTable& tab, int akm, int bkm) {
   if (tab.count != 1) return false;
   const Problem& p = tab.p[0];
   const EpiArgs& e = p.epi;
   const long long lim = 0x7fffffffLL;
-  if ((long long)p.M * p.lda * 2 >= lim || (long long)p.N * p.ldb * 2 >= lim) return false;
+  if ((long long)(akm ? p.K : p.M) * p.lda * 2 >= lim || (long long)(bkm ? p.K : p.N) * p.ldb * 2 >= lim) return false;
   if (p.K < 256 || p.K % 128 != 0 || e.R || e.drop_thr || e.rowsum2 || e.act || e.Zout || e.dact || e.accumulate) return false;
   if (((uintptr_t)e.C & 15) != 0) return false;
+  if ((akm && !bkm) || (akm && p.M % 8 != 0) || (bkm && p.N % 8 != 0)) return false;
   if (e.c_f32)
     return !e.rowstat && !e.ln_stats && (p.nsplit == 1 || p.split_stride > 0) && p.K / 64 / p.nsplit >= 2;
-  return p.nsplit == 1 && (e.ldc & 7) == 0 && (!e.ln_stats || p.N % 8 == 0);
-}
-void launch_gemm_w4(const LaunchTable& tab, hipStream_t s) {
+  return !akm && !bkm && p.nsplit == 1 && (e.ldc & 7) == 0 && (!e.ln_stats || p.N % 8 == 0);
+}
+void launch_gemm_w4(const LaunchTable& tab, int akm, int bkm, hipStream_t s) {
   const EpiArgs& e = tab.p[0].epi;
+  if (akm || bkm) {
+    launch_w4<8>(tab, s);
+    return;
+  }
   if (e.c_f32) { launch_w4<8>(tab, s); return; }
   const int epi = 2 + (e.rowstat ? 1 : 0) + (e.ln_stats ? 4 : 0);
   switch (epi) {
diff --git a/multilingual-image-captioning_amd/engine.py b/multilingual-image-captioning_amd/engine.py
--- a/multilingual-image-captioning_amd/engine.py
+++ b/multilingual-image-captioning_amd/engine.py
@@ -49,10 +49,12 @@
         self._lnf_version = -1
         self._dw_stream = None
         import os as _os
-        self.head_nt = _os.environ.get("MIC_HEAD_NT", "1") != "0"
+        _hn = _os.environ.get("MIC_HEAD_NT")
+        self.head_nt = "w4k" if _hn is None else _hn != "0"
         self.ln_partials = _os.environ.get("MIC_LN_PARTIALS", "1") != "0"
         self._lnp_queue = []
         self._head_nt_state = None
+        self._head_w4k_state = False
         self.fp8_head = 0
         self._head8_state = None
         self._head_x8 = None
@@ -318,6 +320,7 @@
             cb()
         self._bufs.clear()
         self._ET_version, self._ET_event, self._head_nt_state = -1, None, None
+        self._head_w4k_state = False
         self._lnf = {}
         self._lnf_version = -1
 
@@ -752,6 +755,7 @@
         Mhp = _rup(Mh, 64)
         nt = self._head_nt_state
         self._head_nt_state = None
+        w4k, self._head_w4k_state = self._head_w4k_state, False
         h8s, self._head8_state = self._head8_state, None
         if h8s is not None:
             x8 = self._head_x8 or self._quant(hf, Mh, d, "head.x", "head.x", torch.float8_e4m3fn)
@@ -769,6 +773,8 @@
             hfT = self.buf("d.hfT", d, dT.shape[1])
             ops.transpose_bf16(hf, hfT, Mh, d, rows_pad=Kp)
             ops.gemm(dT, hfT, P.g("shared"), P.Vpad, d, Kp)
+        elif w4k:
+            ops.gemm(dlogits, hf, P.g("shared"), P.Vpad, d, max(256, _rup(Mh, 128)), a_kmajor=True, b_kmajor=True, k_valid=Mh, w4_kmajor=True)
         elif self.dt == torch.bfloat16:
             ops.zero(P.g("flb"))
             ops.gemm(dlogits, hf, P.g("shared"), P.Vpad, d, Mhp, a_kmajor=True, b_kmajor=True, a_rowsum=P.g("flb"), rowsum_k=Mh)
@@ -783,7 +789,7 @@
             slab = slab_rows * d
             ops.gemm(h8s[0], ET8, d32, Mh, d, P.Vpad, split_k=nsp, split_stride=slab if nsp > 1 else 0, a_scale_inv=h8s[1][1:], b_scale_inv=wst[1:])
             ops.sum_slabs(d32, nsp + 1, slab, dhc, Mh, d, d32.stride(0), dhc.stride(0))
-        elif nt is not None:
+        elif nt is not None or w4k:
             tiles = ((Mh + 255) // 256) * ((d + 255) // 256)
             nsp = max(1, min(ops.get_cu_budget() // tiles, P.Vpad // 128 // 2))
             slab_rows = _rup(Mh, 256)
@@ -791,7 +797,11 @@
             d32 = self.buf("db.dhf32", cap_rows, d, torch.float32)
             assert nsp * slab_rows <= d32.shape[0], (nsp, slab_rows, d32.shape)
             slab = slab_rows * d
-            ops.gemm(dlogits, self.shared_T(), d32, Mh, d, P.Vpad, split_k=nsp, split_stride=slab if nsp > 1 else 0)
+            if w4k:
+                E = P.w("shared")
+                ops.gemm(dlogits, E, d32, Mh, d, P.Vpad, b_kmajor=True, split_k=nsp, split_stride=slab if nsp > 1 else 0, w4_kmajor=True)
+            else:
+                ops.gemm(dlogits, self.shared_T(), d32, Mh, d, P.Vpad, split_k=nsp, split_stride=slab if nsp > 1 else 0)
             if nsp > 1:
                 ops.sum_slabs(d32, nsp, slab, dhc, Mh, d, d32.stride(0), dhc.stride(0))
             else:
@@ -995,6 +1005,7 @@
                           label_coef=coef)
             self._head8_state = (q, st, coef, labels)
             self._head_nt_state = None
+            self._head_w4k_state = False
         elif backward:
             kcap = self._head_nt_kcap(logits)
             if kcap:
@@ -1003,17 +1014,31 @@
                 ops.zero(P.g("flb"))
                 ops.ce_bwd_t(logits, logits.stride(0), P.V, P.Vpad, labels, mask, label_smoothing, lse, denom, M, dT, rows_pad=Kp, colsum=P.g("flb"))
                 self._head_nt_state = (dT, Kp)
+                self._head_w4k_state = False
+            elif self._head_w4k(logits):
+                ops.zero(P.g("flb"))
+                ops.ce_bwd_colsum(logits, logits.stride(0), P.V, P.Vpad, labels, mask, label_smoothing, lse, denom, M, colsum=P.g("flb"))
+                self._head_nt_state = None
+                self._head_w4k_state = True
             else:
                 ops.ce_bwd(logits, logits.stride(0), P.V, P.Vpad, labels, mask, label_smoothing, lse, denom, M)
                 self._head_nt_state = None
+                self._head_w4k_state = False
         return loss
 
     def _head_nt_kcap(self, logits) -> int:
         P = self.P
-        if not self.head_nt or self.dt != torch.bfloat16 or P.Vpad < 16384 or P.d % 128 != 0 or self._head8():
+        if self.head_nt is not True or self.dt != torch.bfloat16 or P.Vpad < 16384 or P.d % 128 != 0 or self._head8():
             return 0
         kcap = _rup(logits.shape[0], 128)
         return kcap if P.Vpad * kcap * 2 < 0x7fffffff and logits.shape[0] * logits.stride(0) * 2 < 0x7fffffff else 0
+
+    def _head_w4k(self, logits) -> bool:
+        P = self.P
+        if self.head_nt != "w4k" or self.dt != torch.bfloat16 or P.Vpad < 16384 or P.d % 128 != 0 or self._head8():
+            return False
+        return (logits.shape[0] * logits.stride(0) * 2 < 0x7fffffff and P.Vpad * P.d * 2 < 0x7fffffff
+                and _rup(logits.shape[0], 256) * P.d * 2 < 0x7fffffff)
 
     def shared_T(self):
         P = self.P
@@ -1032,7 +1057,7 @@
     def refresh_shared_T(self, side, version: int):
         P = self.P
         ET = self._bufs.get(("w.sharedT", P.d, P.Vpad, self.dt))
-        if not self.head_nt or self.dt != torch.bfloat16 or ET is None or self._head8():
+        if self.head_nt is not True or self.dt != torch.bfloat16 or ET is None or self._head8():
             return
         ev = torch.cuda.Event()
         ev.record(torch.cuda.current_stream())
diff --git a/multilingual-image-captioning_amd/ops.py b/multilingual-image-captioning_amd/ops.py
--- a/multilingual-image-captioning_amd/ops.py
+++ b/multilingual-image-captioning_amd/ops.py
@@ -56,7 +56,7 @@
               bias=None, act=0, zout=None, zin=None, dact=0, residual=None, accumulate=False, dropout_p=0.0, dropout_seed=0,
               alpha=1.0, lda=None, ldb=None, ldc=None, ldz=None, ldr=None, split_k=0, split_stride=0, a_rowsum=None, rowsum_k=0,
               a_scale_inv=None, b_scale_inv=None, rowstat=None, rowstat_nvalid=0, ln_stats=None, ln_colsum=None, ln_width=0,
-              ln_eps=0.0, rowsum2=None, k_valid=0, c_q8=None) -> "L.GemmArgs":
+              ln_eps=0.0, rowsum2=None, k_valid=0, c_q8=None, w4_kmajor=False) -> "L.GemmArgs":
     g = L.GemmArgs()
     g.dtype, g.c_dtype = _dt(a), _dt(out)
     if g.dtype == L.MIC_FP8:
@@ -81,6 +81,7 @@
         g.a_ln_stats, g.a_ln_colsum, g.a_ln_width, g.a_ln_eps = _p(ln_stats), _p(ln_colsum), int(ln_width), float(ln_eps)
     g.rowsum2 = _p(rowsum2)
     g.k_valid = int(k_valid)
+    g.w4_kmajor = int(w4_kmajor)
     if c_q8 is not None:
         if g.c_dtype != L.MIC_FP8:
             raise L.MicError("c_q8 goes with an fp8 output tensor")
@@ -325,6 +326,11 @@
                                          _p(dE), dE.stride(0), _stream()), "mic_head_label_terms")
 
 
+def ce_bwd_colsum(logits, ld, V, Vpad, labels, mask, ls, row_lse, denom, rows, colsum=None, loss_scale=1.0):
+    L.check(L.lib().mic_ce_bwd_colsum(rows, V, Vpad, _p(logits), ld, _p(labels), _p(mask), float(ls), _p(row_lse), _p(denom), float(loss_scale),
+                                      _p(colsum), _stream()), "mic_ce_bwd_colsum")
+
+
 def ce_bwd_t(logits, ld, V, Vpad, labels, mask, ls, row_lse, denom, rows, dlogits_t, rows_pad=0, colsum=None, loss_scale=1.0):
     L.check(L.lib().mic_ce_bwd_t(rows, V, Vpad, _p(logits), ld, _p(labels), _p(mask), float(ls), _p(row_lse), _p(denom), float(loss_scale),
                                  _p(dlogits_t), dlogits_t.stride(0), int(rows_pad), _p(colsum), _stream()), "mic_ce_bwd_t")
```
